# BassyKuo/DAVO

Measured on AMD Instinct MI355X. Metric: pose-net triplets/sec (128x416x3-frame), higher is better.
Workload: dtype f32 (v_mfma_f32_32x32x2_f32: the reference's arithmetic, slim.conv2d in float32); 1 GPU; BASELINE.json configs[1]: single MI355X, batch=32 synthetic 128x416 triplets, dilatedPoseNN-cnv6_128 + se_flow + fc_tanh (segmask_all + abs_flow); batch_per_gpu=32, height=128, width=416, parallelism=window-sharded replicas x1, batches_in_flight=1

## Files before the change

davo_amd/_lib.py:

```python
import ctypes
import os
import subprocess

_HERE = os.path.dirname(os.path.abspath(__file__))
CSRC = os.path.join(_HERE, "csrc")
INCLUDE = os.path.join(os.path.dirname(_HERE), "include")
UNITS = ("api", "forward", "range_guard", "plan", "weights", "launch_f32", "launch_h3", "launch_h3s", "launch_h3w", "launch_h3_generic", "launch_misc", "launch_feature", "comm")


HIPCC_FLAGS = ["--offload-arch=gfx950", "-O3", "-std=c++17", "-fno-slp-vectorize"]


def lib_path(suffix=None):
    if suffix is None:
        suffix = os.environ.get("DAVO_LIB_SUFFIX", "")
    return os.path.join(_HERE, "libdavo_hip%s.so" % suffix)


LIB_PATH = lib_path()

EXPORTS = (
    "davo_create", "davo_set_posenn_se", "davo_load_weight", "davo_weights_missing", "davo_forward", "davo_forward_device", "davo_submit", "davo_wait", "davo_pending",
    "davo_forward_depth", "davo_forward_device_depth", "davo_submit_depth", "davo_calibrate_depth",
    "davo_last_error", "davo_destroy", "davo_device_malloc", "davo_device_free", "davo_memcpy_h2d",
    "davo_memcpy_d2h", "davo_synchronize", "davo_set_stream", "davo_set_inflight", "davo_profile_enable",
    "davo_profile_reset", "davo_profile_entry", "davo_profile_samples", "davo_last_plan", "davo_last_split", "davo_set_option", "davo_set_precision", "davo_set_impl", "davo_debug_read", "davo_conv2d_same",
    "davo_host_alloc", "davo_host_free", "davo_host_register", "davo_host_unregister", "davo_calibrate", "davo_activation_range", "davo_set_activation_shifts", "davo_reset_range_state", "davo_range_stats", "davo_range_report",
    "davo_comm_preload", "davo_comm_unique_id", "davo_comm_init", "davo_comm_size", "davo_allgather_poses", "davo_allgather_poses_device",
    "davo_comm_allreduce", "davo_comm_barrier", "davo_comm_destroy", "davo_plan_layer", "davo_tile_filter_rows",
    "davo_set_pairs", "davo_get_pairs",
    "davo_set_feature_export", "davo_forward_features",
)
COMM_ID_BYTES = 128


class DavoVariant(ctypes.Structure):
    _fields_ = [(n, ctypes.c_int32) for n in ("cin_per_frame", "cnv6_out", "se_act", "norm_flow",
                                              "abs_mode", "att_source", "mask_rgb", "mask_info")]


class DavoFeatureOut(ctypes.Structure):
    _fields_ = [(n, ctypes.c_void_p) for n in ("att_19", "attention", "masked_image", "image", "feat_rot", "feat_trans")]


def sources():
    return sorted(os.path.join(CSRC, f) for f in os.listdir(CSRC) if f.endswith((".hip", ".h"))) + \
           [os.path.join(INCLUDE, "davo_hip.h")]


LLVM_OBJDUMP = "/opt/rocm/lib/llvm/bin/llvm-objdump"


class PackedF32Error(RuntimeError):
    """The linked device code holds packed float32 arithmetic (see HIPCC_FLAGS above): the build is refused."""


def scan_packed_f32(so_path):
    import re
    import shutil
    import tempfile
    pat = re.compile(r"^\s*v_pk_(fma|mul|add)_f32\b")
    hits = []
    d = tempfile.mkdtemp(prefix="davo_isa_")
    try:
        tmp = os.path.join(d, "lib.so")
        shutil.copy(so_path, tmp)
        subprocess.check_call([LLVM_OBJDUMP, "--offloading", tmp], stdout=subprocess.DEVNULL, cwd=d)
        objs = sorted(f for f in os.listdir(d) if "amdgcn" in f)
        if not objs:
            raise PackedF32Error("no gfx950 code object found in %s: the packed-float32 scan cannot vouch for it" % so_path)
        for f in objs:
            kernel = None
            out = subprocess.run([LLVM_OBJDUMP, "-d", os.path.join(d, f)], check=True, capture_output=True, text=True).stdout
            for line in out.splitlines():
                m = re.match(r"^[0-9a-f]+ <([^>]+)>:", line)
                if m:
                    kernel = m.group(1)
                elif pat.match(line):
                    hits.append((kernel, line.strip()))
    finally:
        shutil.rmtree(d, ignore_errors=True)
    return hits


def build(force=False, verbose=False, suffix=None, extra_flags=(), allow_packed_f32=False):
    out = lib_path(suffix)
    if not force and os.path.exists(out) and all(os.path.getmtime(out) >= os.path.getmtime(s) for s in sources()):
        return out
    from concurrent.futures import ThreadPoolExecutor
    hipcc = os.environ.get("HIPCC", "/opt/rocm/bin/hipcc")
    flags = HIPCC_FLAGS + ["-fPIC", "-Wall", "-Wno-unused-function"] + \
        list(extra_flags) + os.environ.get("DAVO_EXTRA_HIPCC_FLAGS", "").split()
    objdir = os.path.join(CSRC, "build%s" % (suffix if suffix is not None else os.environ.get("DAVO_LIB_SUFFIX", "")))
    os.makedirs(objdir, exist_ok=True)
    headers = [s for s in sources() if s.endswith(".h")]
    newest_header = max(os.path.getmtime(h) for h in headers)

    def compile_unit(u):
        src, obj = os.path.join(CSRC, u + ".hip"), os.path.join(objdir, u + ".o")
        if not force and os.path.exists(obj) and os.path.getmtime(obj) >= max(os.path.getmtime(src), newest_header):
            return obj
        cmd = [hipcc] + flags + ["-c", "-o", obj, src]
        if verbose:
            print(" ".join(cmd), flush=True)
        subprocess.check_call(cmd)
        return obj

    with ThreadPoolExecutor(max_workers=min(len(UNITS), os.cpu_count() or 4)) as ex:
        objs = list(ex.map(compile_unit, UNITS))
    staged = out + ".unchecked"
    cmd = [hipcc, "--offload-arch=gfx950", "-shared", "-fPIC", "-o", staged] + objs + ["-ldl", "-Wl,-rpath,/opt/rocm/lib"]
    if verbose:
        print(" ".join(cmd), flush=True)
    subprocess.check_call(cmd)
    hits = [] if allow_packed_f32 else scan_packed_f32(staged)
    if hits:
        os.remove(staged)
        raise PackedF32Error("%d packed float32 instruction(s) in the device code, e.g. %s: `%s' - one operand-select form of them "
                             "miscomputes on gfx950 (DESIGN.md section 4); the library was not installed"
                             % (len(hits), hits[0][0], hits[0][1]))
    os.replace(staged, out)
    return out


_lib = None
_lib_lock = __import__("threading").Lock()


def lib():
    global _lib
    if _lib is not None:
        return _lib
    with _lib_lock:
        return _load()


def _load():
    global _lib
    if _lib is not None:
        return _lib
    if not os.path.exists(LIB_PATH):
        raise RuntimeError("libdavo_hip.so is not built (%s missing): run `python -c 'import "
                           "__graft_entry__ as g; g.build()'`; there is no CPU fallback" % LIB_PATH)
    L = ctypes.CDLL(LIB_PATH)
    vp, i, f32p = ctypes.c_void_p, ctypes.c_int, ctypes.POINTER(ctypes.c_float)
    L.davo_create.argtypes = [ctypes.POINTER(vp), i, i, i, i, ctypes.POINTER(DavoVariant)]
    L.davo_set_posenn_se.argtypes = [vp, i]
    L.davo_load_weight.argtypes = [vp, ctypes.c_char_p, f32p, ctypes.POINTER(ctypes.c_int64), i]
    L.davo_weights_missing.argtypes = [vp]
    L.davo_forward.argtypes = [vp, i, vp, vp, vp, vp]
    L.davo_forward_device.argtypes = [vp, i, vp, vp, vp, vp, ctypes.POINTER(ctypes.c_float)]
    L.davo_submit.argtypes = [vp, i, vp, vp, vp, vp, i]
    L.davo_forward_depth.argtypes = [vp, i, vp, vp, vp, vp, vp]
    L.davo_forward_device_depth.argtypes = [vp, i, vp, vp, vp, vp, vp, ctypes.POINTER(ctypes.c_float)]
    L.davo_submit_depth.argtypes = [vp, i, vp, vp, vp, vp, vp, i]
    L.davo_calibrate_depth.argtypes = [vp, i, vp, vp, vp, vp, ctypes.POINTER(i)]
    L.davo_wait.argtypes = [vp, i]
    L.davo_pending.argtypes = [vp]
    L.davo_last_error.argtypes = [vp]
    L.davo_last_error.restype = ctypes.c_char_p
    L.davo_destroy.argtypes = [vp]
    L.davo_destroy.restype = None
    L.davo_device_malloc.argtypes = [vp, ctypes.c_size_t, ctypes.POINTER(vp)]
    L.davo_device_free.argtypes = [vp, vp]
    L.davo_host_alloc.argtypes = [i, ctypes.c_size_t, ctypes.POINTER(vp)]
    L.davo_host_free.argtypes = [vp]
    L.davo_host_register.argtypes = [i, vp, ctypes.c_size_t]
    L.davo_host_unregister.argtypes = [vp]
    L.davo_calibrate.argtypes = [vp, i, vp, vp, vp, ctypes.POINTER(i)]
    L.davo_activation_range.argtypes = [vp, f32p, ctypes.POINTER(i), i]
    L.davo_set_activation_shifts.argtypes = [vp, ctypes.POINTER(i)]
    L.davo_reset_range_state.argtypes = [vp]
    llp = ctypes.POINTER(ctypes.c_longlong)
    L.davo_range_stats.argtypes = [vp, llp, llp, llp]
    L.davo_range_report.argtypes = [vp]
    L.davo_range_report.restype = ctypes.c_char_p
    L.davo_memcpy_h2d.argtypes = [vp, vp, vp, ctypes.c_size_t]
    L.davo_memcpy_d2h.argtypes = [vp, vp, vp, ctypes.c_size_t]
    L.davo_synchronize.argtypes = [vp]
    L.davo_set_stream.argtypes = [vp, vp]
    L.davo_set_inflight.argtypes = [vp, i]
    L.davo_profile_enable.argtypes = [vp, i]
    L.davo_profile_reset.argtypes = [vp]
    L.davo_profile_entry.argtypes = [vp, i, ctypes.c_char_p, i, ctypes.POINTER(i), ctypes.POINTER(ctypes.c_double)]
    L.davo_profile_samples.argtypes = [vp, ctypes.c_char_p, i, f32p, i]
    L.davo_last_plan.argtypes = [vp, i, i, ctypes.POINTER(i), ctypes.POINTER(i)]
    L.davo_last_split.argtypes = [vp, i, ctypes.POINTER(i)]
    L.davo_set_option.argtypes = [vp, ctypes.c_char_p, i]
    L.davo_set_precision.argtypes = [vp, i]
    L.davo_set_impl.argtypes = [vp, i]
    L.davo_set_pairs.argtypes = [vp, i]
    L.davo_get_pairs.argtypes = [vp]
    L.davo_set_feature_export.argtypes = [vp, i]
    L.davo_forward_features.argtypes = [vp, i, vp, vp, vp, vp, vp, ctypes.POINTER(DavoFeatureOut)]
    L.davo_debug_read.argtypes = [vp, ctypes.c_char_p, f32p, ctypes.c_size_t]
    L.davo_conv2d_same.argtypes = [i, f32p, i, i, i, i, f32p, i, i, f32p, i, i, i, i, f32p, ctypes.c_char_p, i]
    ip = ctypes.POINTER(i)
    L.davo_plan_layer.argtypes = [i, i, i, ip, ip, ip]
    L.davo_tile_filter_rows.argtypes = [i] * 8 + [ip, ip, i, ip]
    L.davo_comm_preload.argtypes = [ctypes.c_char_p, i]
    L.davo_comm_unique_id.argtypes = [vp, ctypes.c_char_p, i]
    L.davo_comm_init.argtypes = [vp, i, i, vp]
    L.davo_comm_size.argtypes = [vp, ip, ip]
    L.davo_allgather_poses.argtypes = [vp, f32p, i, i, f32p, f32p]
    L.davo_allgather_poses_device.argtypes = [vp, vp, i, vp, f32p]
    L.davo_comm_allreduce.argtypes = [vp, ctypes.POINTER(ctypes.c_double), i]
    L.davo_comm_barrier.argtypes = [vp]
    L.davo_comm_destroy.argtypes = [vp]
    for name in EXPORTS:
        fn = getattr(L, name)
        if name not in ("davo_last_error", "davo_destroy", "davo_range_report"):
            fn.restype = ctypes.c_int
    _lib = L
    return L
```

davo_amd/csrc/api.hip:

```cpp
#include <algorithm>
#include <cmath>
#include <cstdlib>
#include <cstdint>
#include <cstring>

#include "ctx.h"
#include "launch.h"
#include "plan.h"

using namespace davo;

namespace davo {

int zero_now(davo_ctx* c, void* p, size_t bytes) {
    HIP_TRY(c, hipMemset(p, 0, bytes));
    HIP_TRY(c, hipStreamSynchronize(nullptr));
    return DAVO_OK;
}

int alloc_input_set(davo_ctx* c, InputSet* s, bool zero_unread) {
    const PlaneBytes nb = plane_bytes(c);
    const size_t n = (size_t)c->max_batch;
    HIP_TRY(c, hipMalloc(&s->img, nb.img * n));
    HIP_TRY(c, hipMalloc(&s->flow, nb.flow * n));
    HIP_TRY(c, hipMalloc(&s->seg, nb.seg * n));
    if (needs_depth(c)) HIP_TRY(c, hipMalloc(&s->depth, nb.depth * n));
    if (zero_unread) {
        { int rc = zero_now(c, s->flow, nb.flow * n); if (rc) return rc; }
        { int rc = zero_now(c, s->seg, nb.seg * n); if (rc) return rc; }
    }
    return DAVO_OK;
}

}

namespace {

void free_input_set(InputSet& s) {
    for (void* q : {s.img, s.flow, s.seg, s.depth}) if (q) (void)hipFree(q);
    s = InputSet();
}

void free_slot(Slot& s) {
    for (auto p : s.d_act) if (p) (void)hipFree(p);
    void* misc[] = {s.d_partial, s.d_tab, s.d_packed, s.d_pose_partial, s.d_counters, s.d_se, s.d_se_scale, s.d_se_partial};
    for (auto p : misc) if (p) (void)hipFree(p);
    if (s.stream) (void)hipStreamDestroy(s.stream);
    s = Slot();
}

void free_se_workspace(Slot& s) {
    for (float** p : {&s.d_se, &s.d_se_scale, &s.d_se_partial}) { if (*p) (void)hipFree(*p); *p = nullptr; }
}

int alloc_se_workspace(davo_ctx* c, Slot* s) {
    const size_t NB = 2 * (size_t)c->max_batch;
    free_se_workspace(*s);
    HIP_TRY(c, hipMalloc(reinterpret_cast<void**>(&s->d_se), NB * c->H2 * c->W2 * 512 * sizeof(float)));
    HIP_TRY(c, hipMalloc(reinterpret_cast<void**>(&s->d_se_scale), NB * 2 * 256 * sizeof(float)));
    HIP_TRY(c, hipMalloc(reinterpret_cast<void**>(&s->d_se_partial), NB * SE5_CHUNKS * 256 * sizeof(float)));
    return DAVO_OK;
}

int alloc_slot(davo_ctx* c, Slot* s) {
    const size_t NB = 2 * (size_t)c->max_batch;
    HIP_TRY(c, hipStreamCreateWithFlags(&s->stream, hipStreamNonBlocking));
    for (int i = 0; i < 7; ++i)
        HIP_TRY(c, hipMalloc(reinterpret_cast<void**>(&s->d_act[i]), NB * c->act_floats_per_img[i] * sizeof(float)));
    HIP_TRY(c, hipMalloc(reinterpret_cast<void**>(&s->d_packed), NB * (size_t)c->H * c->W * 10 * sizeof(float)));
    const size_t partial_bytes = (size_t)c->max_batch * SQ_CHUNKS * (att_class_table(c->v.att_source) ? 3 * SQ_REC : 2 * 2) * sizeof(float);
    HIP_TRY(c, hipMalloc(reinterpret_cast<void**>(&s->d_partial), partial_bytes));
    HIP_TRY(c, hipMalloc(reinterpret_cast<void**>(&s->d_tab), (size_t)c->max_batch * 3 * NCLS * sizeof(float)));
    HIP_TRY(c, hipMalloc(reinterpret_cast<void**>(&s->d_pose_partial), NB * 2 * PH_SPLIT * 3 * sizeof(float)));
    { int rc = zero_now(c, s->d_partial, partial_bytes); if (rc) return rc; }
    HIP_TRY(c, hipMalloc(reinterpret_cast<void**>(&s->d_counters), ((size_t)c->max_batch + 1 + SK_TILE_COUNTERS) * sizeof(unsigned)));
    { int rc = zero_now(c, s->d_counters, ((size_t)c->max_batch + 1 + SK_TILE_COUNTERS) * sizeof(unsigned)); if (rc) return rc; }
    if (c->posenn_se) { int rc = alloc_se_workspace(c, s); if (rc) return rc; }
    return DAVO_OK;
}

}

extern "C" {

int davo_create(davo_ctx** out, int device, int H, int W, int max_batch, const davo_variant* v) {
    if (!out || !v) return DAVO_ERR_INVALID;
    *out = nullptr;
    davo_ctx* c = new davo_ctx();
    *out = c;
    c->device = device; c->H = H; c->W = W; c->max_batch = max_batch;
    c->v = Variant{v->cin_per_frame, v->cnv6_out, v->se_act, v->norm_flow, v->abs_mode, v->att_source,
                   v->mask_rgb, v->mask_info};
    if (H < 16 || W < 16 || H % 4 || W % 4) return fail(c, DAVO_ERR_INVALID, "H and W must be multiples of 4 and >= 16 (got %dx%d)", H, W);
    if (max_batch < 1) return fail(c, DAVO_ERR_INVALID, "max_batch must be >= 1");
    if (v->cin_per_frame != 5 && v->cin_per_frame != 3) return fail(c, DAVO_ERR_INVALID, "cin_per_frame must be 3 or 5");
    if (ilog2_exact(v->cnv6_out) < 5 || v->cnv6_out > 256) return fail(c, DAVO_ERR_INVALID, "cnv6_out must be 32, 64, 128 or 256");
    if (v->se_act < 0 || v->se_act > 2 || v->abs_mode < 0 || v->abs_mode > 3 || v->att_source < 0 || v->att_source > 12)
        return fail(c, DAVO_ERR_INVALID, "variant field out of range");
    int ndev = 0;
    HIP_TRY(c, hipGetDeviceCount(&ndev));
    if (device < 0 || device >= ndev) return fail(c, DAVO_ERR_INVALID, "device %d not present (%d visible)", device, ndev);
    HIP_TRY(c, hipSetDevice(device));
    {
        hipDeviceProp_t prop;
        HIP_TRY(c, hipGetDeviceProperties(&prop, device));
        c->dev_cus = prop.multiProcessorCount > 0 ? prop.multiProcessorCount : 256;
        c->ncu = c->dev_cus;
    }
    c->needed = needed_names(c->v);

    c->H1 = (H + 1) / 2; c->W1 = (W + 1) / 2;
    c->H2 = (c->H1 + 1) / 2; c->W2 = (c->W1 + 1) / 2;
    c->H3 = (c->H2 + 1) / 2; c->W3 = (c->W2 + 1) / 2;
    const int c6 = c->v.cnv6_out;
    init_layer(c->L[0], "cnv1", 7, 2, 1, 8, 16, 1);
    init_layer(c->L[1], "cnv2", 5, 2, 1, 16, 32, 1);
    init_layer(c->L[2], "cnv3", 3, 1, 2, 32, 64, 1);
    init_layer(c->L[3], "cnv4", 3, 1, 4, 64, 128, 1);
    init_layer(c->L[4], "cnv5", 3, 1, 8, 128, 256, 1);
    init_layer(c->L[5], "cnv6", 3, 1, 2, 256, 2 * c6, 1);
    init_layer(c->L[6], "cnv7", 3, 2, 1, c6, 256, 2);

    const int ch[7] = {16, 32, 64, 128, 256, 2 * c6, 512};
    const size_t px[7] = {(size_t)c->H1 * c->W1, (size_t)c->H2 * c->W2, (size_t)c->H2 * c->W2, (size_t)c->H2 * c->W2,
                          (size_t)c->H2 * c->W2, (size_t)c->H2 * c->W2, (size_t)c->H3 * c->W3};
    for (int i = 0; i < 7; ++i) {
        c->act_ch[i] = ch[i];
        c->act_floats_per_img[i] = px[i] * ch[i];
    }
    c->slots.resize(1);
    { int rc = alloc_slot(c, &c->slots[0]); if (rc) return rc; }
    HIP_TRY(c, hipMalloc(reinterpret_cast<void**>(&c->d_zeros), 256));
    { int rc = zero_now(c, c->d_zeros, 256); if (rc) return rc; }
    HIP_TRY(c, hipMalloc(reinterpret_cast<void**>(&c->d_range_base), (1 + RANGE_RING) * RANGE_WORDS * sizeof(unsigned)));
    { int rc = zero_now(c, c->d_range_base, (1 + RANGE_RING) * RANGE_WORDS * sizeof(unsigned)); if (rc) return rc; }
    return DAVO_OK;
}

int davo_set_posenn_se(davo_ctx* c, int mode) {
    if (!c) return DAVO_ERR_INVALID;
    if (mode != 0 && mode != 1) return fail(c, DAVO_ERR_INVALID, "posenn_se mode must be 0 (none) or 1 (insert)");
    if (!c->weights.empty() || c->forward_seen)
        return fail(c, DAVO_ERR_INVALID, "davo_set_posenn_se must be called before the first davo_load_weight and the first forward "
                    "(it changes the variant's variables and cnv6's layout)");
    if (mode && c->v.att_source != 0)
        return fail(c, DAVO_ERR_INVALID, "the feature-attention PoseNN (`-se_insert') runs with att_source 0 (`-no_segmask') only, got %d", c->v.att_source);
    HIP_TRY(c, hipSetDevice(c->device));
    c->posenn_se = mode;
    const int c6 = c->v.cnv6_out;
    if (mode) init_layer(c->L[5], "cnv6", 3, 1, 2, 256, c6, 2);
    else init_layer(c->L[5], "cnv6", 3, 1, 2, 256, 2 * c6, 1);
    c->needed = needed_names(c->v, mode);
    for (Slot& s : c->slots) {
        if (mode) { int rc = alloc_se_workspace(c, &s); if (rc) return rc; }
        else free_se_workspace(s);
    }
    c->last_slot = 0;
    return DAVO_OK;
}

int davo_load_weight(davo_ctx* c, const char* tf_name, const float* data, const int64_t* shape, int ndim) {
    if (!c || !tf_name || !data || !shape || ndim < 1 || ndim > 4) return fail(c, DAVO_ERR_INVALID, "bad argument to davo_load_weight");
    std::vector<int64_t> want;
    if (!expected_shape(c, tf_name, &want)) return fail(c, DAVO_ERR_INVALID, "unknown variable `%s'", tf_name);
    bool listed = false;
    for (auto& n : c->needed) listed |= (n == tf_name);
    if (!listed) return fail(c, DAVO_ERR_INVALID, "variable `%s' is not part of this variant", tf_name);
    std::vector<int64_t> got(shape, shape + ndim);
    if (got != want) {
        std::string g, w;
        for (auto d : got) g += std::to_string(d) + ",";
        for (auto d : want) w += std::to_string(d) + ",";
        return fail(c, DAVO_ERR_INVALID, "`%s': shape [%s] does not match expected [%s]", tf_name, g.c_str(), w.c_str());
    }
    size_t n = 1;
    for (auto d : got) n *= (size_t)d;
    HostTensor& t = c->weights[tf_name];
    t.shape = got;
    t.data.assign(data, data + n);
    HIP_TRY(c, hipSetDevice(c->device));
    const std::string nm = tf_name;
    const bool dense = is_dense_weight(nm);
    if (t.dev) { (void)hipFree(t.dev); t.dev = nullptr; }
    if (dense) { int rc = upload(c, t.data, &t.dev); if (rc) return rc; }
    c->packed_ready = false;
    c->packed_h_ready = false;
    c->pred_ready = false;
    return DAVO_OK;
}

int davo_weights_missing(davo_ctx* c) {
    if (!c) return DAVO_ERR_INVALID;
    std::string names;
    const int n = missing_weights(c, &names);
    if (n) c->err = "weights not loaded: " + names;
    return n;
}

namespace {

int resolve_depth(davo_ctx* c, const char* fn, bool depth_form, const void** depth) {
    if (!needs_depth(c)) { *depth = nullptr; return DAVO_OK; }
    if (!depth_form) return fail(c, DAVO_ERR_INVALID, "%s: this variant reads depth planes (att_source %d): call %s_depth", fn, c->v.att_source, fn);
    if (!*depth) return fail(c, DAVO_ERR_INVALID, "%s_depth: null depth pointer", fn);
    return DAVO_OK;
}

}

static int forward_device_entry(davo_ctx* c, int B, const void* d_img, const void* d_flow, const void* d_seg, const void* d_depth,
                                void* d_pose, float* elapsed_ms, bool depth_form) {
    if (!c) return DAVO_ERR_INVALID;
    if (B < 1 || B > c->max_batch) return fail(c, DAVO_ERR_INVALID, "batch %d outside [1,%d]", B, c->max_batch);
    if (!d_img || !d_flow || !d_seg || !d_pose) return fail(c, DAVO_ERR_INVALID, "null device pointer");
    { int rc = resolve_depth(c, "davo_forward_device", depth_form, &d_depth); if (rc) return rc; }
    const Inputs in{d_img, d_flow, d_seg, d_depth};
    HIP_TRY(c, hipSetDevice(c->device));
    const bool ticketed = c->impl == 0 && c->precision == 1;
    if (ticketed) { int rc = ticket_reserve(c); if (rc) return rc; }
    Run run = make_run(c, c->next_slot);
    c->next_slot = (c->next_slot + 1) % c->inflight;
    Ticket t{};
    if (ticketed) { int rc = ticket_begin(c, &run, B, in, &t); if (rc) return rc; }
    if (!ticketed && c->book.spans_full()) {
        const int rc = judge_all(c);
        if (rc == DAVO_ERR_RANGE) c->book.defer(rc, c->err);
        else if (rc) return rc;
    }
    c->book.note_issue(d_pose, B);
    RunResult res;
    if (!elapsed_ms) {
        int rc = forward_device(c, run, B, in, d_pose, &res);
        return ticketed ? ticket_end(c, rc, res, t, d_pose) : rc;
    }
    hipEvent_t e0 = nullptr, e1 = nullptr;
    int rc = DAVO_OK;
    auto hip_ok = [&](hipError_t e, const char* what) {
        if (e != hipSuccess && rc == DAVO_OK) rc = fail(c, DAVO_ERR_HIP, "%s failed: %s", what, hipGetErrorString(e));
        return e == hipSuccess;
    };
    if (hip_ok(hipEventCreate(&e0), "hipEventCreate") && hip_ok(hipEventCreate(&e1), "hipEventCreate") &&
        hip_ok(hipEventRecord(e0, run.stream), "hipEventRecord")) {
        rc = forward_device(c, run, B, in, d_pose, &res);
        if (rc == DAVO_OK && hip_ok(hipEventRecord(e1, run.stream), "hipEventRecord") &&
            hip_ok(hipEventSynchronize(e1), "hipEventSynchronize"))
            hip_ok(hipEventElapsedTime(elapsed_ms, e0, e1), "hipEventElapsedTime");
    }
    if (e0) (void)hipEventDestroy(e0);
    if (e1) (void)hipEventDestroy(e1);
    if (ticketed) rc = ticket_end(c, rc, res, t, d_pose);
    if (rc == DAVO_OK && c->inflight == 1) rc = judge_all(c);
    return rc;
}

int davo_forward_device(davo_ctx* c, int B, const void* d_img, const void* d_flow, const void* d_seg,
                        void* d_pose, float* elapsed_ms) {
    return forward_device_entry(c, B, d_img, d_flow, d_seg, nullptr, d_pose, elapsed_ms, false);
}

int davo_forward_device_depth(davo_ctx* c, int B, const void* d_img, const void* d_flow, const void* d_seg, const void* d_depth,
                              void* d_pose, float* elapsed_ms) {
    return forward_device_entry(c, B, d_img, d_flow, d_seg, d_depth, d_pose, elapsed_ms, true);
}


namespace {

int ensure_stream_state(davo_ctx* c, int slot) {
    if (!c->d_pose_ring[0])
        for (int k = 0; k < STREAM_POSES; ++k) {
            HIP_TRY(c, hipMalloc(reinterpret_cast<void**>(&c->d_pose_ring[k]), (size_t)c->max_batch * 12 * sizeof(float)));
            HIP_TRY(c, hipHostMalloc(reinterpret_cast<void**>(&c->h_pose_ring[k]), (size_t)c->max_batch * 12 * sizeof(float), hipHostMallocDefault));
            HIP_TRY(c, hipEventCreateWithFlags(&c->pose_done[k], hipEventDisableTiming));
            HIP_TRY(c, hipEventCreateWithFlags(&c->st_copied[k], hipEventDisableTiming));
        }
    if (!c->stream_sets[slot].img) { int rc = alloc_input_set(c, &c->stream_sets[slot], true); if (rc) return rc; }
    return DAVO_OK;
}

Inputs from_window(const davo_ctx* c, const Inputs& in, int b0) {
    const PlaneBytes nb = plane_bytes(c);
    auto at = [b0](const void* q, size_t bytes) -> const void* { return q ? static_cast<const uint8_t*>(q) + bytes * b0 : nullptr; };
    return Inputs{at(in.img, nb.img), at(in.flow, nb.flow), at(in.seg, nb.seg), at(in.depth, nb.depth)};
}

int stage_inputs(davo_ctx* c, const InputSet& set, const Inputs& host, int b0, int nb, bool sources_only_seg, int sel, hipStream_t s) {
    const PlaneBytes n = plane_bytes(c);
    const Inputs src = from_window(c, host, b0);
    auto dst = [b0](void* q, size_t bytes) { return static_cast<uint8_t*>(q) + bytes * b0; };
    if (sel != PAIRS_BOTH) {
        const int src1 = sel == PAIRS_SRC1;
        auto copy2d = [&](uint8_t* d, const void* h, size_t pitch, size_t off, size_t width, size_t rows) {
            return hipMemcpy2DAsync(d + off, pitch, static_cast<const uint8_t*>(h) + off, pitch, width, rows, hipMemcpyHostToDevice, s);
        };
        const size_t row = (size_t)c->W * 9, third = row / 3;
        HIP_TRY(c, copy2d(dst(set.img, n.img), src.img, row, src1 ? third : 0, 2 * third, (size_t)nb * c->H));
        HIP_TRY(c, copy2d(dst(set.flow, n.flow), src.flow, n.flow, src1 ? n.flow / 4 : 0, n.flow / 4, nb));
        const size_t plane = n.seg / 3;
        if (att_tgt_attended(c->v.att_source)) HIP_TRY(c, copy2d(dst(set.seg, n.seg), src.seg, n.seg, src1 ? plane : 0, 2 * plane, nb));
        else HIP_TRY(c, copy2d(dst(set.seg, n.seg), src.seg, n.seg, src1 ? 2 * plane : 0, plane, nb));
        if (src.depth) HIP_TRY(c, copy2d(dst(set.depth, n.depth), src.depth, n.depth, src1 ? plane : 0, 2 * plane, nb));
        return DAVO_OK;
    }
    HIP_TRY(c, hipMemcpyAsync(dst(set.img, n.img), src.img, n.img * nb, hipMemcpyHostToDevice, s));
    if (nb == 1) HIP_TRY(c, hipMemcpyAsync(dst(set.flow, n.flow), src.flow, n.flow / 2, hipMemcpyHostToDevice, s));
    else HIP_TRY(c, hipMemcpy2DAsync(dst(set.flow, n.flow), n.flow, src.flow, n.flow, n.flow / 2, nb, hipMemcpyHostToDevice, s));
    if (!sources_only_seg || att_tgt_attended(c->v.att_source) || nb < 4) HIP_TRY(c, hipMemcpyAsync(dst(set.seg, n.seg), src.seg, n.seg * nb, hipMemcpyHostToDevice, s));
    else
        for (int plane = 0; plane < 3; plane += 2)
            HIP_TRY(c, hipMemcpy2DAsync(dst(set.seg, n.seg) + plane * (n.seg / 3), n.seg, (const uint8_t*)src.seg + plane * (n.seg / 3), n.seg,
                                        n.seg / 3, nb, hipMemcpyHostToDevice, s));
    if (src.depth) HIP_TRY(c, hipMemcpyAsync(dst(set.depth, n.depth), src.depth, n.depth * nb, hipMemcpyHostToDevice, s));
    return DAVO_OK;
}

int deliver_front(davo_ctx* c) {
    const StreamJob j = c->jobs.front();
    c->jobs.pop_front();
    while (j.ticketed && c->book.pending(j.seq)) {
        const int rc = judge_front(c);
        if (rc == DAVO_ERR_RANGE && !c->opt_auto_range) c->book.defer(rc, c->err);
        else if (rc) return rc;
    }
    HIP_TRY(c, hipEventSynchronize(c->pose_done[j.pr]));
    memcpy(j.pose_out, c->h_pose_ring[j.pr], (size_t)j.B * 12 * sizeof(float));
    return DAVO_OK;
}

int deliver_all(davo_ctx* c) {
    while (!c->jobs.empty()) { const int rc = deliver_front(c); if (rc) { c->jobs.clear(); return rc; } }
    return DAVO_OK;
}

}

static int submit_entry(davo_ctx* c, int B, const uint8_t* img, const float* flow, const float* seg, const float* depth_in, float* pose_out,
                        int hold, bool depth_form) {
    if (!c) return DAVO_ERR_INVALID;
    if (!img || !flow || !seg || !pose_out) return fail(c, DAVO_ERR_INVALID, "null host pointer");
    const void* depth = depth_in;
    { int rc = resolve_depth(c, "davo_submit", depth_form, &depth); if (rc) return rc; }
    if (B < 1 || B > c->max_batch) return fail(c, DAVO_ERR_INVALID, "batch %d outside [1,%d]", B, c->max_batch);
    if (hold < 0) return fail(c, DAVO_ERR_INVALID, "hold must be >= 0");
    HIP_TRY(c, hipSetDevice(c->device));
    while (!c->jobs.empty() && ((int)c->jobs.size() >= STREAM_POSES || hipEventQuery(c->pose_done[c->jobs.front().pr]) == hipSuccess)) {
        const int rc = deliver_front(c);
        if (rc) return rc;
    }
    const bool ticketed = c->impl == 0 && c->precision == 1;
    if (ticketed) { int rc = ticket_reserve(c); if (rc) return rc; }
    const int slot = c->next_slot, pr = (int)(c->n_submitted % STREAM_POSES);
    { int rc = ensure_stream_state(c, slot); if (rc) return rc; }
    Run run = make_run(c, slot);
    c->next_slot = (c->next_slot + 1) % c->inflight;
    hipStream_t s = run.stream;
    const InputSet& set = c->stream_sets[slot];
    { int rc = stage_inputs(c, set, Inputs{img, flow, seg, depth}, 0, B, true, c->pairs, s); if (rc) return rc; }
    const bool track_copy = hold < STREAM_POSES;
    if (track_copy) HIP_TRY(c, hipEventRecord(c->st_copied[pr], s));

    Ticket t{};
    if (ticketed) { int rc = ticket_begin(c, &run, B, set.view(), &t, true); if (rc) return rc; }
    c->book.note_issue();
    RunResult res;
    int rc = forward_device(c, run, B, set.view(), c->d_pose_ring[pr], &res);
    if (ticketed) rc = ticket_end(c, rc, res, t, c->d_pose_ring[pr], c->h_pose_ring[pr]);
    if (rc) return rc;
    HIP_TRY(c, hipMemcpyAsync(c->h_pose_ring[pr], c->d_pose_ring[pr], (size_t)B * 12 * sizeof(float), hipMemcpyDeviceToHost, s));
    HIP_TRY(c, hipEventRecord(c->pose_done[pr], s));
    c->jobs.push_back(StreamJob{B, pose_out, pr, ticketed && res.h3, t.seq});
    c->copy_tracked[pr] = track_copy;
    ++c->n_submitted;
    if (track_copy && (unsigned long long)hold < c->n_submitted) {
        const int q = (int)((c->n_submitted - 1 - hold) % STREAM_POSES);
        if (c->copy_tracked[q]) HIP_TRY(c, hipEventSynchronize(c->st_copied[q]));
    }
    return DAVO_OK;
}

int davo_submit(davo_ctx* c, int B, const uint8_t* img, const float* flow, const float* seg, float* pose_out, int hold) {
    return submit_entry(c, B, img, flow, seg, nullptr, pose_out, hold, false);
}

int davo_submit_depth(davo_ctx* c, int B, const uint8_t* img, const float* flow, const float* seg, const float* depth, float* pose_out, int hold) {
    return submit_entry(c, B, img, flow, seg, depth, pose_out, hold, true);
}

int davo_wait(davo_ctx* c, int leave_pending) {
    if (!c) return DAVO_ERR_INVALID;
    if (leave_pending < 0) return fail(c, DAVO_ERR_INVALID, "leave_pending must be >= 0");
    HIP_TRY(c, hipSetDevice(c->device));
    while ((int)c->jobs.size() > leave_pending) { const int rc = deliver_front(c); if (rc) return rc; }
    return DAVO_OK;
}

int davo_pending(davo_ctx* c) { return c ? (int)c->jobs.size() : DAVO_ERR_INVALID; }

namespace {

struct FxLayout { size_t rot, trans, masked, image, attention, att_19, total; };
FxLayout fx_layout(const davo_ctx* c, int cap) {
    const size_t HW = (size_t)c->H * c->W, n = (size_t)cap, c6 = (size_t)c->v.cnv6_out;
    FxLayout l{};
    l.rot = 0;
    l.trans = l.rot + n * HW * c6;
    l.masked = l.trans + n * HW * c6;
    l.image = l.masked + n * HW * 9;
    l.attention = l.image + n * HW * 9;
    l.att_19 = l.attention + n * HW * 3;
    l.total = l.att_19 + n * 3 * NCLS;
    return l;
}

void free_fx_workspace(davo_ctx* c) {
    if (c->d_fx) (void)hipFree(c->d_fx);
    c->d_fx = nullptr;
    c->fx_cap = 0;
}

bool fx_wanted(const davo_feature_out* o) {
    return o && (o->att_19 || o->attention || o->masked_image || o->image || o->feat_rot || o->feat_trans);
}

int export_features(davo_ctx* c, const Inputs& in, int w0, int nw, int b0, int B, const davo_feature_out& out) {
    if (!c->d_fx || c->fx_cap < 1) return fail(c, DAVO_ERR_INVALID, "internal: no feature export workspace");
    if (c->last_pairs != PAIRS_BOTH || w0 < 0 || w0 + nw > c->last_B) return fail(c, DAVO_ERR_INVALID, "internal: feature export of windows the last forward did not run");
    const size_t HW = (size_t)c->H * c->W, c6 = (size_t)c->v.cnv6_out;
    const bool h3 = c->last_precision == 1;
    const FxLayout l = fx_layout(c, c->fx_cap);
    const Slot& ws = last_workspace(c);
    hipStream_t s = last_stream(c);
    for (int p0 = 0; p0 < nw; p0 += c->fx_cap) {
        const int np = std::min(c->fx_cap, nw - p0);
        const Inputs win = from_window(c, in, w0 + p0);
        float* const w_att19 = out.att_19 ? c->d_fx + l.att_19 : nullptr;
        float* const w_att = out.attention ? c->d_fx + l.attention : nullptr;
        float* const w_masked = out.masked_image ? c->d_fx + l.masked : nullptr;
        float* const w_image = out.image ? c->d_fx + l.image : nullptr;
        float* const w_rot = out.feat_rot ? c->d_fx + l.rot : nullptr;
        float* const w_trans = out.feat_trans ? c->d_fx + l.trans : nullptr;
        if (w_att19 || w_att || w_masked || w_image) {
            ProfScope ps(c, s, "feature_maps");
            HIP_TRY(c, launch_feature_maps(static_cast<const uint8_t*>(win.img), static_cast<const float*>(win.seg),
                                           ws.d_tab + (size_t)(w0 + p0) * 3 * NCLS, c->v, np, c->H, c->W, w_att19, w_att, w_masked, w_image, s));
        }
        if (w_rot || w_trans) {
            ProfScope ps(c, s, "feature_resize_cnv6");
            HIP_TRY(c, launch_feature_resize_cnv6(h3, ws.d_act[5], w0 + p0, np, c->H2, c->W2, (int)c6, h3 ? ldexpf(1.0f, -c->act_shift[5]) : 1.0f,
                                                  w_rot, w_trans, s));
        }
        const size_t first = (size_t)(b0 + p0);
        auto frames = [&](float* host, const float* dev, size_t per_window) -> int {
            if (!host) return DAVO_OK;
            for (int f = 0; f < 3; ++f)
                HIP_TRY(c, hipMemcpyAsync(host + ((size_t)f * B + first) * per_window, dev + (size_t)f * np * per_window,
                                          (size_t)np * per_window * sizeof(float), hipMemcpyDeviceToHost, s));
            return DAVO_OK;
        };
        { int rc = frames(out.att_19, w_att19, NCLS); if (rc) return rc; }
        { int rc = frames(out.attention, w_att, HW); if (rc) return rc; }
        { int rc = frames(out.masked_image, w_masked, HW * 3); if (rc) return rc; }
        { int rc = frames(out.image, w_image, HW * 3); if (rc) return rc; }
        if (w_rot) HIP_TRY(c, hipMemcpyAsync(out.feat_rot + first * HW * c6, w_rot, (size_t)np * HW * c6 * sizeof(float), hipMemcpyDeviceToHost, s));
        if (w_trans) HIP_TRY(c, hipMemcpyAsync(out.feat_trans + first * HW * c6, w_trans, (size_t)np * HW * c6 * sizeof(float), hipMemcpyDeviceToHost, s));
        HIP_TRY(c, hipStreamSynchronize(s));
    }
    return DAVO_OK;
}

}

static int forward_entry(davo_ctx* c, int B, const uint8_t* img, const float* flow, const float* seg, const float* depth_in, float* pose_out,
                         bool depth_form, const davo_feature_out* fx = nullptr) {
    if (!c) return DAVO_ERR_INVALID;
    if (!img || !flow || !seg || !pose_out) return fail(c, DAVO_ERR_INVALID, "null host pointer");
    const void* depth = depth_in;
    { int rc = resolve_depth(c, "davo_forward", depth_form, &depth); if (rc) return rc; }
    if (B < 1 || B > c->max_batch) return fail(c, DAVO_ERR_INVALID, "batch %d outside [1,%d]", B, c->max_batch);
    HIP_TRY(c, hipSetDevice(c->device));
    { int rc = deliver_all(c); if (rc) return rc; }
    { int rc = sync_all_slots(c); if (rc) return rc; }
    if (!c->host_set.img) {
        { int rc = alloc_input_set(c, &c->host_set, false); if (rc) return rc; }
        HIP_TRY(c, hipMalloc(&c->s_pose, (size_t)c->max_batch * 12 * sizeof(float)));
    }
    if (!c->copy_stream) HIP_TRY(c, hipStreamCreateWithFlags(&c->copy_stream, hipStreamNonBlocking));
    { int rc = judge_all(c); if (rc) return rc; }
    Run run = make_run(c, 0);
    if (c->book.host_record_due()) {
        HIP_TRY(c, hipMemsetAsync(c->d_range_base, 0, RANGE_WORDS * sizeof(unsigned), run.stream));
    }
    const int chunk = (c->host_chunk > 0 && B >= 2 * c->host_chunk) ? c->host_chunk : B;
    const int nchunks = (B + chunk - 1) / chunk;
    while ((int)c->copy_done.size() < nchunks) {
        hipEvent_t e;
        HIP_TRY(c, hipEventCreateWithFlags(&e, hipEventDisableTiming));
        c->copy_done.push_back(e);
    }
    bool f32_fallback = false;
    RunResult res;
    const bool h3_call = c->impl == 0 && c->precision == 1;
    if (h3_call) { int rc = ensure_ring(c, false); if (rc) return rc; }
    if (!c->h_sync_pose) HIP_TRY(c, hipHostMalloc(reinterpret_cast<void**>(&c->h_sync_pose), (size_t)c->max_batch * 12 * sizeof(float), hipHostMallocDefault));
    unsigned seq = 0;
    for (int i = 0; i < nchunks; ++i) {
        const int b0 = i * chunk, nb = std::min(chunk, B - b0);
        hipStream_t cs = nchunks == 1 ? run.stream : c->copy_stream;
        { int rc = stage_inputs(c, c->host_set, Inputs{img, flow, seg, depth}, b0, nb, false, c->pairs, cs); if (rc) return rc; }
        if (nchunks > 1) {
            HIP_TRY(c, hipEventRecord(c->copy_done[i], c->copy_stream));
            HIP_TRY(c, hipStreamWaitEvent(run.stream, c->copy_done[i], 0));
        }
        if (h3_call && i == nchunks - 1) {
            seq = c->book.next_seq();
            run.snap.record = c->d_range_base; run.snap.host_mirror = c->h_range_dev; run.snap.seq = seq; run.snap.B = nb; run.snap.se = c->posenn_se;
        }
        int rc = forward_device(c, run, nb, from_window(c, c->host_set.view(), b0), (float*)c->s_pose + (size_t)b0 * 12, &res);
        if (rc) return rc;
        f32_fallback |= res.f32_fallback;
        if (fx && i < nchunks - 1 && (rc = export_features(c, from_window(c, c->host_set.view(), b0), 0, nb, b0, B, *fx))) return rc;
    }
    const int last_b0 = (nchunks - 1) * chunk;
    auto export_last = [&]() { return fx ? export_features(c, from_window(c, c->host_set.view(), last_b0), 0, B - last_b0, last_b0, B, *fx) : DAVO_OK; };
    if (f32_fallback) ++c->n_f32_batches;
    HIP_TRY(c, hipMemcpyAsync(c->h_sync_pose, c->s_pose, (size_t)B * 12 * sizeof(float), hipMemcpyDeviceToHost, run.stream));
    HIP_TRY(c, hipStreamSynchronize(run.stream));
    memcpy(pose_out, c->h_sync_pose, (size_t)B * 12 * sizeof(float));
    if (!res.h3) return export_last();
    unsigned raw[RANGE_WORDS];
    int rc = wait_record(c, c->h_range, seq, run.stream, raw);
    if (rc) return rc;
    rc = judge_record(c, raw, c->act_shift);
    if (rc == DAVO_ERR_RANGE && c->opt_auto_range) {
        rc = recover_batch(c, Reissue{B, c->pairs, c->host_set.view(), c->s_pose, false, 0});
        if (rc == DAVO_OK) HIP_TRY(c, hipMemcpy(pose_out, c->s_pose, (size_t)B * 12 * sizeof(float), hipMemcpyDeviceToHost));
        if (rc == DAVO_OK && fx) rc = export_features(c, c->host_set.view(), 0, B, 0, B, *fx);
        return rc;
    }
    return rc == DAVO_OK ? export_last() : rc;
}

int davo_forward(davo_ctx* c, int B, const uint8_t* img, const float* flow, const float* seg, float* pose_out) {
    return forward_entry(c, B, img, flow, seg, nullptr, pose_out, false);
}

int davo_forward_depth(davo_ctx* c, int B, const uint8_t* img, const float* flow, const float* seg, const float* depth, float* pose_out) {
    return forward_entry(c, B, img, flow, seg, depth, pose_out, true);
}

int davo_set_feature_export(davo_ctx* c, int on) {
    if (!c) return DAVO_ERR_INVALID;
    HIP_TRY(c, hipSetDevice(c->device));
    { int rc = sync_all_slots(c); if (rc) return rc; }
    if (!on) { free_fx_workspace(c); c->fx_on = false; return DAVO_OK; }
    if (!c->d_fx) {
        const int cap = c->host_chunk > 0 ? std::min(c->max_batch, 2 * c->host_chunk - 1) : c->max_batch;
        HIP_TRY(c, hipMalloc(reinterpret_cast<void**>(&c->d_fx), fx_layout(c, cap).total * sizeof(float)));
        c->fx_cap = cap;
    }
    c->fx_on = true;
    return DAVO_OK;
}

int davo_forward_features(davo_ctx* c, int B, const uint8_t* img, const float* flow, const float* seg, const float* depth, float* pose_out,
                          const davo_feature_out* out) {
    if (!c) return DAVO_ERR_INVALID;
    if (!c->fx_on) return fail(c, DAVO_ERR_NOT_READY, "davo_forward_features: the feature export is off - call davo_set_feature_export(ctx, 1) first");
    if (c->pairs != PAIRS_BOTH)
        return fail(c, DAVO_ERR_INVALID, "davo_forward_features runs both pairs of every window, the reference's semantics (davo.py:1456-1457): "
                    "davo_set_pairs(ctx, DAVO_PAIRS_BOTH) first (the selection is %d)", c->pairs);
    return forward_entry(c, B, img, flow, seg, depth, pose_out, true, fx_wanted(out) ? out : nullptr);
}

int davo_range_stats(davo_ctx* c, long long* recalibrations, long long* f32_batches, long long* reissued) {
    if (!c) return DAVO_ERR_INVALID;
    if (recalibrations) *recalibrations = c->n_recalibrations;
    if (f32_batches) *f32_batches = c->n_f32_batches;
    if (reissued) *reissued = c->n_reissued;
    return DAVO_OK;
}

int davo_activation_range(davo_ctx* c, float* max_abs, int* shifts, int reset) {
    if (!c) return DAVO_ERR_INVALID;
    HIP_TRY(c, hipSetDevice(c->device));
    { int rc = judge_all(c); if (rc && rc != DAVO_ERR_RANGE) return rc; }
    for (int i = 0; i < 6; ++i) {
        if (max_abs) max_abs[i] = c->range_seen[i];
        if (shifts) shifts[i] = c->act_shift[i];
    }
    if (reset) for (int i = 0; i < 6; ++i) c->range_seen[i] = 0.f;
    return DAVO_OK;
}

const char* davo_range_report(const davo_ctx* c) { return c ? c->range_report.c_str() : ""; }

int davo_set_activation_shifts(davo_ctx* c, const int* shifts) {
    if (!c) return DAVO_ERR_INVALID;
    { int rc = judge_all(c); if (rc) return rc; }
    { int rc = freeze_pending_and_reset_ring(c); if (rc) return rc; }
    c->book.host_record_stale();
    for (int i = 0; i < 6; ++i) {
        const int s = shifts ? shifts[i] : 0;
        if (s < -60 || s > 60) return fail(c, DAVO_ERR_INVALID, "activation shift %d outside [-60,60]", s);
        c->act_shift[i] = s;
    }
    return DAVO_OK;
}

int davo_reset_range_state(davo_ctx* c) {
    if (!c) return DAVO_ERR_INVALID;
    HIP_TRY(c, hipSetDevice(c->device));
    const int verdict = judge_all(c);
    if (verdict && verdict != DAVO_ERR_RANGE) return verdict;
    const std::string verdict_err = c->err;
    { int rc = freeze_pending_and_reset_ring(c); if (rc) return rc; }
    { int rc = zero_now(c, c->d_range_base, RANGE_WORDS * sizeof(unsigned)); if (rc) return rc; }
    for (int i = 0; i < 7; ++i) c->act_shift[i] = 0;
    for (int i = 0; i < 6; ++i) c->range_seen[i] = 0.f;
    c->book.reset();
    c->range_report.clear();
    if (verdict) { c->err = verdict_err; return verdict; }
    return DAVO_OK;
}

static int calibrate_entry(davo_ctx* c, int B, const void* d_img, const void* d_flow, const void* d_seg, const void* d_depth, int* shifts_out,
                           bool depth_form) {
    if (!c) return DAVO_ERR_INVALID;
    if (B < 1 || B > c->max_batch) return fail(c, DAVO_ERR_INVALID, "batch %d outside [1,%d]", B, c->max_batch);
    if (!d_img || !d_flow || !d_seg) return fail(c, DAVO_ERR_INVALID, "null device pointer");
    { int rc = resolve_depth(c, "davo_calibrate", depth_form, &d_depth); if (rc) return rc; }
    HIP_TRY(c, hipSetDevice(c->device));
    { int rc = judge_all(c); if (rc) return rc; }
    { int rc = freeze_pending_and_reset_ring(c); if (rc) return rc; }
    float* d_pose = nullptr;
    HIP_TRY(c, hipMalloc(reinterpret_cast<void**>(&d_pose), (size_t)B * 12 * sizeof(float)));
    const int rc = calibrate_on(c, B, Inputs{d_img, d_flow, d_seg, d_depth}, d_pose, PAIRS_BOTH);
    (void)hipFree(d_pose);
    if (rc == DAVO_OK && shifts_out) for (int i = 0; i < 6; ++i) shifts_out[i] = c->act_shift[i];
    return rc;
}

int davo_calibrate(davo_ctx* c, int B, const void* d_img, const void* d_flow, const void* d_seg, int* shifts_out) {
    return calibrate_entry(c, B, d_img, d_flow, d_seg, nullptr, shifts_out, false);
}

int davo_calibrate_depth(davo_ctx* c, int B, const void* d_img, const void* d_flow, const void* d_seg, const void* d_depth, int* shifts_out) {
    return calibrate_entry(c, B, d_img, d_flow, d_seg, d_depth, shifts_out, true);
}

const char* davo_last_error(const davo_ctx* c) { return c ? c->err.c_str() : "null context"; }

void davo_destroy(davo_ctx* c) {
    if (!c) return;
    (void)hipSetDevice(c->device);
    (void)sync_all_slots(c);
    comm_release(c);
    for (auto& kv : c->weights) if (kv.second.dev) (void)hipFree(kv.second.dev);
    for (auto& L : c->L) {
        if (L.d_w) (void)hipFree(L.d_w);
        if (L.d_b) (void)hipFree(L.d_b);
        if (L.d_wh) (void)hipFree(L.d_wh);
        if (L.d_bh) (void)hipFree(L.d_bh);
    }
    for (auto e : c->copy_done) (void)hipEventDestroy(e);
    if (c->copy_stream) { (void)hipStreamSynchronize(c->copy_stream); (void)hipStreamDestroy(c->copy_stream); }
    free_input_set(c->host_set);
    for (InputSet& set : c->stream_sets) free_input_set(set);
    for (InputSet& set : c->snap_sets) free_input_set(set);
    if (c->read_stream) { (void)hipStreamSynchronize(c->read_stream); (void)hipStreamDestroy(c->read_stream); }
    if (c->h_range) (void)hipHostFree(c->h_range);
    for (int k = 0; k < STREAM_POSES; ++k) {
        if (c->d_pose_ring[k]) (void)hipFree(c->d_pose_ring[k]);
        if (c->h_pose_ring[k]) (void)hipHostFree(c->h_pose_ring[k]);
        if (c->pose_done[k]) (void)hipEventDestroy(c->pose_done[k]);
        if (c->st_copied[k]) (void)hipEventDestroy(c->st_copied[k]);
    }
    if (c->h_sync_pose) (void)hipHostFree(c->h_sync_pose);
    free_fx_workspace(c);
    void* misc[] = {c->d_reissue_pose, c->d_range_base, c->d_splitk, c->d_pose_tiles, c->d_w1patch, c->d_w2patch, c->d_w3patch, c->d_w1patch_f32, c->d_w2patch_f32, c->d_w3patch_f32, c->d_zeros, c->d_wpred, c->d_bpred, c->s_pose};
    for (auto p : misc) if (p) (void)hipFree(p);
    for (auto& kv : c->tile_orders) if (kv.second) (void)hipFree(kv.second);
    for (auto& pe : c->prof_entries)
        for (auto& ab : pe.pending) { (void)hipEventDestroy(ab.first); (void)hipEventDestroy(ab.second); }
    for (auto e : c->event_pool) (void)hipEventDestroy(e);
    for (auto& sl : c->slots) free_slot(sl);
    delete c;
}

int davo_host_alloc(int device, size_t bytes, void** out) {
    if (!out || bytes == 0) return DAVO_ERR_INVALID;
    if (hipSetDevice(device) != hipSuccess) return DAVO_ERR_HIP;
    return hipHostMalloc(out, bytes, hipHostMallocDefault) == hipSuccess ? DAVO_OK : DAVO_ERR_HIP;
}
int davo_host_free(void* p) { return hipHostFree(p) == hipSuccess ? DAVO_OK : DAVO_ERR_HIP; }
int davo_host_register(int device, void* p, size_t bytes) {
    if (!p || bytes == 0) return DAVO_ERR_INVALID;
    if (hipSetDevice(device) != hipSuccess) return DAVO_ERR_HIP;
    return hipHostRegister(p, bytes, hipHostRegisterDefault) == hipSuccess ? DAVO_OK : DAVO_ERR_HIP;
}
int davo_host_unregister(void* p) { return hipHostUnregister(p) == hipSuccess ? DAVO_OK : DAVO_ERR_HIP; }

int davo_device_malloc(davo_ctx* c, size_t bytes, void** out) {
    if (!c || !out) return DAVO_ERR_INVALID;
    HIP_TRY(c, hipSetDevice(c->device));
    HIP_TRY(c, hipMalloc(out, bytes));
    return DAVO_OK;
}
int davo_device_free(davo_ctx* c, void* p) {
    if (!c) return DAVO_ERR_INVALID;
    HIP_TRY(c, hipSetDevice(c->device));
    HIP_TRY(c, hipFree(p));
    return DAVO_OK;
}
int davo_memcpy_h2d(davo_ctx* c, void* dst, const void* src, size_t bytes) {
    if (!c) return DAVO_ERR_INVALID;
    HIP_TRY(c, hipSetDevice(c->device));
    HIP_TRY(c, hipMemcpyAsync(dst, src, bytes, hipMemcpyHostToDevice, last_stream(c)));
    HIP_TRY(c, hipStreamSynchronize(last_stream(c)));
    return DAVO_OK;
}
int davo_memcpy_d2h(davo_ctx* c, void* dst, const void* src, size_t bytes) {
    if (!c) return DAVO_ERR_INVALID;
    HIP_TRY(c, hipSetDevice(c->device));
    HIP_TRY(c, hipMemcpyAsync(dst, src, bytes, hipMemcpyDeviceToHost, last_stream(c)));
    HIP_TRY(c, hipStreamSynchronize(last_stream(c)));
    return DAVO_OK;
}
int davo_synchronize(davo_ctx* c) {
    if (!c) return DAVO_ERR_INVALID;
    HIP_TRY(c, hipSetDevice(c->device));
    { int rc = deliver_all(c); if (rc) return rc; }
    return judge_all(c);
}
int davo_set_stream(davo_ctx* c, void* hip_stream) {
    if (!c) return DAVO_ERR_INVALID;
    if (hip_stream && c->inflight > 1) return fail(c, DAVO_ERR_INVALID, "a caller-owned stream needs davo_set_inflight(ctx, 1)");
    HIP_TRY(c, hipSetDevice(c->device));
    { int rc = deliver_all(c); if (rc) return rc; }
    { int rc = judge_all(c); if (rc) return rc; }
    c->user_stream = static_cast<hipStream_t>(hip_stream);
    c->last_slot = 0;
    return DAVO_OK;
}

int davo_profile_enable(davo_ctx* c, int on) {
    if (!c) return DAVO_ERR_INVALID;
    if (!on && c->prof) { int rc = prof_collect(c); if (rc) return rc; }
    c->prof = on != 0;
    c->prof_dominant_only = on == 2;
    return DAVO_OK;
}
int davo_profile_reset(davo_ctx* c) {
    if (!c) return DAVO_ERR_INVALID;
    int rc = prof_collect(c);
    if (rc) return rc;
    for (auto& pe : c->prof_entries) { pe.launches = 0; pe.total_ms = 0.0; pe.dur_ms.clear(); pe.period_ms.clear(); }
    return DAVO_OK;
}
int davo_profile_samples(davo_ctx* c, const char* name, int which, float* out, int cap) {
    if (!c || !name || which < 0 || which > 1 || cap < 0 || (cap > 0 && !out)) return DAVO_ERR_INVALID;
    int rc = prof_collect(c);
    if (rc) return rc;
    for (const auto& pe : c->prof_entries)
        if (pe.name == name) {
            const std::vector<float>& v = which == 0 ? pe.dur_ms : pe.period_ms;
            const int n = (int)std::min(v.size(), (size_t)cap);
            for (int i = 0; i < n; ++i) out[i] = v[i];
            return (int)v.size();
        }
    return 0;
}
int davo_profile_entry(davo_ctx* c, int i, char* name, int name_len, int* launches, double* total_ms) {
    if (!c) return DAVO_ERR_INVALID;
    int rc = prof_collect(c);
    if (rc) return rc;
    if (i < 0 || i >= (int)c->prof_entries.size()) return DAVO_ERR_INVALID;
    const ProfEntry& pe = c->prof_entries[i];
    if (name && name_len > 0) { strncpy(name, pe.name.c_str(), name_len - 1); name[name_len - 1] = 0; }
    if (launches) *launches = pe.launches;
    if (total_ms) *total_ms = pe.total_ms;
    return DAVO_OK;
}

int davo_last_plan(davo_ctx* c, int layer, int launch, int* mtiles, int* bn) {
    if (!c || layer < 0 || layer > 6 || launch < 0 || launch > 1) return DAVO_ERR_INVALID;
    const int v = c->last_plan[layer][launch];
    if (mtiles) *mtiles = v / 1000;
    if (bn) *bn = v % 1000;
    return DAVO_OK;
}

int davo_last_split(davo_ctx* c, int layer, int* parts) {
    if (!c || layer < 0 || layer > 6) return DAVO_ERR_INVALID;
    if (parts) *parts = c->last_split[layer];
    return DAVO_OK;
}

static int rebuild_slot_streams(davo_ctx* c, int n) {
    for (int i = 0; i < (int)c->slots.size(); ++i) {
        Slot& s = c->slots[i];
        if (s.stream) { HIP_TRY(c, hipStreamDestroy(s.stream)); s.stream = nullptr; }
        if (c->cu_partition && n > 1 && i < n && c->dev_cus == 256) {
            uint32_t mask[8] = {0, 0, 0, 0, 0, 0, 0, 0};
            const int lo = i * 32 / n, hi = (i + 1) * 32 / n;
            for (int b = 0; b < 256; ++b)
                if (b / 8 >= lo && b / 8 < hi) mask[b / 32] |= 1u << (b % 32);
            HIP_TRY(c, hipExtStreamCreateWithCUMask(&s.stream, 8, mask));
        } else {
            HIP_TRY(c, hipStreamCreateWithFlags(&s.stream, hipStreamNonBlocking));
        }
    }
    c->ncu = (c->cu_partition && n > 1 && c->dev_cus == 256) ? 256 / n : c->dev_cus;
    c->last_slot = 0;
    return DAVO_OK;
}

int davo_set_inflight(davo_ctx* c, int n) {
    if (!c || n < 1 || n > MAX_INFLIGHT) return fail(c, DAVO_ERR_INVALID, "inflight must be 1..4");
    if (n > 1 && c->user_stream) return fail(c, DAVO_ERR_INVALID, "in-flight slots use the context's own streams: clear davo_set_stream first");
    HIP_TRY(c, hipSetDevice(c->device));
    { int rc = deliver_all(c); if (rc) return rc; }
    { int rc = sync_all_slots(c); if (rc) return rc; }
    while ((int)c->slots.size() < n) {
        c->slots.emplace_back();
        int rc = alloc_slot(c, &c->slots.back());
        if (rc) return rc;
    }
    c->inflight = n;
    c->next_slot = 0;
    if (c->cu_partition || c->ncu != c->dev_cus) { int rc = rebuild_slot_streams(c, n); if (rc) return rc; }
    return DAVO_OK;
}

int davo_set_option(davo_ctx* c, const char* key, int value) {
    if (!c || !key) return DAVO_ERR_INVALID;
    const std::string k = key;
    if (k == "fuse_pose") c->opt_fuse_pose = value != 0;
    else if (k == "fuse_pack") c->opt_fuse_pack = value < 0 ? -1 : (value != 0);
    else if (k == "share_taps") c->opt_share_taps = value != 0;
    else if (k == "merge_rem") c->opt_merge_rem = value != 0;
    else if (k == "merge_cnv4") c->opt_merge_cnv4 = value != 0;
    else if (k == "tile_208x128") c->opt_tile_208x128 = value != 0;
    else if (k == "merge_order") c->opt_merge_order = value < 0 ? -1 : (value > 2 ? 0 : value);
    else if (k == "skip_order") c->opt_skip_order = value < 0 ? 0 : (value > 2 ? 2 : value);
    else if (k == "patch_cnv2") c->opt_patch_cnv2 = value != 0;
    else if (k == "patch_cnv3") c->opt_patch_cnv3 = value != 0;
    else if (k == "fold_tails") c->opt_fold_tails = value < 0 ? -1 : (value > 2 ? 1 : value);
    else if (k == "deep_ring") c->opt_deep_ring = value != 0;
    else if (k == "wave128") c->opt_wave128 = value < 0 ? 0 : (value > 3 ? 3 : value);
    else if (k == "split_k") c->opt_split_k = value != 0;
    else if (k == "fold_fixup") c->opt_fold_fixup = value != 0;
    else if (k == "f32_n16") c->opt_f32_n16 = value != 0;
    else if (k == "f32_n256") c->opt_f32_n256 = value != 0;
    else if (k == "merge_rem_f32") c->opt_merge_rem_f32 = value < 0 ? 0 : (value > 2 ? 2 : value);
    else if (k == "patch_f32") c->opt_patch_f32 = value != 0;
    else if (k == "auto_range") { int rc = judge_all(c); if (rc) return rc; c->opt_auto_range = value != 0; }
    else if (k == "stable_inputs") { int rc = judge_all(c); if (rc) return rc; c->opt_stable_inputs = value != 0; }
    else if (k == "force_tile") {
        if (value < -1 || value >= NUM_TILES) return fail(c, DAVO_ERR_INVALID, "force_tile must be -1..%d", NUM_TILES - 1);
        for (auto& L : c->L) L.tile_h = (value >= 0 && L.cout >= tile_shape(value).bn) ? value : -1;
    }
    else if (k == "cu_partition") {
        if (c->user_stream) return fail(c, DAVO_ERR_INVALID, "cu_partition uses the context's own streams: clear davo_set_stream first");
        HIP_TRY(c, hipSetDevice(c->device));
        { int rc = sync_all_slots(c); if (rc) return rc; }
        c->cu_partition = value != 0;
        int rc = rebuild_slot_streams(c, c->inflight);
        if (rc) return rc;
    }
    else if (k == "profile_stride") { if (value < 1) return fail(c, DAVO_ERR_INVALID, "profile_stride must be >= 1"); c->prof_stride = value; c->prof_tick = 0; }
    else if (k == "host_chunk") { if (value < 0) return fail(c, DAVO_ERR_INVALID, "host_chunk must be >= 0"); c->host_chunk = value; }
    else return fail(c, DAVO_ERR_INVALID, "unknown option `%s'", key);
    return DAVO_OK;
}

int davo_set_precision(davo_ctx* c, int precision) {
    if (!c || (precision != 0 && precision != 1)) return fail(c, DAVO_ERR_INVALID, "precision must be 0 (f32) or 1 (f16x3)");
    c->precision = precision;
    return DAVO_OK;
}

int davo_set_pairs(davo_ctx* c, int pairs) {
    if (!c) return DAVO_ERR_INVALID;
    if (pairs != DAVO_PAIRS_SRC0 && pairs != DAVO_PAIRS_SRC1 && pairs != DAVO_PAIRS_BOTH)
        return fail(c, DAVO_ERR_INVALID, "pairs must be DAVO_PAIRS_SRC0 (1), DAVO_PAIRS_SRC1 (2) or DAVO_PAIRS_BOTH (3), got %d", pairs);
    c->pairs = pairs;
    return DAVO_OK;
}

int davo_get_pairs(const davo_ctx* c) { return c ? c->pairs : DAVO_ERR_INVALID; }

int davo_set_impl(davo_ctx* c, int impl) {
    if (!c || (impl != 0 && impl != 1)) return fail(c, DAVO_ERR_INVALID, "impl must be 0 (mfma) or 1 (direct)");
    c->impl = impl;
    return DAVO_OK;
}

int davo_debug_read(davo_ctx* c, const char* tensor, float* host_out, size_t n_floats) {
    if (!c || !tensor || !host_out) return DAVO_ERR_INVALID;
    if (c->last_B < 1) return fail(c, DAVO_ERR_NOT_READY, "no forward has run yet");
    const size_t NB = (size_t)pairs_per_window(c->last_pairs) * c->last_B;
    const float* src = nullptr;
    size_t n = 0;
    const std::string t = tensor;
    const Slot& ws = last_workspace(c);
    if (t == "att_table") { src = ws.d_tab; n = (size_t)c->last_B * 3 * NCLS; }
    else if (t == "cnv5_se_scale" || t == "cnv5_se") {
        if (!c->posenn_se) return fail(c, DAVO_ERR_NOT_READY, "`%s' exists in the feature-attention variant only (davo_set_posenn_se)", tensor);
        if (t == "cnv5_se") { src = ws.d_se; n = NB * c->H2 * c->W2 * 512; }
        else { src = ws.d_se_scale; n = NB * 2 * 256; }
    }
    else if (t == "packed") {
        if (!c->packed_valid) {
            HIP_TRY(c, launch_mask_pack(16, static_cast<const uint8_t*>(c->last_in.img), static_cast<const float*>(c->last_in.flow),
                                        static_cast<const float*>(c->last_in.seg), ws.d_tab, c->v, c->last_B, c->H, c->W, ws.d_packed, c->last_pairs, last_stream(c)));
            c->packed_valid = true;
        }
        src = ws.d_packed; n = NB * c->H * c->W * c->packed_ld;
    }
    else {
        const char* names[7] = {"cnv1", "cnv2", "cnv3", "cnv4", "cnv5", "cnv6", "cnv7"};
        for (int i = 0; i < 7; ++i)
            if (t == names[i]) { src = ws.d_act[i]; n = NB * c->act_floats_per_img[i]; }
    }
    if (t == "pose_tiles") {
        if (c->cnv7_valid || !c->d_pose_tiles) return fail(c, DAVO_ERR_NOT_READY, "the pose head did not run fused");
#ifndef DAVO_POSE_DEBUG
        if (n_floats > c->pose_tiles_floats) return fail(c, DAVO_ERR_INVALID, "pose_tiles holds %zu floats", c->pose_tiles_floats);
#endif
        return davo_memcpy_d2h(c, host_out, c->d_pose_tiles, n_floats * sizeof(float));
    }
    if (t == "cnv7" && !c->cnv7_valid)
        return fail(c, DAVO_ERR_NOT_READY, "cnv7 was not materialised: the pose head ran fused (davo_set_option(ctx, \"fuse_pose\", 0))");
    if (!src) return fail(c, DAVO_ERR_INVALID, "unknown tensor `%s'", tensor);
    if (n != n_floats) return fail(c, DAVO_ERR_INVALID, "`%s' holds %zu floats, caller asked for %zu", tensor, n, n_floats);
    int rc = davo_memcpy_d2h(c, host_out, src, n * sizeof(float));
    if (rc) return rc;
    const bool split = c->last_precision == 1 && t != "att_table" && t != "cnv7" && t != "cnv5_se_scale";
    if (split) {
        int ch = 8;
        const char* names[6] = {"cnv1", "cnv2", "cnv3", "cnv4", "cnv5", "cnv6"};
        for (int i = 0; i < 6; ++i) if (t == names[i]) ch = c->act_ch[i];
        if (t == "cnv5_se") ch = 512;
        const int cb = ch < 32 ? ch : 32;
        int shift = t == "cnv5_se" ? c->act_shift[4] : 0;
        for (int i = 0; i < 6; ++i) if (t == names[i]) shift = c->act_shift[i];
        std::vector<float> tmp(ch);
        const size_t npix = n / ch;
        for (size_t px = 0; px < npix; ++px) {
            const _Float16* raw = reinterpret_cast<const _Float16*>(host_out + px * ch);
            for (int k = 0; k < ch; ++k) {
                const _Float16* blk = raw + (size_t)(k / cb) * cb * 2;
                tmp[k] = ldexpf((float)blk[k % cb] + (float)blk[cb + k % cb], -shift);
            }
            memcpy(host_out + px * ch, tmp.data(), ch * sizeof(float));
        }
    }
    return DAVO_OK;
}

int davo_tile_filter_rows(int m0, int m1, int Hout, int Wout, int Hin, int stride, int pad_t, int rate,
                          int* ky0, int* nky, int nblocks, int* chunk_map) {
    if (!ky0 || !nky || Hout < 1 || Wout < 1 || Hin < 1 || stride < 1 || rate < 1 || m0 < 0 || nblocks < 0) return DAVO_ERR_INVALID;
    const FilterRows fr = valid_filter_rows(m0, m1, Hout, Wout, Hin, stride, pad_t, rate);
    *ky0 = fr.ky0;
    *nky = fr.nky;
    if (chunk_map)
        for (int v = 0; v < 3 * fr.nky * nblocks; ++v) chunk_map[v] = h3_real_chunk(v, fr.ky0, fr.nky);
    return DAVO_OK;
}

int davo_plan_layer(int M, int npad, int groups, int* rows, int* tile_bm, int* tile_bn) {
    if (M < 1 || npad < 32 || npad % 32 || groups < 1 || !rows || !tile_bm || !tile_bn) return DAVO_ERR_INVALID;
    const std::vector<LaunchH> plan = plan_layer_h3(M, npad, groups, -1, npad == 256);
    if (plan.empty() || plan.size() > 2) return DAVO_ERR_INVALID;
    for (size_t i = 0; i < plan.size(); ++i) {
        const TileShape ts = tile_shape(plan[i].tile);
        rows[i] = plan[i].rows; tile_bm[i] = ts.bm; tile_bn[i] = ts.bn;
    }
    return (int)plan.size();
}

int davo_conv2d_same(int device, const float* x, int N, int H, int W, int Cin, const float* w, int k, int Cout,
                     const float* bias, int stride, int rate, int relu, int precision, float* y, char* err, int err_len) {
    auto bad = [&](const char* m, int code) {
        if (err && err_len > 0) { strncpy(err, m, err_len - 1); err[err_len - 1] = 0; }
        return code;
    };
    const int cl = ilog2_exact(Cin);
    if (!x || !w || !bias || !y) return bad("null pointer", DAVO_ERR_INVALID);
    if (cl < 2) return bad("Cin must be a power of two >= 4", DAVO_ERR_INVALID);
    if (precision == 1 && cl < 3) return bad("f16x3 needs Cin >= 8", DAVO_ERR_INVALID);
    if (!(k == 1 || k == 3 || k == 5 || k == 7) || !(stride == 1 || stride == 2) || rate < 1)
        return bad("k in {1,3,5,7}, stride in {1,2}, rate >= 1", DAVO_ERR_INVALID);
    if (hipSetDevice(device) != hipSuccess) return bad("hipSetDevice failed", DAVO_ERR_HIP);
    ConvLayer L;
    init_layer(L, "conv", k, stride, rate, Cin, Cout, 1);
    int Ho, Wo, pt, pl;
    same_pad(H, k, stride, rate, &Ho, &pt);
    same_pad(W, k, stride, rate, &Wo, &pl);
    const size_t nx = (size_t)N * H * W * Cin, ny = (size_t)N * Ho * Wo * Cout;
    std::vector<float> bp(precision == 1 ? L.npad_h : L.npad, 0.f);
    memcpy(bp.data(), bias, Cout * sizeof(float));
    std::vector<float> wp;
    std::vector<_Float16> wph, xh;
    const void *hx = x, *hw = nullptr;
    size_t wbytes = 0;
    if (precision == 1) {
        wph.assign((size_t)L.npad_h * L.nchunks_h * 64, (_Float16)0.0f);
        L.wscale = weight_prescale(w, (size_t)k * k * Cin * Cout);
        pack_conv_weights_h3(w, k, Cin, Cout, nullptr, Cin, L.cb_log2, L.tpc_log2, L.cpb, L.nchunks_h, L.wscale, wph.data());
        hw = wph.data(); wbytes = wph.size() * sizeof(_Float16);
        const int cb = 1 << L.cb_log2;
        xh.resize(nx * 2);
        for (size_t px = 0; px < nx / Cin; ++px)
            for (int ch = 0; ch < Cin; ++ch) {
                _Float16* blk = xh.data() + px * Cin * 2 + (size_t)(ch / cb) * cb * 2;
                split_f16(x[px * Cin + ch], blk + ch % cb, blk + cb + ch % cb);
            }
        hx = xh.data();
    } else {
        wp.assign((size_t)L.npad * L.kpad, 0.f);
        pack_conv_weights(w, k, Cin, Cout, nullptr, Cin, L.npad, L.kpad, wp.data());
        hw = wp.data(); wbytes = wp.size() * sizeof(float);
    }
    void *dx = nullptr, *dw = nullptr, *db = nullptr, *dy = nullptr, *dz = nullptr;
    hipError_t e = hipSuccess;
    auto chk = [&](hipError_t r) { if (e == hipSuccess) e = r; };
    chk(hipMalloc(&dx, nx * 4)); chk(hipMalloc(&dw, wbytes));
    chk(hipMalloc(&db, bp.size() * 4)); chk(hipMalloc(&dy, ny * 4));
    chk(hipMalloc(&dz, 256));
    if (e == hipSuccess) {
        chk(hipMemset(dz, 0, 256));
        chk(hipMemcpy(dx, hx, nx * 4, hipMemcpyHostToDevice));
        chk(hipMemcpy(dw, hw, wbytes, hipMemcpyHostToDevice));
        chk(hipMemcpy(db, bp.data(), bp.size() * 4, hipMemcpyHostToDevice));
        if (precision == 1) {
            const int tile = Cout <= 32 ? TILE_128x32 : Cout <= 64 ? TILE_256x64 : Cout <= 128 ? TILE_256x128 : TILE_128x256;
            const TileShape ts = tile_shape(tile);
            ConvParamsH p{};
            p.x = static_cast<const uint8_t*>(dx); p.w = static_cast<const uint8_t*>(dw);
            p.bias = static_cast<const float*>(db); p.y = static_cast<uint8_t*>(dy);
            p.zeros = static_cast<const uint8_t*>(dz);
            p.Hin = H; p.Win = W; p.Hout = Ho; p.Wout = Wo; p.x_pix_bytes = (long)Cin * 4; p.x_pix_log2 = -1;
            p.cb_log2 = L.cb_log2; p.tpc_log2 = L.tpc_log2; p.cpb = L.cpb; p.nchunks = L.nchunks_h;
            p.w_row_bytes = (long)L.nchunks_h * 128; p.y_mode = 0; p.y_ld = Cout; p.Cout = Cout;
            p.pad_t = pt; p.pad_l = pl; p.rate = rate; p.M = N * Ho * Wo; p.ntaps = k * k;
            p.Mtot = p.M; p.xs = 0; p.ntiles_n = L.npad_h / ts.bn; p.relu = relu; p.out_scale = 1.0f / L.wscale; p.bias_scale = L.wscale; p.range = nullptr;
            dim3 grid((p.M + ts.bm - 1) / ts.bm * p.ntiles_n, 1);
            const hipError_t le = launch_h3_generic(k, stride, tile, p, grid, nullptr);
            chk(le);
        } else {
            ConvParams p{};
            p.x = static_cast<const float*>(dx); p.w = static_cast<const float*>(dw);
            p.bias = static_cast<const float*>(db); p.y = static_cast<float*>(dy);
            p.zeros = static_cast<const float*>(dz);
            p.Hin = H; p.Win = W; p.Hout = Ho; p.Wout = Wo; p.cin_log2 = cl; p.x_ld = Cin; p.y_ld = Cout;
            p.Cout = Cout; p.pad_t = pt; p.pad_l = pl; p.rate = rate; p.M = N * Ho * Wo;
            p.nchunks = L.nchunks; p.Kpad = L.kpad; p.ntaps = k * k; p.ntiles_n = L.npad / L.BN; p.relu = relu;
            dim3 grid((p.M + BM - 1) / BM * p.ntiles_n, 1);
            chk(launch_conv(k, stride, L.BN, p, grid, nullptr));
        }
        chk(hipDeviceSynchronize());
        chk(hipMemcpy(y, dy, ny * 4, hipMemcpyDeviceToHost));
    }
    (void)hipFree(dz); (void)hipFree(dx); (void)hipFree(dw); (void)hipFree(db); (void)hipFree(dy);
    if (e != hipSuccess) return bad(hipGetErrorString(e), DAVO_ERR_HIP);
    return DAVO_OK;
}

}
```

davo_amd/csrc/conv_igemm.h:

```cpp
#pragma once
#include <hip/hip_runtime.h>
#include <stdint.h>

#include "params.h"

#ifndef DAVO_F32_ABLATE_A
#define DAVO_F32_ABLATE_A 0
#define DAVO_F32_ABLATE_B 0
#endif
#ifndef DAVO_F32_EARLY_STORE
#define DAVO_F32_EARLY_STORE 1
#endif
#ifndef DAVO_F32_FRAG0
#define DAVO_F32_FRAG0 1
#endif
#ifndef DAVO_F32_FAST_EPILOGUE
#define DAVO_F32_FAST_EPILOGUE 1
#endif
#ifndef DAVO_F32_FRAG_AHEAD
#define DAVO_F32_FRAG_AHEAD 0
#endif
#ifndef DAVO_F32_EARLY_STORE_MIN_BN
#define DAVO_F32_EARLY_STORE_MIN_BN 32
#endif
#ifndef DAVO_F32_ACC_AGPR
#define DAVO_F32_ACC_AGPR 0
#endif
#if DAVO_F32_ACC_AGPR
#define DAVO_MFMA32(acc_, a_, b_) asm volatile("v_mfma_f32_32x32x2_f32 %0, %1, %2, %0" : "+a"(acc_) : "v"(a_), "v"(b_))
#else
#define DAVO_MFMA32(acc_, a_, b_) acc_ = __builtin_amdgcn_mfma_f32_32x32x2f32(a_, b_, acc_, 0, 0, 0)
#endif
#if DAVO_F32_ACC_AGPR
#define DAVO_F4C(v_, c_) ((c_) == 0 ? (v_).x : (c_) == 1 ? (v_).y : (c_) == 2 ? (v_).z : (v_).w)
#define DAVO_MFMA_TILE(FA_, FB_)                                                                   \
            _Pragma("unroll") for (int c_ = 0; c_ < 4; ++c_)                                       \
                _Pragma("unroll") for (int i_ = 0; i_ < T::TM; ++i_)                               \
                    _Pragma("unroll") for (int j_ = 0; j_ < T::TN; ++j_)                           \
                        DAVO_MFMA32(acc[i_][j_], DAVO_F4C(FA_, c_), DAVO_F4C(FB_, c_));
#else
#define DAVO_MFMA_TILE(FA_, FB_)                                                                   \
            _Pragma("unroll") for (int i_ = 0; i_ < T::TM; ++i_)                                   \
                _Pragma("unroll") for (int j_ = 0; j_ < T::TN; ++j_) {                             \
                    DAVO_MFMA32(acc[i_][j_], (FA_).x, (FB_).x);                                    \
                    DAVO_MFMA32(acc[i_][j_], (FA_).y, (FB_).y);                                    \
                    DAVO_MFMA32(acc[i_][j_], (FA_).z, (FB_).z);                                    \
                    DAVO_MFMA32(acc[i_][j_], (FA_).w, (FB_).w);                                    \
                }
#endif
#ifndef DAVO_F32_ABLATE_BARRIER
#define DAVO_F32_ABLATE_BARRIER 0
#endif

namespace davo {

typedef float f32x16 __attribute__((ext_vector_type(16)));

__device__ __forceinline__ int xcd_remap(int bid, int nwg) {
    const int q = nwg >> 3, r = nwg & 7, xcd = bid & 7;
    const int start = xcd < r ? xcd * (q + 1) : r * (q + 1) + (xcd - r) * q;
    return start + (bid >> 3);
}

template <int KS, int STRIDE, int BN, int LAYER>
__device__ __forceinline__ void conv_igemm_f32_body(const ConvParams& p, const int wg_x, const int nwg_x, const int wg_y) {
    using T = Tile<BN>;
    constexpr bool N16 = BN == 16;
    extern __shared__ __attribute__((aligned(16))) float smem[];
    float* As = smem;
    float* Bs = smem + 2 * BM * LDK;

    const int tid = threadIdx.x;
    const int lane = tid & 63, wid = tid >> 6;
    const int li = lane & 31, lh = lane >> 5;
    const int wm = wid / T::WN, wn = wid % T::WN;

    const int tile_i = xcd_remap(wg_x, nwg_x);
    const int tile = p.tile_order ? __builtin_amdgcn_readfirstlane(p.tile_order[tile_i]) : tile_i;
    const int ntile = tile % p.ntiles_n, mtile = p.mtile0 + tile / p.ntiles_n;
    const int grp = wg_y;
    const float* __restrict__ xg = p.x + p.x_coff + grp * p.g_x_coff;
    const float* __restrict__ wg = p.w + grp * p.g_w + (long)ntile * BN * p.Kpad;
    const float* __restrict__ bg = p.bias + grp * p.g_bias + ntile * BN;
    float* __restrict__ yg = p.y + p.y_coff + grp * p.g_y_coff;

    const int r0 = tid >> 3, kk = (tid & 7) * 4;
    constexpr int RPP = T::RPP;
    int iy0[4], ix0[4], pix0[4];
#pragma unroll
    for (int j = 0; j < 4; ++j) {
        if (j >= T::A_LOADS) { iy0[j] = -(1 << 28); ix0[j] = 0; pix0[j] = 0; continue; }
        const int m = mtile * BM + r0 + RPP * j;
        if (m < p.M) {
            const int hw = p.Hout * p.Wout;
            const int n = m / hw, rem = m - n * hw;
            const int oy = rem / p.Wout, ox = rem - oy * p.Wout;
            iy0[j] = oy * STRIDE - p.pad_t;
            ix0[j] = ox * STRIDE - p.pad_l;
            pix0[j] = n * p.Hin * p.Win;
        } else {
            iy0[j] = -(1 << 28);
            ix0[j] = 0;
            pix0[j] = 0;
        }
    }
    const int cmask = (1 << p.cin_log2) - 1;

    float4 ra0, ra1, ra2, ra3, rb0, rb1, rb2, rb3;
    rb0 = rb1 = rb2 = rb3 = make_float4(0.f, 0.f, 0.f, 0.f);
    float4 sa0, sa1, sa2, sa3, sb0, sb1, sb2, sb3;
    sa0 = sa1 = sa2 = sa3 = sb0 = sb1 = sb2 = sb3 = make_float4(0.f, 0.f, 0.f, 0.f);
    const float *pa0 = p.zeros, *pa1 = p.zeros, *pa2 = p.zeros, *pa3 = p.zeros;
    int st0 = 0, st1 = 0, st2 = 0, st3 = 0;
    const int cpt = p.cin_log2 >= 5 ? 1 << (p.cin_log2 - 5) : 1;
    int l_cb = 0;
#define DAVO_ADDR_A(j_, ptr_, st_)                                                                 \
    {                                                                                              \
        const int iy = iy0[j_] + dy, ix = ix0[j_] + dx;                                            \
        const bool ok = tap_ok && (unsigned)iy < (unsigned)p.Hin && (unsigned)ix < (unsigned)p.Win && !DAVO_F32_ABLATE_A; \
        const long off = (long)(pix0[j_] + iy * p.Win + ix) * p.x_ld + c;                          \
               \
        ptr_ = ok ? xg + off : p.zeros;                                                            \
        st_ = ok ? BK : 0;                                                                         \
    }
#define DAVO_LOAD_CHUNK(q_) DAVO_LOAD_CHUNK_R(q_, ra0, ra1, ra2, ra3, rb0, rb1, rb2, rb3)
#define DAVO_LOAD_CHUNK_R(q_, ra0, ra1, ra2, ra3, rb0, rb1, rb2, rb3)                              \
    {                                                                                              \
        const int kg = (q_) * BK + kk;                                                             \
        if (l_cb == 0) {                                                                           \
            const int tap = kg >> p.cin_log2, c = kg & cmask;                                      \
            const int ky = tap / KS, kx = tap - ky * KS;                                           \
            const int dy = ky * p.rate, dx = kx * p.rate;                                          \
            const bool tap_ok = tap < p.ntaps;                                                     \
            DAVO_ADDR_A(0, pa0, st0) DAVO_ADDR_A(1, pa1, st1)                                      \
            if constexpr (T::A_LOADS > 2) { DAVO_ADDR_A(2, pa2, st2) DAVO_ADDR_A(3, pa3, st3) }    \
        } else {                                                                                   \
            pa0 += st0; pa1 += st1;                                                                \
            if constexpr (T::A_LOADS > 2) { pa2 += st2; pa3 += st3; }                              \
        }                                                                                          \
        l_cb = l_cb + 1 == cpt ? 0 : l_cb + 1;                                                     \
        ra0 = *reinterpret_cast<const float4*>(pa0);                                               \
        ra1 = *reinterpret_cast<const float4*>(pa1);                                               \
        if constexpr (T::A_LOADS > 2) {                                                            \
            ra2 = *reinterpret_cast<const float4*>(pa2);                                           \
            ra3 = *reinterpret_cast<const float4*>(pa3);                                           \
        }                                                                                          \
        const float* wrow = wg + (long)r0 * p.Kpad + (DAVO_F32_ABLATE_B ? kk : kg);               \
        if (!N16 || r0 < 16) rb0 = *reinterpret_cast<const float4*>(wrow);                         \
        if constexpr (T::NB_LOADS > 1) rb1 = *reinterpret_cast<const float4*>(wrow + (long)RPP * p.Kpad); \
        if constexpr (T::NB_LOADS > 2) {                                                           \
            rb2 = *reinterpret_cast<const float4*>(wrow + 2L * RPP * p.Kpad);                      \
            rb3 = *reinterpret_cast<const float4*>(wrow + 3L * RPP * p.Kpad);                      \
        }                                                                                          \
    }
#define DAVO_STORE_CHUNK(buf_) DAVO_STORE_CHUNK_R(buf_, ra0, ra1, ra2, ra3, rb0, rb1, rb2, rb3)
#define DAVO_STORE_CHUNK_R(buf_, ra0, ra1, ra2, ra3, rb0, rb1, rb2, rb3)                           \
    {                                                                                              \
        float* a_ = As + (buf_) * BM * LDK + r0 * LDK + kk;                                        \
        float* b_ = Bs + (buf_) * BN * LDK + r0 * LDK + kk;                                        \
        *reinterpret_cast<float4*>(a_) = ra0;                                                      \
        *reinterpret_cast<float4*>(a_ + RPP * LDK) = ra1;                                          \
        if constexpr (T::A_LOADS > 2) {                                                            \
            *reinterpret_cast<float4*>(a_ + 2 * RPP * LDK) = ra2;                                  \
            *reinterpret_cast<float4*>(a_ + 3 * RPP * LDK) = ra3;                                  \
        }                                                                                          \
        if (!N16 || r0 < 16) *reinterpret_cast<float4*>(b_) = rb0;                                 \
        if constexpr (T::NB_LOADS > 1) *reinterpret_cast<float4*>(b_ + RPP * LDK) = rb1;           \
        if constexpr (T::NB_LOADS > 2) {                                                           \
            *reinterpret_cast<float4*>(b_ + 2 * RPP * LDK) = rb2;                                  \
            *reinterpret_cast<float4*>(b_ + 3 * RPP * LDK) = rb3;                                  \
        }                                                                                          \
    }

    f32x16 acc[T::TM][T::TN];
    typedef float f32x4_t __attribute__((ext_vector_type(4)));
    f32x4_t acc16[2];
    const int l16 = lane & 15, q16 = lane >> 4;
    if constexpr (N16) {
        const float bv = bg[l16];
#pragma unroll
        for (int i = 0; i < 2; ++i)
#pragma unroll
            for (int r = 0; r < 4; ++r) acc16[i][r] = bv;
    } else {
#pragma unroll
    for (int j = 0; j < T::TN; ++j) {
        const float bv = bg[wn * T::TN * 32 + j * 32 + li];
#pragma unroll
        for (int i = 0; i < T::TM; ++i)
#pragma unroll
            for (int r = 0; r < 16; ++r) acc[i][j][r] = bv;
    }
    }

    int q0 = 0, q1 = p.nchunks;
    if constexpr (KS == 3) {
        if (p.cin_log2 >= 5) {
            const FilterRows fr = valid_filter_rows(mtile * BM, min(mtile * BM + BM, p.M) - 1, p.Hout, p.Wout, p.Hin, STRIDE, p.pad_t, p.rate);
            const int per_row = 3 << (p.cin_log2 - 5);
            q0 = __builtin_amdgcn_readfirstlane(fr.ky0 * per_row);
            q1 = __builtin_amdgcn_readfirstlane((fr.ky0 + fr.nky) * per_row);
        }
    }
    DAVO_LOAD_CHUNK(q0)
    DAVO_STORE_CHUNK(0)
    __syncthreads();

#define DAVO_COMPUTE16(buf_)                                                                       \
    {                                                                                              \
        const float* a = As + (buf_) * BM * LDK + (wm * 32 + l16) * LDK + 4 * q16;                 \
        const float* b = Bs + (buf_) * BN * LDK + l16 * LDK + 4 * q16;                             \
        _Pragma("unroll") for (int g = 0; g < 2; ++g) {                                            \
            const float4 fb = *reinterpret_cast<const float4*>(b + g * 16);                        \
            _Pragma("unroll") for (int i = 0; i < 2; ++i) {                                        \
                const float4 fa = *reinterpret_cast<const float4*>(a + i * 16 * LDK + g * 16);     \
                acc16[i] = __builtin_amdgcn_mfma_f32_16x16x4f32(fa.x, fb.x, acc16[i], 0, 0, 0);    \
                acc16[i] = __builtin_amdgcn_mfma_f32_16x16x4f32(fa.y, fb.y, acc16[i], 0, 0, 0);    \
                acc16[i] = __builtin_amdgcn_mfma_f32_16x16x4f32(fa.z, fb.z, acc16[i], 0, 0, 0);    \
                acc16[i] = __builtin_amdgcn_mfma_f32_16x16x4f32(fa.w, fb.w, acc16[i], 0, 0, 0);    \
            }                                                                                      \
        }                                                                                          \
    }
#define DAVO_COMPUTE(buf_)                                                                         \
    if constexpr (N16) DAVO_COMPUTE16(buf_) else                                                   \
    {                                                                                              \
        const float* a = As + (buf_) * BM * LDK + (wm * T::TM * 32 + li) * LDK + 4 * lh;           \
        const float* b = Bs + (buf_) * BN * LDK + (wn * T::TN * 32 + li) * LDK + 4 * lh;           \
        _Pragma("unroll") for (int g = 0; g < 4; ++g) {                                            \
            float4 fa[T::TM], fb[T::TN];                                                           \
            _Pragma("unroll") for (int i = 0; i < T::TM; ++i)                                      \
                fa[i] = *reinterpret_cast<const float4*>(a + i * 32 * LDK + g * 8);                \
            _Pragma("unroll") for (int j = 0; j < T::TN; ++j)                                      \
                fb[j] = *reinterpret_cast<const float4*>(b + j * 32 * LDK + g * 8);                \
            DAVO_MFMA_TILE(fa[i_], fb[j_])                                                         \
        }                                                                                          \
    }

#define DAVO_FRAG0(buf_)                                                                           \
    {                                                                                              \
        const float* a = As + (buf_) * BM * LDK + (wm * T::TM * 32 + li) * LDK + 4 * lh;           \
        const float* b = Bs + (buf_) * BN * LDK + (wn * T::TN * 32 + li) * LDK + 4 * lh;           \
        _Pragma("unroll") for (int i = 0; i < T::TM; ++i) pf_a[i] = *reinterpret_cast<const float4*>(a + i * 32 * LDK); \
        _Pragma("unroll") for (int j = 0; j < T::TN; ++j) pf_b[j] = *reinterpret_cast<const float4*>(b + j * 32 * LDK); \
    }
#define DAVO_COMPUTE_PF(buf_) DAVO_COMPUTE_PF_G(buf_, 0, 4)
#define DAVO_COMPUTE_PF_G(buf_, G0_, G1_)                                                           \
    {                                                                                              \
        const float* a = As + (buf_) * BM * LDK + (wm * T::TM * 32 + li) * LDK + 4 * lh;           \
        const float* b = Bs + (buf_) * BN * LDK + (wn * T::TN * 32 + li) * LDK + 4 * lh;           \
        float4 fa[2][T::TM], fb[2][T::TN];                                                         \
        _Pragma("unroll") for (int i = 0; i < T::TM; ++i) fa[0][i] = pf_a[i];                      \
        _Pragma("unroll") for (int j = 0; j < T::TN; ++j) fb[0][j] = pf_b[j];                      \
        _Pragma("unroll") for (int g = (G0_); g < (G1_); ++g) {                                    \
             \
            if (DAVO_F32_FRAG_AHEAD && g + 1 < 4) {                                                \
                _Pragma("unroll") for (int i = 0; i < T::TM; ++i)                                  \
                    fa[(g + 1) & 1][i] = *reinterpret_cast<const float4*>(a + i * 32 * LDK + (g + 1) * 8); \
                _Pragma("unroll") for (int j = 0; j < T::TN; ++j)                                  \
                    fb[(g + 1) & 1][j] = *reinterpret_cast<const float4*>(b + j * 32 * LDK + (g + 1) * 8); \
                __builtin_amdgcn_sched_barrier(0);                                                 \
            }                                                                                      \
            if (!DAVO_F32_FRAG_AHEAD && g > 0) {                                                   \
                _Pragma("unroll") for (int i = 0; i < T::TM; ++i)                                  \
                    fa[g & 1][i] = *reinterpret_cast<const float4*>(a + i * 32 * LDK + g * 8);     \
                _Pragma("unroll") for (int j = 0; j < T::TN; ++j)                                  \
                    fb[g & 1][j] = *reinterpret_cast<const float4*>(b + j * 32 * LDK + g * 8);     \
            }                                                                                      \
            DAVO_MFMA_TILE(fa[g & 1][i_], fb[g & 1][j_])                                           \
            if (DAVO_F32_FRAG_AHEAD) __builtin_amdgcn_sched_barrier(0);                            \
        }                                                                                          \
    }
    float4 pf_a[T::TM], pf_b[T::TN];

    constexpr bool EARLY_STORE = DAVO_F32_EARLY_STORE && BN >= DAVO_F32_EARLY_STORE_MIN_BN;
    if constexpr (EARLY_STORE) {
        int q = q0;
        if (q + 1 < q1) DAVO_LOAD_CHUNK_R(q + 1, sa0, sa1, sa2, sa3, sb0, sb1, sb2, sb3)
#define DAVO_EARLY_STEP(buf_, RS_, RL_)                                                             \
        {                                                                                          \
            if (DAVO_F32_FRAG0) { DAVO_FRAG0(buf_) __builtin_amdgcn_sched_barrier(0); }            \
            DAVO_STORE_CHUNK_R((buf_) ^ 1, RS_)                         \
            __builtin_amdgcn_sched_barrier(0);                                                     \
            if (q + 2 < q1) DAVO_LOAD_CHUNK_R(q + 2, RL_)               \
            __builtin_amdgcn_sched_barrier(0);                                                     \
            DAVO_PRIO_UP(DAVO_MMPRIO);                                                             \
            if (DAVO_F32_FRAG0) DAVO_COMPUTE_PF(buf_) else DAVO_COMPUTE(buf_)                      \
            DAVO_PRIO_DOWN(DAVO_MMPRIO);                                                           \
            __builtin_amdgcn_sched_barrier(0);                                                     \
            if (!DAVO_F32_ABLATE_BARRIER) __syncthreads();                                         \
            ++q;                                                                                   \
        }
#define DAVO_SET_S sa0, sa1, sa2, sa3, sb0, sb1, sb2, sb3
#define DAVO_SET_R ra0, ra1, ra2, ra3, rb0, rb1, rb2, rb3
        while (q + 2 < q1) {
            DAVO_EARLY_STEP(0, DAVO_SET_S, DAVO_SET_R)
            DAVO_EARLY_STEP(1, DAVO_SET_R, DAVO_SET_S)
        }
        if (q + 1 < q1) {
            DAVO_EARLY_STEP(0, DAVO_SET_S, DAVO_SET_R)
            DAVO_COMPUTE(1)
        } else {
            DAVO_COMPUTE(0)
        }
#undef DAVO_EARLY_STEP
#undef DAVO_SET_S
#undef DAVO_SET_R
    } else {
    for (int q = q0; q + 1 < q1; ++q) {
        const int buf = (q - q0) & 1;
        DAVO_LOAD_CHUNK(q + 1)
        __builtin_amdgcn_sched_barrier(0);
        DAVO_PRIO_UP(DAVO_MMPRIO);
        DAVO_COMPUTE(buf)
        DAVO_PRIO_DOWN(DAVO_MMPRIO);
        __builtin_amdgcn_sched_barrier(0);
        DAVO_STORE_CHUNK(buf ^ 1)
        if (!DAVO_F32_ABLATE_BARRIER) __syncthreads();
    }
    DAVO_COMPUTE((q1 - 1 - q0) & 1)
    }

#if DAVO_F32_ACC_AGPR
    if constexpr (!N16) {
#pragma unroll
        for (int i = 0; i < T::TM; ++i)
#pragma unroll
            for (int j = 0; j < T::TN; ++j) asm volatile("s_nop 15\n\ts_nop 3" : "+a"(acc[i][j]));
    }
#endif
    if constexpr (N16) {
        const int n = ntile * BN + l16;
#pragma unroll
        for (int i = 0; i < 2; ++i)
#pragma unroll
            for (int r = 0; r < 4; ++r) {
                const int m = mtile * BM + wm * 32 + i * 16 + 4 * q16 + r;
                float v = acc16[i][r];
                if (p.relu) v = fmaxf(v, 0.f);
                if (n < p.Cout && m < p.M) yg[(long)m * p.y_ld + n] = v;
            }
        return;
    }
    if (p.pose_w) {
        const int row0 = mtile * BM;
        const int img0 = row0 / p.pose_P;
        const int split_row = (img0 + 1) * p.pose_P - row0;
        float q[6] = {0.f, 0.f, 0.f, 0.f, 0.f, 0.f};
#pragma unroll
        for (int j = 0; j < T::TN; ++j) {
            const int n = ntile * BN + wn * T::TN * 32 + j * 32 + li;
            const bool n_ok = n < p.Cout;
            const float* wp = p.pose_w + ((long)grp * p.Cout + (n_ok ? n : 0)) * 3;
            const float w0 = n_ok ? wp[0] : 0.f, w1 = n_ok ? wp[1] : 0.f, w2 = n_ok ? wp[2] : 0.f;
            float s0 = 0.f, s1 = 0.f;
#pragma unroll
            for (int i = 0; i < T::TM; ++i)
#pragma unroll
                for (int r = 0; r < 16; ++r) {
                    const int row = wm * T::TM * 32 + i * 32 + (r & 3) + 8 * (r >> 2) + 4 * lh;
                    float v = fmaxf(acc[i][j][r], 0.f);
                    if (row0 + row >= p.M) v = 0.f;
                    if (row < split_row) s0 += v; else s1 += v;
                }
            q[0] += s0 * w0; q[1] += s0 * w1; q[2] += s0 * w2;
            q[3] += s1 * w0; q[4] += s1 * w1; q[5] += s1 * w2;
        }
#pragma unroll
        for (int k = 0; k < 6; ++k)
#pragma unroll
            for (int o = 32; o > 0; o >>= 1) q[k] += __shfl_down(q[k], o, 64);
        __syncthreads();
        float* red = smem;
        if (lane == 0)
#pragma unroll
            for (int k = 0; k < 6; ++k) red[wid * 6 + k] = q[k];
        __syncthreads();
        constexpr int UNITS = BN >= 32 ? BN / 32 : 1;
        if (tid < 6 * UNITS) {
            const int unit = tid / 6, k = tid - unit * 6;
            float t = 0.f;
            if (unit == 0)
                for (int w = 0; w < T::WAVES; ++w) t += red[w * 6 + k];
            p.pose_partial[(((long)grp * p.pose_mt + mtile) * 8 + ntile * UNITS + unit) * 6 + k] = t;
        }
        return;
    }
    if (DAVO_F32_FAST_EPILOGUE && (mtile + 1) * BM <= p.M && (ntile + 1) * BN <= p.Cout) {
        float* __restrict__ tbase = yg + (long)mtile * BM * p.y_ld + ntile * BN;
        const unsigned ld = (unsigned)p.y_ld;
        const bool relu = p.relu != 0;
#pragma unroll
        for (int i = 0; i < T::TM; ++i)
#pragma unroll
            for (int r = 0; r < 16; ++r) {
                const unsigned roff = (unsigned)(wm * T::TM * 32 + i * 32 + (r & 3) + 8 * (r >> 2) + 4 * lh) * ld + (unsigned)(wn * T::TN * 32 + li);
#pragma unroll
                for (int j = 0; j < T::TN; ++j) {
                    float v = acc[i][j][r];
                    if (relu) v = fmaxf(v, 0.f);
                    tbase[roff + j * 32] = v;
                }
            }
        return;
    }
#pragma unroll
    for (int j = 0; j < T::TN; ++j) {
        const int ncol = wn * T::TN * 32 + j * 32 + li;
        const int n = ntile * BN + ncol;
        const bool n_ok = n < p.Cout;
#pragma unroll
        for (int i = 0; i < T::TM; ++i)
#pragma unroll
            for (int r = 0; r < 16; ++r) {
                const int row = wm * T::TM * 32 + i * 32 + (r & 3) + 8 * (r >> 2) + 4 * lh;
                const int m = mtile * BM + row;
                float v = acc[i][j][r];
                if (p.relu) v = fmaxf(v, 0.f);
                if (n_ok && m < p.M) yg[(long)m * p.y_ld + n] = v;
            }
    }
}

template <int KS, int STRIDE, int BN, int LAYER>
__global__ __launch_bounds__(256, 2) void conv_igemm_f32(ConvParams p) {
    conv_igemm_f32_body<KS, STRIDE, BN, LAYER>(p, blockIdx.x, gridDim.x, blockIdx.y);
}

template <int KS, int STRIDE, int LAYER>
__global__ __launch_bounds__(512, 1) void conv_igemm_f32_n256(ConvParams p) {
    conv_igemm_f32_body<KS, STRIDE, 256, LAYER>(p, blockIdx.x, gridDim.x, blockIdx.y);
}

template <int KS, int STRIDE, int RBN, int LAYER>
__global__ __launch_bounds__(256, 2) void conv_igemm_f32_mainrem(ConvParams pm, ConvParams pr, int n_main, int n_rem, int groups) {
    const int b = blockIdx.x, nm = groups * n_main;
    if (b < nm) conv_igemm_f32_body<KS, STRIDE, 128, LAYER>(pm, b % n_main, n_main, b / n_main);
    else conv_igemm_f32_body<KS, STRIDE, RBN, LAYER>(pr, (b - nm) % n_rem, n_rem, (b - nm) / n_rem);
}

#undef DAVO_ADDR_A
#undef DAVO_LOAD_CHUNK
#undef DAVO_LOAD_CHUNK_R
#undef DAVO_STORE_CHUNK_R
#undef DAVO_STORE_CHUNK
#undef DAVO_COMPUTE
#undef DAVO_COMPUTE16
#undef DAVO_FRAG0
#undef DAVO_COMPUTE_PF
#undef DAVO_COMPUTE_PF_G

}
```

davo_amd/csrc/ctx.h:

```cpp
#pragma once
#include <hip/hip_runtime.h>

#include <cstdarg>
#include <cstdint>
#include <cstdio>
#include <deque>
#include <map>
#include <string>
#include <vector>

#include "../../include/davo_hip.h"
#include "params.h"
#include "range_book.h"

namespace davo {

static_assert(RECORD_WORDS == RANGE_WORDS, "range_book.h sizes a ticket's copy of its record");

struct HostTensor {
    std::vector<float> data;
    std::vector<int64_t> shape;
    float* dev = nullptr;
};

struct ConvLayer {
    const char* label;
    int KS, stride, rate;
    int cin, cin_log2, cout;
    int BN, npad, kpad, nchunks, groups;
    float* d_w = nullptr;
    float* d_b = nullptr;
    int cb_log2 = 0, tpc_log2 = 0, cpb = 0, nchunks_h = 0, npad_h = 0, tile_h = 0;
    float wscale = 1.f;
    uint8_t* d_wh = nullptr;
    float* d_bh = nullptr;
};

struct ProfEntry {
    std::string name;
    int launches = 0;
    double total_ms = 0.0;
    std::vector<std::pair<hipEvent_t, hipEvent_t>> pending;
    std::vector<float> dur_ms, period_ms;
};
constexpr size_t PROF_SAMPLES_CAP = 8192;

constexpr int MAX_INFLIGHT = 4;
struct Slot {
    hipStream_t stream = nullptr;
    float *d_partial = nullptr, *d_tab = nullptr, *d_packed = nullptr, *d_pose_partial = nullptr;
    float* d_act[7] = {nullptr, nullptr, nullptr, nullptr, nullptr, nullptr, nullptr};
    float *d_se = nullptr, *d_se_scale = nullptr, *d_se_partial = nullptr;
    unsigned* d_counters = nullptr;
};

struct InputSet {
    void *img = nullptr, *flow = nullptr, *seg = nullptr, *depth = nullptr;
    Inputs view() const { return Inputs{img, flow, seg, depth}; }
};

constexpr int SK_TILE_COUNTERS = 256;

constexpr int STREAM_POSES = 8;
struct StreamJob {
    int B;
    float* pose_out;
    int pr;
    bool ticketed;
    unsigned seq;
};

struct Run {
    int slot = 0;
    hipStream_t stream = nullptr;
    unsigned* range = nullptr;
    bool zero_record = false;
    SnapArgs snap{};
    int pairs = PAIRS_BOTH;
    int precision = 1, impl = 0;
};
struct RunResult {
    bool h3 = false;
    bool f32_fallback = false;
};

struct Comm;

}

struct davo_ctx {
    int device = 0, H = 0, W = 0, max_batch = 0;
    std::vector<davo::Slot> slots;
    int inflight = 1, next_slot = 0;
    int dev_cus = 256;
    int ncu = 256;
    bool cu_partition = false;
    hipStream_t user_stream = nullptr;
    bool opt_fuse_pose = true;
    int opt_fuse_pack = -1;
    bool opt_patch_cnv2 = true;
    bool opt_patch_cnv3 = true;
    bool opt_merge_rem = true;
    int opt_fold_tails = -1;
    int opt_wave128 = 2;
    bool opt_deep_ring = true;
    int opt_merge_order = -1;
    int opt_skip_order = 1;
    std::map<std::vector<int>, int*> tile_orders;
    bool opt_tile_208x128 = false;
    bool opt_merge_cnv4 = false;
    bool opt_share_taps = true;
    bool opt_f32_n256 = false;
    int opt_merge_rem_f32 = 1;
    bool opt_f32_n16 = true;
    bool opt_fold_fixup = false;
    int xcd_rr = -1;
    bool opt_split_k = true;
    float* d_splitk = nullptr;
    size_t splitk_floats = 0;
    float* d_pose_tiles = nullptr;
    size_t pose_tiles_floats = 0;
    bool cnv7_valid = true;
    davo::Variant v{};
    int posenn_se = 0;
    bool forward_seen = false;
    int impl = 0;
    int precision = 1;
    bool packed_h_ready = false;
    int weight_channel_spread_log2 = 0;
    std::string weight_channel_spread_layer;
    std::string err;
    std::map<std::string, davo::HostTensor> weights;
    std::vector<std::string> needed;
    bool packed_ready = false;
    bool pred_ready = false;
    davo::ConvLayer L[7];
    float *d_wpred = nullptr, *d_bpred = nullptr;
    uint8_t* d_w1patch = nullptr;
    uint8_t* d_w2patch = nullptr;
    float *d_w1patch_f32 = nullptr, *d_w2patch_f32 = nullptr, *d_w3patch_f32 = nullptr;
    bool opt_patch_f32 = true;
    uint8_t* d_w3patch = nullptr;
    int H1, W1, H2, W2, H3, W3;
    float* d_zeros = nullptr;
    size_t act_floats_per_img[7];
    int act_ch[7];
    int pairs = davo::PAIRS_BOTH;
    int last_slot = 0;
    int last_B = 0;
    int last_pairs = davo::PAIRS_BOTH;
    int last_precision = 0;
    int packed_ld = 8;
    bool packed_valid = true;
    davo::Inputs last_in{};
    int last_plan[7][2] = {};
    int last_split[7] = {};
    davo::InputSet host_set;
    void* s_pose = nullptr;
    float* h_sync_pose = nullptr;
    hipStream_t copy_stream = nullptr;
    std::vector<hipEvent_t> copy_done;
    int act_shift[7] = {0, 0, 0, 0, 0, 0, 0};
    unsigned* d_range_base = nullptr;
    bool opt_auto_range = true;
    bool opt_stable_inputs = false;
    davo::RangeBook book;
    davo::InputSet snap_sets[davo::RANGE_RING];
    hipStream_t read_stream = nullptr;
    unsigned* h_range = nullptr;
    unsigned* h_range_dev = nullptr;
    float range_seen[6] = {0.f, 0.f, 0.f, 0.f, 0.f, 0.f};
    std::string range_report;
    long long n_recalibrations = 0, n_f32_batches = 0, n_reissued = 0;
    int host_chunk = 8;
    bool fx_on = false;
    float* d_fx = nullptr;
    int fx_cap = 0;
    davo::InputSet stream_sets[davo::MAX_INFLIGHT];
    hipEvent_t st_copied[davo::STREAM_POSES] = {};
    bool copy_tracked[davo::STREAM_POSES] = {};
    float *d_pose_ring[davo::STREAM_POSES] = {}, *h_pose_ring[davo::STREAM_POSES] = {};
    hipEvent_t pose_done[davo::STREAM_POSES] = {};
    std::deque<davo::StreamJob> jobs;
    unsigned long long n_submitted = 0;
    float* d_reissue_pose = nullptr;
    bool prof = false;
    bool prof_dominant_only = false;
    int prof_stride = 1, prof_tick = 0;
    std::vector<davo::ProfEntry> prof_entries;
    std::vector<hipEvent_t> event_pool;
    davo::Comm* comm = nullptr;
};

namespace davo {

inline int fail(davo_ctx* c, int code, const char* fmt, ...) {
    char buf[1024];
    va_list ap;
    va_start(ap, fmt);
    vsnprintf(buf, sizeof buf, fmt, ap);
    va_end(ap);
    if (c) c->err = buf;
    return code;
}

#define HIP_TRY(c, expr)                                                                       \
    do {                                                                                       \
        hipError_t e_ = (expr);                                                                \
        if (e_ != hipSuccess)                                                                  \
            return ::davo::fail(c, DAVO_ERR_HIP, "%s failed: %s (%s:%d)", #expr, hipGetErrorString(e_), \
                                __FILE__, __LINE__);                                           \
    } while (0)

inline void same_pad(int in, int k, int stride, int rate, int* out, int* before) {
    const int o = (in + stride - 1) / stride;
    const int keff = (k - 1) * rate + 1;
    int total = (o - 1) * stride + keff - in;
    if (total < 0) total = 0;
    *out = o;
    *before = total / 2;
}

struct PlaneBytes { size_t img, flow, seg, depth; };
inline PlaneBytes plane_bytes(const davo_ctx* c) {
    const size_t HW = (size_t)c->H * c->W;
    return PlaneBytes{HW * 9, HW * 8 * sizeof(float), HW * 3 * sizeof(float), HW * 3 * sizeof(float)};
}
inline bool needs_depth(const davo_ctx* c) { return att_desc_depth(c->v.att_source); }

inline int ilog2_exact(int v) {
    int l = 0;
    while ((1 << l) < v) ++l;
    return (1 << l) == v ? l : -1;
}

inline hipStream_t slot_stream(const davo_ctx* c, int i) { return (c->user_stream && i == 0) ? c->user_stream : c->slots[i].stream; }
inline Run make_run(const davo_ctx* c, int i) {
    return Run{i, slot_stream(c, i), c->d_range_base, false, SnapArgs{}, c->pairs, c->precision, c->impl};
}
inline hipStream_t last_stream(const davo_ctx* c) { return slot_stream(c, c->last_slot); }
inline const Slot& last_workspace(const davo_ctx* c) { return c->slots[c->last_slot]; }

struct ProfScope {
    davo_ctx* c;
    hipStream_t s;
    ProfEntry* e = nullptr;
    hipEvent_t a = nullptr, b = nullptr;
    ProfScope(davo_ctx* ctx, hipStream_t stream, const char* name);
    ~ProfScope();
};
int prof_collect(davo_ctx* c);
int sync_all_slots(davo_ctx* c);

void init_layer(ConvLayer& L, const char* label, int KS, int stride, int rate, int cin, int cout, int groups);
std::vector<std::string> needed_names(const Variant& v, int posenn_se = 0);
const char* se_weight_name(int att_source, int k);
bool is_dense_weight(const std::string& name);
bool expected_shape(const davo_ctx* c, const std::string& name, std::vector<int64_t>* sh);
int upload(davo_ctx* c, const std::vector<float>& host, float** dev);
int build_packed_weights(davo_ctx* c);
int build_pred_weights(davo_ctx* c);
int build_packed_weights_h3(davo_ctx* c);
int missing_weights(davo_ctx* c, std::string* names);
float weight_prescale(const float* w, size_t n);
void pack_conv_weights(const float* w_tf, int KS, int cin_tf, int cout, const int* chmap, int cin_packed,
                       int npad, int kpad, float* out);
void pack_conv_weights_h3(const float* w_tf, int KS, int cin_tf, int cout, const int* chmap, int cin_packed,
                          int cb_log2, int tpc_log2, int cpb, int nchunks, float scale, _Float16* out);
inline void split_f16(float v, _Float16* hi, _Float16* lo) {
    const _Float16 h = (_Float16)v;
    *hi = h;
    *lo = (_Float16)(v - (float)h);
}

int forward_device(davo_ctx* c, const Run& run, int B, const Inputs& in, void* d_pose, RunResult* res = nullptr);

int zero_now(davo_ctx* c, void* p, size_t bytes);
int alloc_input_set(davo_ctx* c, InputSet* s, bool zero_unread);

int ensure_ring(davo_ctx* c, bool snapshots);
int wait_record(davo_ctx* c, const unsigned* m, unsigned seq, hipStream_t s, unsigned raw[RANGE_WORDS]);
int judge_record(davo_ctx* c, const unsigned* raw , const int* shifts);
int recover_batch(davo_ctx* c, const Reissue& b);
int judge_front(davo_ctx* c);
int judge_all(davo_ctx* c);
int freeze_pending_and_reset_ring(davo_ctx* c);
int calibrate_on(davo_ctx* c, int B, const Inputs& in, void* d_pose, int sel);
int ticket_reserve(davo_ctx* c);
int ticket_begin(davo_ctx* c, Run* run, int B, const Inputs& in, Ticket* t, bool own_inputs = false);
int ticket_end(davo_ctx* c, int rc, const RunResult& res, Ticket t, void* d_pose, float* h_pose = nullptr);

void comm_release(davo_ctx* c);

}
```

davo_amd/csrc/forward.hip:

```cpp
#include <cmath>
#include <cstdlib>
#include <cstring>

#include "ctx.h"
#include "launch.h"
#include "plan.h"

namespace davo {

ProfScope::ProfScope(davo_ctx* ctx, hipStream_t stream, const char* name) : c(ctx), s(stream) {
    if (!c->prof) return;
    if (c->prof_dominant_only) {
        if (strcmp(name, "cnv6") != 0) return;
        if (c->prof_tick++ % c->prof_stride != 0) return;
    }
    for (auto& pe : c->prof_entries)
        if (pe.name == name) { e = &pe; break; }
    if (!e) {
        c->prof_entries.emplace_back();
        e = &c->prof_entries.back();
        e->name = name;
    }
    auto get = [&]() {
        hipEvent_t ev = nullptr;
        if (!c->event_pool.empty()) { ev = c->event_pool.back(); c->event_pool.pop_back(); }
        else if (hipEventCreate(&ev) != hipSuccess) ev = nullptr;
        return ev;
    };
    a = get(); b = get();
    if (a) (void)hipEventRecord(a, s);
}

ProfScope::~ProfScope() {
    if (!e) return;
    if (b) (void)hipEventRecord(b, s);
    if (a && b) e->pending.emplace_back(a, b);
    else {
        if (a) c->event_pool.push_back(a);
        if (b) c->event_pool.push_back(b);
    }
}

int sync_all_slots(davo_ctx* c) {
    for (auto& s : c->slots) HIP_TRY(c, hipStreamSynchronize(s.stream));
    if (c->user_stream) HIP_TRY(c, hipStreamSynchronize(c->user_stream));
    return DAVO_OK;
}

int prof_collect(davo_ctx* c) {
    { int rc = sync_all_slots(c); if (rc) return rc; }
    for (auto& pe : c->prof_entries) {
        hipEvent_t prev_start = nullptr;
        for (auto& ab : pe.pending) {
            float ms = 0.f, gap = -1.f;
            if (hipEventElapsedTime(&ms, ab.first, ab.second) == hipSuccess) {
                pe.total_ms += ms;
                pe.launches += 1;
                if (prev_start && hipEventElapsedTime(&gap, prev_start, ab.first) != hipSuccess) gap = -1.f;
                if (pe.dur_ms.size() < PROF_SAMPLES_CAP) { pe.dur_ms.push_back(ms); pe.period_ms.push_back(gap); }
            }
            if (prev_start) c->event_pool.push_back(prev_start);
            prev_start = ab.first;
            c->event_pool.push_back(ab.second);
        }
        if (prev_start) c->event_pool.push_back(prev_start);
        pe.pending.clear();
    }
    return DAVO_OK;
}

namespace {

constexpr int MAX_WEIGHT_CHANNEL_SPREAD_LOG2 = 14;
constexpr int FOLD_EXCITE_MAX_BATCH = 2;
constexpr int FUSE_PACK_MAX_BATCH = 0;

const int* tile_order_for(davo_ctx* c, int li, int kind, int bm, int mtile0, int mtiles, int ntiles_n, int M,
                          int Hout, int Wout, int Hin, int stride, int pad_t, int rate) {
    if (!c->opt_skip_order) return nullptr;
    const std::vector<int> key = {li, kind, bm, mtile0, mtiles, ntiles_n, M, Hout, Wout};
    auto it = c->tile_orders.find(key);
    if (it != c->tile_orders.end()) return it->second;
    const int nt = mtiles * ntiles_n;
    std::vector<int> cost(nt), order(nt);
    bool uniform = true;
    for (int t = 0; t < nt; ++t) {
        const int m0 = (mtile0 + t / ntiles_n) * bm, m1 = std::min(m0 + bm, M) - 1;
        cost[t] = valid_filter_rows(m0, m1, Hout, Wout, Hin, stride, pad_t, rate).nky;
        uniform = uniform && cost[t] == cost[0];
    }
    int* dev = nullptr;
    if (!uniform) {
        const int q = nt >> 3, r = nt & 7;
        for (int x = 0; x < 8; ++x) {
            const int start = x < r ? x * (q + 1) : r * (q + 1) + (x - r) * q, len = q + (x < r ? 1 : 0);
            int w = start;
            for (int want = 3; want >= 1; --want)
                for (int t = start; t < start + len; ++t)
                    if (cost[t] == want) order[w++] = t;
        }
        if (hipMalloc(reinterpret_cast<void**>(&dev), nt * sizeof(int)) != hipSuccess ||
            hipMemcpy(dev, order.data(), nt * sizeof(int), hipMemcpyHostToDevice) != hipSuccess) {
            if (dev) (void)hipFree(dev);
            dev = nullptr;
            (void)hipGetLastError();
        }
    }
    c->tile_orders[key] = dev;
    return dev;
}

int slot_scratch(davo_ctx* c, const Run& run, float** buf, size_t* floats, size_t need, float** region, size_t extra_bytes = 0) {
    if (need > *floats) {
        if (*buf) { int rs = sync_all_slots(c); if (rs) return rs; HIP_TRY(c, hipFree(*buf)); *buf = nullptr; }
        HIP_TRY(c, hipMalloc(reinterpret_cast<void**>(buf), need * sizeof(float) * MAX_INFLIGHT + extra_bytes));
        *floats = need;
    }
    *region = *buf + (size_t)run.slot * *floats;
    return DAVO_OK;
}

int run_conv_layer(davo_ctx* c, const Run& run, int li, const float* x, int x_ld, int Hin, int Win, float* y, int y_ld, int NB, bool fuse_pose = false, int* pose_mt = nullptr) {
    const ConvLayer& L = c->L[li];
    ConvParams p{};
    int Ho, Wo, pt, pl;
    same_pad(Hin, L.KS, L.stride, L.rate, &Ho, &pt);
    same_pad(Win, L.KS, L.stride, L.rate, &Wo, &pl);
    p.x = x; p.w = L.d_w; p.bias = L.d_b; p.y = y; p.zeros = c->d_zeros;
    p.Hin = Hin; p.Win = Win; p.Hout = Ho; p.Wout = Wo;
    p.cin_log2 = L.cin_log2; p.x_ld = x_ld; p.x_coff = 0; p.y_ld = y_ld; p.y_coff = 0;
    p.Cout = L.cout; p.pad_t = pt; p.pad_l = pl; p.rate = L.rate;
    p.M = NB * Ho * Wo; p.nchunks = L.nchunks; p.Kpad = L.kpad; p.ntaps = L.KS * L.KS;
    p.ntiles_n = L.npad / L.BN; p.relu = 1;
    if (L.groups == 2) {
        p.g_x_coff = L.cin; p.g_y_coff = L.cout;
        p.g_w = (long)L.npad * L.kpad; p.g_bias = L.npad;
    }
    const int mtiles = (p.M + BM - 1) / BM;
    std::vector<Launch> plan = plan_layer(mtiles, L.npad, L.groups, c->ncu);
    if (li == 0 && L.cout <= 16 && c->opt_f32_n16) plan = {{0, mtiles, 16}};
    if (fuse_pose) {
        { int rs = slot_scratch(c, run, &c->d_pose_tiles, &c->pose_tiles_floats, (size_t)L.groups * mtiles * 8 * 6, &p.pose_partial); if (rs) return rs; }
        p.pose_w = c->d_wpred;
        p.pose_P = Ho * Wo; p.pose_mt = mtiles;
        if (pose_mt) *pose_mt = mtiles;
    }
    c->last_plan[li][0] = c->last_plan[li][1] = 0; c->last_split[li] = 1;
    auto order_for = [&](const Launch& l, int ntn) {
        return (L.KS == 3 && L.cin_log2 >= 5) ? tile_order_for(c, li, 0, BM, l.mtile0, l.mtiles, ntn, p.M, Ho, Wo, Hin, L.stride, pt, L.rate) : nullptr;
    };
    if (c->opt_f32_n256 && (li == 4 || li == 5) && L.npad == 256 && L.groups == 1 && !fuse_pose && mtiles >= c->ncu) {
        const int main_m = (mtiles / c->ncu) * c->ncu;
        ConvParams pm = p;
        pm.mtile0 = 0; pm.ntiles_n = 1;
        pm.tile_order = tile_order_for(c, li, 2, BM, 0, main_m, 1, p.M, Ho, Wo, Hin, L.stride, pt, L.rate);
        {
            ProfScope ps(c, run.stream, L.label);
            HIP_TRY(c, launch_layer_n256(li, pm, dim3(main_m, 1), run.stream));
        }
        c->last_plan[li][0] = main_m * 1000 + 256;
        if (main_m < mtiles) {
            ConvParams pr = p;
            pr.mtile0 = main_m; pr.ntiles_n = L.npad / 64;
            pr.tile_order = tile_order_for(c, li, 0, BM, main_m, mtiles - main_m, pr.ntiles_n, p.M, Ho, Wo, Hin, L.stride, pt, L.rate);
            const std::string label = std::string(L.label) + ".rem";
            ProfScope ps(c, run.stream, label.c_str());
            HIP_TRY(c, launch_layer(li, 64, pr, dim3((mtiles - main_m) * pr.ntiles_n, 1), run.stream));
            c->last_plan[li][1] = (mtiles - main_m) * 1000 + 64;
        }
        return DAVO_OK;
    }
    if (c->opt_merge_rem_f32 && li >= 3 && (li <= 5 || c->opt_merge_rem_f32 > 1) && plan.size() == 2 && plan[0].BN == 128 && (plan[1].BN == 32 || plan[1].BN == 64)) {
        ConvParams pm = p, pr = p;
        pm.mtile0 = plan[0].mtile0; pm.ntiles_n = L.npad / 128; pm.tile_order = order_for(plan[0], pm.ntiles_n);
        pr.mtile0 = plan[1].mtile0; pr.ntiles_n = L.npad / plan[1].BN; pr.tile_order = order_for(plan[1], pr.ntiles_n);
        const int n_main = plan[0].mtiles * pm.ntiles_n, n_rem = plan[1].mtiles * pr.ntiles_n;
        if (n_main % 8 == 0 && (L.groups == 1 || n_rem % 8 == 0)) {
            ProfScope ps(c, run.stream, L.label);
            HIP_TRY(c, launch_layer_mainrem(li, plan[1].BN, pm, pr, n_main, n_rem, L.groups, run.stream));
            c->last_plan[li][0] = (plan[0].mtiles + plan[1].mtiles) * 1000 + 128;
            return DAVO_OK;
        }
    }
    for (size_t i = 0; i < plan.size(); ++i) {
        p.mtile0 = plan[i].mtile0;
        p.ntiles_n = plan[i].BN == 16 ? 1 : L.npad / plan[i].BN;
        dim3 grid(plan[i].mtiles * p.ntiles_n, L.groups);
        p.tile_order = (L.KS == 3 && L.cin_log2 >= 5) ? tile_order_for(c, li, 0, BM, plan[i].mtile0, plan[i].mtiles, p.ntiles_n, p.M, Ho, Wo, Hin, L.stride, pt, L.rate) : nullptr;
        const std::string label = i == 0 ? std::string(L.label) : std::string(L.label) + ".rem";
        ProfScope ps(c, run.stream, label.c_str());
        HIP_TRY(c, launch_layer(li, plan[i].BN, p, grid, run.stream));
        c->last_plan[li][i] = plan[i].mtiles * 1000 + plan[i].BN;
    }
    return DAVO_OK;
}

int run_conv_layer_h3(davo_ctx* c, const Run& run, int li, const void* x, int x_ch, int Hin, int Win, void* y, int y_ld,
                      bool y_f32, int NB, bool fuse_pose = false, int* pose_bm = nullptr, int* pose_mt = nullptr,
                      int* pose_ntn = nullptr, float* pose_out = nullptr) {
    const ConvLayer& L = c->L[li];
    ConvParamsH p{};
    int Ho, Wo, pt, pl;
    same_pad(Hin, L.KS, L.stride, L.rate, &Ho, &pt);
    same_pad(Win, L.KS, L.stride, L.rate, &Wo, &pl);
    p.x = static_cast<const uint8_t*>(x); p.w = L.d_wh; p.bias = L.d_bh; p.y = static_cast<uint8_t*>(y);
    p.zeros = reinterpret_cast<const uint8_t*>(c->d_zeros);
    p.Hin = Hin; p.Win = Win; p.Hout = Ho; p.Wout = Wo;
    p.x_pix_bytes = (long)x_ch * 4; p.x_boff = 0; p.x_pix_log2 = ilog2_exact(x_ch * 4);
    p.cb_log2 = L.cb_log2; p.tpc_log2 = L.tpc_log2; p.cpb = L.cpb; p.nchunks = L.nchunks_h;
    p.w_row_bytes = (long)L.nchunks_h * 128;
    p.y_mode = y_f32 ? 0 : 1; p.y_ld = y_ld; p.y_coff = 0; p.Cout = L.cout;
    p.pad_t = pt; p.pad_l = pl; p.rate = L.rate;
    p.M = NB * Ho * Wo; p.ntaps = L.KS * L.KS; p.mtile0 = 0; p.relu = 1;
    p.Mtot = p.M; p.xs = c->opt_share_taps ? 1 : 0;
    {
        const int sin = li == 0 ? 0 : c->act_shift[li - 1], sout = li == 6 ? 0 : c->act_shift[li];
        p.out_scale = ldexpf(1.0f / L.wscale, sout - sin);
        p.bias_scale = ldexpf(L.wscale, sin);
        p.range = run.range ? run.range + li : nullptr;
    }
    if (L.groups == 2) {
        p.g_x_boff = L.cin * 4; p.g_y_coff = L.cout;
        p.g_w = (long)L.npad_h * p.w_row_bytes; p.g_bias = L.npad_h;
    }
    if (const char* e = tuning_env("DAVO_DBG")) p.dbg = atoi(e);
    const bool allow_208 = (li >= 4 && L.npad_h == 256) || (li == 3 && L.npad_h == 128 && c->opt_tile_208x128);
    const double others_scale = (c->opt_wave128 && (li == 4 || li == 5) && L.npad_h == 256 && L.groups == 1 && !fuse_pose) ? 0.955 : 1.0;
    std::vector<LaunchH> plan = plan_layer_h3(p.M, L.npad_h, L.groups, L.tile_h, allow_208, c->ncu, others_scale);
    if (fuse_pose) {
        const int P = Ho * Wo;
        const int best = plan_single_tile_h3(p.M, L.npad_h, L.groups, P, L.tile_h, allow_208, c->ncu);
        if (best < 0) return fail(c, DAVO_ERR_INVALID, "no tile fits the fused pose head");
        plan = {{0, p.M, best}};
        const TileShape ts = tile_shape(best);
        const int mt = (p.M + ts.bm - 1) / ts.bm, ntn = L.npad_h / ts.bn;
        size_t debug_bytes = 0;
#ifdef DAVO_POSE_DEBUG
        debug_bytes = (size_t)L.groups * mt * ntn * 512 * 20 * sizeof(float);
#endif
        { int rs = slot_scratch(c, run, &c->d_pose_tiles, &c->pose_tiles_floats, (size_t)L.groups * mt * ntn * 6, &p.pose_partial, debug_bytes); if (rs) return rs; }
        p.y_mode = 2; p.pose_w = c->d_wpred;
        p.pose_P = P; p.pose_mt = mt;
        if (pose_out) {
            p.pose_counter = c->slots[run.slot].d_counters; p.pose_bias = c->d_bpred; p.pose_out = pose_out;
            p.pose_NB = NB; p.pose_bm = ts.bm; p.pose_total = L.groups * mt * ntn; p.pose_sel = run.pairs;
        }
        if (pose_bm) *pose_bm = ts.bm;
        if (pose_mt) *pose_mt = mt;
        if (pose_ntn) *pose_ntn = ntn;
    }
    c->last_plan[li][0] = c->last_plan[li][1] = 0; c->last_split[li] = 1;
    const long t256 = (p.M + 255) / 256;
    const bool rounds_ok = t256 >= c->ncu && (double)((t256 + c->ncu - 1) / c->ncu) * c->ncu <= 1.12 * (double)t256;
    if ((c->opt_wave128 >= 3 || (c->opt_wave128 >= 2 && rounds_ok)) && li == 3 && !fuse_pose && L.groups == 1 && L.npad_h == 128 && L.tile_h < 0 &&
        p.M >= 256 * c->ncu) {
        ConvParamsH pw = p;
        pw.ntiles_n = 1; pw.mtile0 = 0;
        if (layer_h3w128_supported(pw)) {
            {
                ProfScope ps(c, run.stream, L.label);
                HIP_TRY(c, launch_layer_h3w128(pw, run.stream));
            }
            c->last_plan[li][0] = ((p.M + 127) / 128) * 1000 + TILE_256x128;
            return DAVO_OK;
        }
    }
    if (c->opt_merge_cnv4 && c->opt_merge_rem && li == 3 && !fuse_pose && L.npad_h == 128 && L.groups == 1 && c->ncu == 256 && L.tile_h < 0 &&
        plan.size() == 1 && plan[0].tile == TILE_128x128) {
        const int rows1 = (p.M / 256 / c->ncu) * c->ncu * 256;
        const int rem = p.M - rows1, n_rem = (rem + 127) / 128;
        if (rows1 > 0 && rem > 0 && rem % 128 == 0 && n_rem % 64 == 0 && n_rem <= 256)
            plan = {{0, rows1, TILE_256x128}, {rows1, rem, TILE_128x128}};
    }
    const bool merge_256 = plan.size() == 2 && plan[0].tile == TILE_256x256 && plan[1].tile == TILE_128x128 && L.npad_h == 256;
    const bool merge_128 = li == 3 && plan.size() == 2 && plan[0].tile == TILE_256x128 && plan[1].tile == TILE_128x128 && L.npad_h == 128;
    if (c->opt_merge_rem && !fuse_pose && (merge_256 || merge_128) && L.groups == 1 && c->ncu == 256 && !tuning_env("DAVO_NO_MERGE")) {
        ConvParamsH pm = p, pr = p;
        const int rem_ntn = L.npad_h / 128;
        pm.ntiles_n = 1; pm.mtile0 = 0; pm.M = plan[0].rows;
        pr.ntiles_n = rem_ntn; pr.mtile0 = plan[1].row0 / 128; pr.M = plan[1].row0 + plan[1].rows;
        const int n_main = plan[0].rows / 256, n_rem = ((plan[1].rows + 127) / 128) * rem_ntn;
        const bool own_launch = c->opt_wave128 && merge_256 && layer_h3w_supported(li, pm);
        if (!own_launch && layer_h3_mainrem_supported(li, pm, n_main, n_rem)) {
            pm.tile_order = c->opt_skip_order >= 2 ? tile_order_for(c, li, 1, 256, 0, n_main, 1, pm.M, Ho, Wo, Hin, L.stride, pt, L.rate) : nullptr;
            const int order = c->opt_merge_order >= 0 ? c->opt_merge_order : (pm.tile_order ? 2 : 0);
            {
                ProfScope ps(c, run.stream, L.label);
                HIP_TRY(c, launch_layer_h3_mainrem(li, pm, n_main, pr, n_rem, order, run.stream));
            }
            c->last_plan[li][0] = ((plan[0].rows + plan[1].rows + 127) / 128) * 1000 + 7;
            return DAVO_OK;
        }
    }
    if (c->opt_split_k && !fuse_pose && (li == 4 || li == 5) && L.groups == 1 && plan.size() == 1 && p.y_mode == 1 && L.cout % 32 == 0 &&
        !is_208(plan[0].tile)) {
        const TileShape ts = tile_shape(plan[0].tile);
        const int mtiles = (p.M + ts.bm - 1) / ts.bm, ntn = L.npad_h / ts.bn;
        const long tiles = (long)mtiles * ntn;
        auto fits = [&](int S) { return L.nchunks_h % (S * L.cpb) == 0 && ((L.nchunks_h / S) % 3) == 0; };
        const int per_cu = ts.lds * 2 <= 160 * 1024 ? 2 : 1;
        const int S = (fits(4) && tiles * 4 <= (long)per_cu * c->ncu && tiles * 2 <= c->ncu) ? 4 : (fits(2) && tiles * 2 <= c->ncu ? 2 : 1);
        if (S > 1) {
            float* part = nullptr;
            { int rs = slot_scratch(c, run, &c->d_splitk, &c->splitk_floats, (size_t)p.M * S * L.cout, &part); if (rs) return rs; }
            ConvParamsH ps = p;
            ps.nchunks = L.nchunks_h / S;
            ps.g_x_boff = (L.cin / S) * 4; ps.g_w = (long)ps.nchunks * 128; ps.g_bias = L.npad_h; ps.g_y_coff = L.cout;
            ps.y = reinterpret_cast<uint8_t*>(part); ps.y_mode = 0; ps.y_ld = S * L.cout; ps.relu = 0; ps.range = nullptr;
            ps.ntiles_n = ntn; ps.mtile0 = 0;
            dim3 grid(mtiles * ntn, S);
            ps.deep = c->opt_deep_ring && tiles * S <= c->ncu;
            c->last_plan[li][0] = ((p.M + 127) / 128) * 1000 + plan[0].tile; c->last_split[li] = S;
            bool fold = c->opt_fold_fixup && S <= 4 && grid.x % 8 == 0 && (int)grid.x <= SK_TILE_COUNTERS && c->ncu == c->dev_cus && !c->cu_partition &&
                        !c->user_stream;
            if (fold && c->xcd_rr < 0) {
                int ok = 0;
                HIP_TRY(c, xcd_round_robin_probe(run.stream, &ok));
                c->xcd_rr = ok;
            }
            fold = fold && c->xcd_rr > 0;
            if (fold) {
                ps.sk_counter = c->slots[run.slot].d_counters + 1 + c->max_batch;
                ps.sk_y = p.y; ps.sk_range = p.range; ps.sk_parts = S; ps.sk_relu = 1;
            }
            ProfScope pscope(c, run.stream, L.label);
            HIP_TRY(c, launch_layer_h3(li, plan[0].tile, ps, grid, run.stream));
            if (!fold) HIP_TRY(c, launch_splitk_fixup(part, p.M, L.cout, S, 1, p.y, p.range, run.stream));
            return DAVO_OK;
        }
    }
    for (size_t i = 0; i < plan.size() && i < 2; ++i) {
        const TileShape ts = tile_shape(plan[i].tile);
        p.ntiles_n = L.npad_h / ts.bn;
        p.mtile0 = plan[i].row0 / ts.bm;
        const int full_m = p.M;
        p.M = plan[i].row0 + plan[i].rows;
        const int mtiles = (plan[i].rows + ts.bm - 1) / ts.bm;
        dim3 grid(mtiles * p.ntiles_n, L.groups);
        p.deep = c->opt_deep_ring && plan.size() == 1 && (long)grid.x * grid.y <= c->ncu;
        c->last_plan[li][i] = ((plan[i].rows + 127) / 128) * 1000 + plan[i].tile;
        const std::string label = i == 0 ? std::string(L.label) : std::string(L.label) + ".rem";
        {
            ProfScope ps(c, run.stream, label.c_str());
            bool done = false;
            if (c->opt_wave128 && L.groups == 1 && !fuse_pose) {
                if (plan[i].tile == TILE_256x256 && layer_h3w_supported(li, p)) {
                    HIP_TRY(c, launch_layer_h3w(li, p, grid, run.stream));
                    done = true;
                } else if (c->opt_wave128 >= 2 && i == 1 && plan.size() == 2 && plan[0].tile == TILE_256x256 && plan[1].tile == TILE_128x128 &&
                           L.npad_h == 256 && plan[1].row0 % 256 == 0 && plan[1].rows % 256 == 0) {
                    ConvParamsH pr = p;
                    pr.ntiles_n = 4; pr.mtile0 = plan[1].row0 / 256;
                    const hipError_t e = launch_layer_h3w64(li, pr, run.stream);
                    if (e == hipSuccess) done = true;
                    else if (e != hipErrorNotSupported) HIP_TRY(c, e);
                }
            }
            if (!done) HIP_TRY(c, launch_layer_h3(li, plan[i].tile, p, grid, run.stream));
        }
        p.M = full_m;
    }
    return DAVO_OK;
}

struct PatchLayer { int tw, th, per_cu, plan_id; };
constexpr PatchLayer PATCH_LAYERS[3] = {
    {cp1::TW, cp1::TH, 3, 99},
    {cp2::TW, cp2::TH, 2, 98},
    {cp3::TW, cp3::TH, 3, 97}};

int run_patch_layer(davo_ctx* c, const Run& run, int li, bool f32, const void* x, void* y, int NB, bool fused = false, const Inputs& in = Inputs{}) {
    const ConvLayer& L = c->L[li];
    const PatchLayer& t = PATCH_LAYERS[li];
    const uint8_t* const w_h3[3] = {c->d_w1patch, c->d_w2patch, c->d_w3patch};
    const float* const w_f32[3] = {c->d_w1patch_f32, c->d_w2patch_f32, c->d_w3patch_f32};
    const int Hin[3] = {c->H, c->H1, c->H2}, Win[3] = {c->W, c->W1, c->W2};
    ConvPatchParams p{};
    same_pad(Hin[li], L.KS, L.stride, L.rate, &p.Ho, &p.pad_t);
    same_pad(Win[li], L.KS, L.stride, L.rate, &p.Wo, &p.pad_l);
    p.x = static_cast<const uint8_t*>(x); p.w = f32 ? reinterpret_cast<const uint8_t*>(w_f32[li]) : w_h3[li];
    p.bias = f32 ? L.d_b : L.d_bh; p.y = static_cast<uint8_t*>(y);
    p.zeros = reinterpret_cast<const uint8_t*>(c->d_zeros);
    p.H = Hin[li]; p.W = Win[li];
    p.tiles_x = (p.Wo + t.tw - 1) / t.tw; p.tiles_y = (p.Ho + t.th - 1) / t.th;
    p.ntiles = NB * p.tiles_x * p.tiles_y;
    if (!f32) {
        const int sin = li == 0 ? 0 : c->act_shift[li - 1];
        p.out_scale = ldexpf(1.0f / L.wscale, c->act_shift[li] - sin);
        p.bias_scale = ldexpf(L.wscale, sin);
        p.range = run.range ? run.range + li : nullptr;
        if (const char* e = tuning_env("DAVO_PDBG")) p.dbg = atoi(e);
        if (li == 0) {
            p.img = static_cast<const uint8_t*>(in.img); p.flow = static_cast<const float*>(in.flow);
            p.seg = static_cast<const float*>(in.seg); p.tab = c->slots[run.slot].d_tab; p.v = c->v; p.sel = run.pairs;
        }
    }
    c->last_plan[li][0] = ((NB * p.Ho * p.Wo + 127) / 128) * 1000 + t.plan_id; c->last_plan[li][1] = 0; c->last_split[li] = 1;
    const int nblk = p.ntiles < t.per_cu * c->ncu ? p.ntiles : t.per_cu * c->ncu;
    ProfScope ps(c, run.stream, L.label);
    HIP_TRY(c, launch_patch_layer(li, f32, fused, p, nblk, run.stream));
    return DAVO_OK;
}

int run_direct(davo_ctx* c, const Run& run, const char* label, const float* x, int N, int Hin, int Win, int cin, int x_ld,
               int x_coff, const std::string& wname, const std::string& bname, int KS, int cout, int stride,
               int rate, float* y, int y_ld, int y_coff) {
    int Ho, Wo, pt, pl;
    same_pad(Hin, KS, stride, rate, &Ho, &pt);
    same_pad(Win, KS, stride, rate, &Wo, &pl);
    for (const std::string* n : {&wname, &bname}) {
        HostTensor& t = c->weights.at(*n);
        if (!t.dev) { int rc = upload(c, t.data, &t.dev); if (rc) return rc; }
    }
    ProfScope ps(c, run.stream, label);
    HIP_TRY(c, launch_conv_direct(x, N, Hin, Win, cin, x_ld, x_coff, c->weights.at(wname).dev, KS, cout,
                                  c->weights.at(bname).dev, stride, rate, pt, pl, Ho, Wo, 1, y, y_ld, y_coff, run.stream));
    return DAVO_OK;
}

int run_posenn_se(davo_ctx* c, const Run& run, bool h3, const void* x, int NB) {
    static const char* const heads[2] = {"rotation", "translation"};
    static const char* const parts[4] = {"bottleneck_fc/kernel", "bottleneck_fc/bias", "recover_fc/kernel", "recover_fc/bias"};
    const float* w[8];
    for (int h = 0; h < 2; ++h)
        for (int k = 0; k < 4; ++k) {
            const auto it = c->weights.find(std::string("pose_exp_net/pose/") + heads[h] + "/cnv5_se_attention/" + parts[k]);
            if (it == c->weights.end() || !it->second.dev) return fail(c, DAVO_ERR_NOT_READY, "feature-attention weights not loaded");
            w[h * 4 + k] = it->second.dev;
        }
    const Slot& ws = c->slots[run.slot];
    if (!ws.d_se || !ws.d_se_scale || !ws.d_se_partial) return fail(c, DAVO_ERR_INVALID, "internal: no feature-attention workspace");
    const int P = c->H2 * c->W2;
    {
        ProfScope ps(c, run.stream, "se5_squeeze");
        HIP_TRY(c, launch_se5_squeeze(h3, x, NB, P, ws.d_se_partial, run.stream));
    }
    {
        ProfScope ps(c, run.stream, "se5_excite");
        HIP_TRY(c, launch_se5_excite(ws.d_se_partial, NB, P, h3 ? ldexpf(1.0f, -c->act_shift[4]) : 1.0f, w, ws.d_se_scale, run.stream));
    }
    ProfScope ps(c, run.stream, "se5_scale");
    HIP_TRY(c, launch_se5_scale(h3, x, ws.d_se_scale, NB, P, ws.d_se, (h3 && run.range) ? run.range + RANGE_SE : nullptr, run.stream));
    return DAVO_OK;
}

}

int forward_device(davo_ctx* c, const Run& run, int B, const Inputs& in, void* d_pose, RunResult* res) {
    const int sel = run.pairs;
    if (sel != PAIRS_SRC0 && sel != PAIRS_SRC1 && sel != PAIRS_BOTH) return fail(c, DAVO_ERR_INVALID, "internal: pair selection %d", sel);
    if (B < 1 || B > c->max_batch) return fail(c, DAVO_ERR_INVALID, "batch %d outside [1,%d]", B, c->max_batch);
    if (!in.img || !in.flow || !in.seg || !d_pose) return fail(c, DAVO_ERR_INVALID, "null device pointer");
    if (needs_depth(c) && (!in.depth || ((uintptr_t)in.depth & 15)))
        return fail(c, DAVO_ERR_INVALID, "this variant reads depth planes: a 16-byte aligned device pointer is required");
    {
        std::string names;
        if (missing_weights(c, &names)) return fail(c, DAVO_ERR_NOT_READY, "weights not loaded: %s", names.c_str());
    }
    HIP_TRY(c, hipSetDevice(c->device));
    c->forward_seen = true;
    c->last_slot = run.slot;
    if (!c->pred_ready) { int rc = build_pred_weights(c); if (rc) return rc; }
    bool h3 = run.impl == 0 && run.precision == 1, f32_fallback = false;
    if (h3 && !c->packed_h_ready) { int rc = build_packed_weights_h3(c); if (rc) return rc; }
    if (h3 && c->weight_channel_spread_log2 > MAX_WEIGHT_CHANNEL_SPREAD_LOG2) {
        if (!c->opt_auto_range)
            return fail(c, DAVO_ERR_RANGE, "`%s': per-input-channel weight norms span 2^%d (> 2^%d): the f16x3 storage cannot hold every channel "
                        "float32-grade - davo_set_precision(ctx, 0), or leave \"auto_range\" on", c->weight_channel_spread_layer.c_str(),
                        c->weight_channel_spread_log2, MAX_WEIGHT_CHANNEL_SPREAD_LOG2);
        h3 = false;
        f32_fallback = true;
        char note[256];
        snprintf(note, sizeof note, "float32 kernels: per-input-channel weight norms of `%s' span 2^%d (> 2^%d)",
                 c->weight_channel_spread_layer.c_str(), c->weight_channel_spread_log2, MAX_WEIGHT_CHANNEL_SPREAD_LOG2);
        c->range_report = note;
    }
    if (!h3 && run.impl == 0 && !c->packed_ready) { int rc = build_packed_weights(c); if (rc) return rc; }
    unsigned* const range_reset = (h3 && run.zero_record) ? run.range : nullptr;

    const int H = c->H, W = c->W, HW = H * W, NB = pairs_per_window(sel) * B;
    const Variant& v = c->v;
    const Slot& ws = c->slots[run.slot];
    hipStream_t s = run.stream;
    const uint8_t* const d_img = static_cast<const uint8_t*>(in.img);
    const float* const d_flow = static_cast<const float*>(in.flow);
    const float* const d_seg = static_cast<const float*>(in.seg);
    auto wdev = [&](const char* n) -> const float* {
        auto it = c->weights.find(n);
        return it == c->weights.end() ? nullptr : it->second.dev;
    };
    const bool class_table = att_class_table(v.att_source);
    const bool fold_excite = (v.att_source == 1 || class_table) &&
                             (c->opt_fold_tails >= 1 || (c->opt_fold_tails < 0 && B <= FOLD_EXCITE_MAX_BATCH));
    const bool fold_pose = c->opt_fold_tails == 1;
    const float* se_w1 = wdev(se_weight_name(v.att_source, 0));
    const float* se_b1 = wdev(se_weight_name(v.att_source, 1));
    const float* se_w2 = wdev(se_weight_name(v.att_source, 2));
    const float* se_b2 = wdev(se_weight_name(v.att_source, 3));
    if (needs_depth(c)) {
        ProfScope ps(c, run.stream, "se_depth_squeeze");
        HIP_TRY(c, launch_se_depth_squeeze(fold_excite, static_cast<const float*>(in.depth), B, HW, v, reinterpret_cast<unsigned*>(ws.d_partial),
                                           ws.d_counters + 1, se_w1, se_b1, se_w2, se_b2, ws.d_tab, range_reset, sel, s));
    } else if (class_table) {
        ProfScope ps(c, run.stream, "se_class_squeeze");
        HIP_TRY(c, launch_se_class_squeeze(fold_excite, d_img, d_flow, d_seg, B, H, W, v, reinterpret_cast<unsigned*>(ws.d_partial),
                                           ws.d_counters + 1, se_w1, se_b1, se_w2, se_b2, ws.d_tab, range_reset, sel, s));
    } else if (fold_excite) {
        ProfScope ps(c, run.stream, "se_squeeze_partial");
        HIP_TRY(c, launch_se_squeeze_excite(d_flow, B, HW, v, ws.d_partial, ws.d_counters + 1,
                                            se_w1, se_b1, se_w2, se_b2,
                                            wdev("pose_exp_net/pose_exp_net/seg_channel_weight/weight"), ws.d_tab, range_reset, sel, s));
    } else if (v.att_source == 1) {
        ProfScope ps(c, run.stream, "se_squeeze_partial");
        HIP_TRY(c, launch_se_squeeze(d_flow, B, HW, v, ws.d_partial, sel, s));
    }
    if (!fold_excite) {
        ProfScope ps(c, run.stream, "se_excite");
        HIP_TRY(c, launch_se_excite(ws.d_partial, B, HW, v, se_w1, se_b1, se_w2, se_b2,
                                    wdev("pose_exp_net/pose_exp_net/seg_channel_weight/weight"), ws.d_tab, range_reset, sel, s));
    }
    const char* fe = tuning_env("DAVO_FUSE_PACK");
    const char* pe = tuning_env("DAVO_CNV1_PATCH");
    const bool fuse_env = (fe && atoi(fe) == 1) || c->opt_fuse_pack == 1 || (c->opt_fuse_pack < 0 && B <= FUSE_PACK_MAX_BATCH);
    const bool patch1 = !(pe && atoi(pe) == 0);
    const bool fused = h3 && patch1 && fuse_env;
    c->packed_valid = !fused;
    c->last_in = in;
    c->packed_ld = run.impl == 0 ? 8 : 10;
    if (!fused) {
        ProfScope ps(c, run.stream, "mask_pack");
        HIP_TRY(c, launch_mask_pack(h3 ? 16 : (run.impl == 0 ? 8 : 10), d_img, d_flow, d_seg, ws.d_tab, v, B, H, W, ws.d_packed, sel, s));
    }
    const int c6 = v.cnv6_out;
    float* const* a = ws.d_act;
    int rc;
    bool pose_fused = false;
    int pose_bm = 0, pose_mt = 0, pose_ntn = 0;
    c->cnv7_valid = true;
    if (h3) {
        if (patch1) { if ((rc = run_patch_layer(c, run, 0, false, ws.d_packed, a[0], NB, fused, in))) return rc; }
        else if ((rc = run_conv_layer_h3(c, run, 0, ws.d_packed, 8, H, W, a[0], 16, false, NB))) return rc;
        const char* p2e = tuning_env("DAVO_CNV2_PATCH");
        if (c->opt_patch_cnv2 && c->L[1].tile_h < 0 && !(p2e && atoi(p2e) == 0)) { if ((rc = run_patch_layer(c, run, 1, false, a[0], a[1], NB))) return rc; }
        else if ((rc = run_conv_layer_h3(c, run, 1, a[0], 16, c->H1, c->W1, a[1], 32, false, NB))) return rc;
        const char* p3e = tuning_env("DAVO_CNV3_PATCH");
        if (c->opt_patch_cnv3 && c->L[2].tile_h < 0 && !(p3e && atoi(p3e) == 0)) { if ((rc = run_patch_layer(c, run, 2, false, a[1], a[2], NB))) return rc; }
        else if ((rc = run_conv_layer_h3(c, run, 2, a[1], 32, c->H2, c->W2, a[2], 64, false, NB))) return rc;
        if ((rc = run_conv_layer_h3(c, run, 3, a[2], 64, c->H2, c->W2, a[3], 128, false, NB))) return rc;
        if ((rc = run_conv_layer_h3(c, run, 4, a[3], 128, c->H2, c->W2, a[4], 256, false, NB))) return rc;
        if (c->posenn_se) {
            if ((rc = run_posenn_se(c, run, true, a[4], NB))) return rc;
            if ((rc = run_conv_layer_h3(c, run, 5, ws.d_se, 512, c->H2, c->W2, a[5], 2 * c6, false, NB))) return rc;
        } else if ((rc = run_conv_layer_h3(c, run, 5, a[4], 256, c->H2, c->W2, a[5], 2 * c6, false, NB))) return rc;
        pose_fused = c->opt_fuse_pose && c->H3 * c->W3 >= 128;
        if ((rc = run_conv_layer_h3(c, run, 6, a[5], 2 * c6, c->H2, c->W2, a[6], 512, true, NB, pose_fused, &pose_bm, &pose_mt, &pose_ntn,
                                    fold_pose ? static_cast<float*>(d_pose) : nullptr))) return rc;
        c->cnv7_valid = !pose_fused;
    } else if (run.impl == 0) {
        if (c->opt_patch_f32 && c->d_w1patch_f32 && c->packed_ld == 8) { if ((rc = run_patch_layer(c, run, 0, true, ws.d_packed, a[0], NB))) return rc; }
        else if ((rc = run_conv_layer(c, run, 0, ws.d_packed, 8, H, W, a[0], 16, NB))) return rc;
        if (c->opt_patch_f32 && c->d_w2patch_f32) { if ((rc = run_patch_layer(c, run, 1, true, a[0], a[1], NB))) return rc; }
        else if ((rc = run_conv_layer(c, run, 1, a[0], 16, c->H1, c->W1, a[1], 32, NB))) return rc;
        if (c->opt_patch_f32 && c->d_w3patch_f32) { if ((rc = run_patch_layer(c, run, 2, true, a[1], a[2], NB))) return rc; }
        else if ((rc = run_conv_layer(c, run, 2, a[1], 32, c->H2, c->W2, a[2], 64, NB))) return rc;
        if ((rc = run_conv_layer(c, run, 3, a[2], 64, c->H2, c->W2, a[3], 128, NB))) return rc;
        if ((rc = run_conv_layer(c, run, 4, a[3], 128, c->H2, c->W2, a[4], 256, NB))) return rc;
        if (c->posenn_se) {
            if ((rc = run_posenn_se(c, run, false, a[4], NB))) return rc;
            if ((rc = run_conv_layer(c, run, 5, ws.d_se, 512, c->H2, c->W2, a[5], 2 * c6, NB))) return rc;
        } else if ((rc = run_conv_layer(c, run, 5, a[4], 256, c->H2, c->W2, a[5], 2 * c6, NB))) return rc;
        pose_fused = c->opt_fuse_pose && c->H3 * c->W3 >= 128 && c->L[6].npad == 256;
        pose_bm = 128; pose_ntn = 8;
        if ((rc = run_conv_layer(c, run, 6, a[5], 2 * c6, c->H2, c->W2, a[6], 512, NB, pose_fused, &pose_mt))) return rc;
        c->cnv7_valid = !pose_fused;
    } else {
        const std::string P = "pose_exp_net/";
        const int c10 = 2 * v.cin_per_frame;
        if (v.cin_per_frame != 5) return fail(c, DAVO_ERR_INVALID, "impl 1 supports the 10-channel (v1) input only");
        if ((rc = run_direct(c, run, "cnv1", ws.d_packed, NB, H, W, c10, 10, 0, P + "cnv1/weights", P + "cnv1/biases", 7, 16, 2, 1, a[0], 16, 0))) return rc;
        if ((rc = run_direct(c, run, "cnv2", a[0], NB, c->H1, c->W1, 16, 16, 0, P + "cnv2/weights", P + "cnv2/biases", 5, 32, 2, 1, a[1], 32, 0))) return rc;
        if ((rc = run_direct(c, run, "cnv3", a[1], NB, c->H2, c->W2, 32, 32, 0, P + "cnv3/weights", P + "cnv3/biases", 3, 64, 1, 2, a[2], 64, 0))) return rc;
        if ((rc = run_direct(c, run, "cnv4", a[2], NB, c->H2, c->W2, 64, 64, 0, P + "cnv4/weights", P + "cnv4/biases", 3, 128, 1, 4, a[3], 128, 0))) return rc;
        if ((rc = run_direct(c, run, "cnv5", a[3], NB, c->H2, c->W2, 128, 128, 0, P + "cnv5/weights", P + "cnv5/biases", 3, 256, 1, 8, a[4], 256, 0))) return rc;
        if (c->posenn_se && (rc = run_posenn_se(c, run, false, a[4], NB))) return rc;
        const char* heads[2] = {"rotation", "translation"};
        for (int h = 0; h < 2; ++h) {
            const std::string hp = P + "pose/" + heads[h] + "/";
            const float* x6 = c->posenn_se ? ws.d_se : a[4];
            if ((rc = run_direct(c, run, "cnv6", x6, NB, c->H2, c->W2, 256, c->posenn_se ? 512 : 256, c->posenn_se ? h * 256 : 0, hp + "cnv6/weights", hp + "cnv6/biases", 3, c6, 1, 2, a[5], 2 * c6, h * c6))) return rc;
            if ((rc = run_direct(c, run, "cnv7", a[5], NB, c->H2, c->W2, c6, 2 * c6, h * c6, hp + "cnv7/weights", hp + "cnv7/biases", 3, 256, 2, 1, a[6], 512, h * 256))) return rc;
        }
    }
    bool snap_done = false;
    if (!(pose_fused && fold_pose)) {
        ProfScope ps(c, run.stream, "pose_head");
        if (pose_fused) {
            HIP_TRY(c, launch_pose_from_tiles(c->d_pose_tiles + (size_t)run.slot * c->pose_tiles_floats, NB, c->H3 * c->W3, pose_bm,
                                              pose_mt, pose_ntn, c->d_bpred, static_cast<float*>(d_pose), h3 ? run.snap : SnapArgs{}, sel, s));
            snap_done = true;
        } else {
            HIP_TRY(c, launch_pose_head(a[6], NB, c->H3 * c->W3, c->d_wpred, c->d_bpred, ws.d_pose_partial, static_cast<float*>(d_pose), sel, s));
        }
    }
    if (h3 && run.snap.record && !snap_done) HIP_TRY(c, launch_range_guard_snapshot(run.snap, s));
    c->last_B = B;
    c->last_pairs = sel;
    c->last_precision = h3 ? 1 : 0;
    if (res) *res = RunResult{h3, f32_fallback};
    return DAVO_OK;
}

}
```

davo_amd/csrc/launch_f32.hip:

```cpp
#include "conv_igemm.h"
#include "launch.h"

namespace davo {
namespace {

template <int KS, int STRIDE, int BN, int LAYER>
hipError_t launch_conv_t(const ConvParams& p, dim3 grid, hipStream_t s) {
    auto kern = conv_igemm_f32<KS, STRIDE, BN, LAYER>;
    hipError_t e = ensure_dynamic_lds(reinterpret_cast<const void*>(kern), Tile<BN>::LDS_BYTES);
    if (e != hipSuccess) return e;
    hipLaunchKernelGGL(kern, grid, dim3(256), Tile<BN>::LDS_BYTES, s, p);
    return hipGetLastError();
}

template <int KS, int STRIDE, int LAYER>
hipError_t launch_bn(int BN, const ConvParams& p, dim3 grid, hipStream_t s) {
    switch (BN) {
        case 32: return launch_conv_t<KS, STRIDE, 32, LAYER>(p, grid, s);
        case 64: return launch_conv_t<KS, STRIDE, 64, LAYER>(p, grid, s);
        case 128: return launch_conv_t<KS, STRIDE, 128, LAYER>(p, grid, s);
    }
    return hipErrorInvalidValue;
}

template <int KS, int STRIDE, int RBN, int LAYER>
hipError_t launch_mainrem_t(const ConvParams& pm, const ConvParams& pr, int n_main, int n_rem, int groups, hipStream_t s) {
    auto kern = conv_igemm_f32_mainrem<KS, STRIDE, RBN, LAYER>;
    hipError_t e = ensure_dynamic_lds(reinterpret_cast<const void*>(kern), Tile<128>::LDS_BYTES);
    if (e != hipSuccess) return e;
    hipLaunchKernelGGL(kern, dim3((n_main + n_rem) * groups), dim3(256), Tile<128>::LDS_BYTES, s, pm, pr, n_main, n_rem, groups);
    return hipGetLastError();
}

template <int LAYER>
hipError_t launch_n256_t(const ConvParams& p, dim3 grid, hipStream_t s) {
    auto kern = conv_igemm_f32_n256<3, 1, LAYER>;
    hipError_t e = ensure_dynamic_lds(reinterpret_cast<const void*>(kern), Tile<256>::LDS_BYTES);
    if (e != hipSuccess) return e;
    hipLaunchKernelGGL(kern, grid, dim3(512), Tile<256>::LDS_BYTES, s, p);
    return hipGetLastError();
}

}

hipError_t launch_layer_n256(int layer, const ConvParams& p, dim3 grid, hipStream_t s) {
    if (layer == 4) return launch_n256_t<5>(p, grid, s);
    if (layer == 5) return launch_n256_t<6>(p, grid, s);
    return hipErrorInvalidValue;
}

hipError_t launch_layer_mainrem(int layer, int rbn, const ConvParams& pm, const ConvParams& pr, int n_main, int n_rem, int groups, hipStream_t s) {
    if (n_main < 8 || n_main % 8 || n_rem < 1 || (groups > 1 && n_rem % 8)) return hipErrorInvalidValue;
    switch (layer * 1000 + rbn) {
        case 3032: return launch_mainrem_t<3, 1, 32, 4>(pm, pr, n_main, n_rem, groups, s);
        case 3064: return launch_mainrem_t<3, 1, 64, 4>(pm, pr, n_main, n_rem, groups, s);
        case 4032: return launch_mainrem_t<3, 1, 32, 5>(pm, pr, n_main, n_rem, groups, s);
        case 4064: return launch_mainrem_t<3, 1, 64, 5>(pm, pr, n_main, n_rem, groups, s);
        case 5032: return launch_mainrem_t<3, 1, 32, 6>(pm, pr, n_main, n_rem, groups, s);
        case 5064: return launch_mainrem_t<3, 1, 64, 6>(pm, pr, n_main, n_rem, groups, s);
        case 6032: return launch_mainrem_t<3, 2, 32, 7>(pm, pr, n_main, n_rem, groups, s);
        case 6064: return launch_mainrem_t<3, 2, 64, 7>(pm, pr, n_main, n_rem, groups, s);
    }
    return hipErrorInvalidValue;
}

hipError_t launch_conv(int KS, int stride, int BN, const ConvParams& p, dim3 grid, hipStream_t s) {
    if (stride == 1) {
        switch (KS) {
            case 1: return launch_bn<1, 1, 0>(BN, p, grid, s);
            case 3: return launch_bn<3, 1, 0>(BN, p, grid, s);
            case 5: return launch_bn<5, 1, 0>(BN, p, grid, s);
            case 7: return launch_bn<7, 1, 0>(BN, p, grid, s);
        }
    } else if (stride == 2) {
        switch (KS) {
            case 1: return launch_bn<1, 2, 0>(BN, p, grid, s);
            case 3: return launch_bn<3, 2, 0>(BN, p, grid, s);
            case 5: return launch_bn<5, 2, 0>(BN, p, grid, s);
            case 7: return launch_bn<7, 2, 0>(BN, p, grid, s);
        }
    }
    return hipErrorInvalidValue;
}

hipError_t launch_layer(int layer, int BN, const ConvParams& p, dim3 grid, hipStream_t s) {
    if (layer == 0 && BN == 16) return launch_conv_t<7, 2, 16, 1>(p, grid, s);
    switch (layer) {
        case 0: return launch_bn<7, 2, 1>(BN, p, grid, s);
        case 1: return launch_bn<5, 2, 2>(BN, p, grid, s);
        case 2: return launch_bn<3, 1, 3>(BN, p, grid, s);
        case 3: return launch_bn<3, 1, 4>(BN, p, grid, s);
        case 4: return launch_bn<3, 1, 5>(BN, p, grid, s);
        case 5: return launch_bn<3, 1, 6>(BN, p, grid, s);
        case 6: return launch_bn<3, 2, 7>(BN, p, grid, s);
    }
    return hipErrorInvalidValue;
}

}
```

davo_amd/csrc/params.h:

```cpp
#pragma once
#include <stdint.h>

#ifndef DAVO_MMPRIO
#define DAVO_MMPRIO 1
#endif
#ifndef DAVO_MMPRIO_H3
#define DAVO_MMPRIO_H3 0
#endif
#define DAVO_PRIO_UP(level_) do { if ((level_) > 0) __builtin_amdgcn_s_setprio(level_); } while (0)
#define DAVO_PRIO_DOWN(level_) do { if ((level_) > 0) __builtin_amdgcn_s_setprio(0); } while (0)

namespace davo {

constexpr int NCLS = 19;
constexpr int SQ_CHUNKS = 32;
constexpr int PH_SPLIT = 8;
constexpr int SE5_C = 256, SE5_HID = 32, SE5_CHUNKS = 32;

struct Variant {
    int cin_per_frame, cnv6_out, se_act, norm_flow, abs_mode, att_source, mask_rgb, mask_info;
};

constexpr int SQ_REC = 24;
__host__ __device__ inline bool att_class_table(int a) { return a >= 4 && a <= 12; }
__host__ __device__ inline bool att_tgt_attended(int a) { return a == 3 || a == 6 || a == 8 || a == 10 || a == 12; }
__host__ __device__ inline bool att_desc_depth(int a) { return a == 11 || a == 12; }
__host__ __device__ inline bool att_desc_hist(int a) { return a == 4 || (a >= 7 && a <= 10); }
__host__ __device__ inline bool att_desc_rgb(int a) { return a == 5 || a == 6; }
__host__ __device__ inline bool att_desc_flow(int a) { return a >= 7 && a <= 10; }
__host__ __device__ inline int att_se_in(int a) { return a == 1 ? 2 : att_desc_depth(a) ? 1 : att_desc_rgb(a) ? 3 : a == 4 ? NCLS : NCLS + 2; }
__host__ __device__ inline int att_se_hidden(int a) { return (a == 4 || a == 7 || a == 8) ? NCLS : 8; }
__host__ __device__ inline int att_se_frames(int a) { return (att_tgt_attended(a) || att_desc_depth(a)) ? 3 : 2; }

constexpr int PAIRS_SRC0 = 1, PAIRS_SRC1 = 2, PAIRS_BOTH = 3;
__host__ __device__ inline int pairs_per_window(int sel) { return sel == PAIRS_BOTH ? 2 : 1; }
__host__ __device__ inline int pair_window(int n, int sel) { return sel == PAIRS_BOTH ? n >> 1 : n; }
__host__ __device__ inline int pair_source(int n, int sel) { return sel == PAIRS_BOTH ? n & 1 : sel >> 1; }
__host__ __device__ inline int pair_pose_row(int n, int sel) { return 2 * pair_window(n, sel) + pair_source(n, sel); }
__host__ __device__ inline bool pair_reads_frame(int frame, int sel) { return frame == 0 || ((sel >> (frame - 1)) & 1); }

struct FilterRows { int ky0, nky; };
__host__ __device__ inline FilterRows valid_filter_rows(int m0, int m1, int Hout, int Wout, int Hin, int stride, int pad_t, int rate) {
    FilterRows fr = {0, 3};
    const int hw = Hout * Wout;
    const int n0 = m0 / hw;
    if (m1 < m0 || m1 / hw != n0) return fr;
    const int ymin = (m0 - n0 * hw) / Wout, ymax = (m1 - n0 * hw) / Wout;
    int lo = 0, hi = 2;
    while (lo < hi && ymax * stride - pad_t + lo * rate < 0) ++lo;
    while (hi > lo && ymin * stride - pad_t + hi * rate > Hin - 1) --hi;
    fr.ky0 = lo;
    fr.nky = hi - lo + 1;
    return fr;
}
__host__ __device__ inline int h3_real_chunk(int v, int ky0, int nky) {
    const int sc = v / 3, kx = v - 3 * sc;
    const int blk = nky == 3 ? sc / 3 : (nky == 2 ? sc >> 1 : sc);
    return (blk * 3 + ky0 + (sc - blk * nky)) * 3 + kx;
}

struct ConvParams {
    const float* x;
    const float* w;
    const float* bias;
    float* y;
    const float* zeros;
    int Hin, Win, Hout, Wout;
    int cin_log2;
    int x_ld, x_coff;
    int y_ld, y_coff;
    int Cout;
    int pad_t, pad_l, rate;
    const int* tile_order;
    int M;
    int nchunks, Kpad, ntaps;
    int ntiles_n;
    int mtile0;
    int relu;
    int g_x_coff, g_y_coff;
    long g_w, g_bias;
    const float* pose_w;
    float* pose_partial;
    int pose_P, pose_mt;
};

constexpr int BM = 128;
constexpr int BK = 32;
constexpr int LDK = 36;

template <int BN> struct Tile;
template <> struct Tile<16> {
    static constexpr int WN = 1, WM = 4, TM = 1, TN = 1, NB_LOADS = 1, WAVES = 4, RPP = 32, A_LOADS = 4;
    static constexpr int LDS_BYTES = 2 * (128 + 16) * 36 * 4;
};
template <int BN> struct Tile {
    static constexpr int WAVES = BN == 256 ? 8 : 4;
    static constexpr int WN = BN == 256 ? 4 : (BN >= 64 ? 2 : 1);
    static constexpr int WM = WAVES / WN;
    static constexpr int TM = BM / WM / 32;
    static constexpr int TN = BN / WN / 32;
    static constexpr int RPP = WAVES * 8;
    static constexpr int A_LOADS = BM / RPP;
    static constexpr int NB_LOADS = BN / RPP;
    static constexpr int LDS_BYTES = 2 * (BM + BN) * LDK * 4;
};

struct ConvParamsH {
    const uint8_t* x;
    const uint8_t* w;
    const float* bias;
    uint8_t* y;
    const uint8_t* zeros;
    int Hin, Win, Hout, Wout;
    long x_pix_bytes;
    int x_pix_log2;
    int x_boff;
    int cb_log2;
    int tpc_log2;
    int cpb;
    int nchunks;
    long w_row_bytes;
    int y_mode, y_ld, y_coff, Cout;
    int pad_t, pad_l, rate;
    int M, ntaps, ntiles_n, mtile0, relu;
    const int* tile_order;
    int Mtot;
    int xs;
    int deep;
    unsigned* sk_counter;
    uint8_t* sk_y;
    unsigned* sk_range;
    int sk_parts, sk_relu;
    int g_x_boff, g_y_coff;
    long g_w, g_bias;
    float out_scale;
    float bias_scale;
    unsigned* range;
    const float* pose_w;
    float* pose_partial;
    int pose_P, pose_mt;
    unsigned* pose_counter;
    const float* pose_bias;
    float* pose_out;
    int pose_NB, pose_bm, pose_total;
    int pose_sel;
    int dbg;
};

constexpr int LDB = 144;

template <int WM, int WN, int TM, int TN, int NSTG = 2> struct TileH {
    static constexpr int THREADS = WM * WN * 64;
    static constexpr int BMH = WM * TM * 32;
    static constexpr int BNH = WN * TN * 32;
    static constexpr int A_LOADS = BMH * 8 / THREADS;
    static constexpr int B_LOADS = BNH * 8 / THREADS;
    static constexpr int ROWS_PER_PASS = THREADS / 8;
    static constexpr int LDS_BYTES = 2 * (BMH + BNH) * LDB;
#ifndef DAVO_H3_STAGES
#define DAVO_H3_STAGES 2
#endif
    static constexpr int DMA_STAGES = DAVO_H3_STAGES == 2 ? NSTG : DAVO_H3_STAGES;
    static constexpr int LDS_BYTES_DMA = DMA_STAGES * (BMH + BNH) * 128;
    static_assert(A_LOADS >= 1 && A_LOADS <= 4 && B_LOADS >= 1 && B_LOADS <= 4, "staging shape");
};

template <int WM, int WN, int TM, int TN, int NSTG, int RATE> struct TileX {
    using T = TileH<WM, WN, TM, TN, NSTG>;
    static constexpr int PR = (T::BMH + 2 * RATE + 7) / 8 * 8;
    static constexpr int NWV = WM * WN;
    static constexpr int A_SLOTS = (PR / 8 + NWV - 1) / NWV;
    static constexpr int APC = (A_SLOTS + 2) / 3;
    static constexpr int LDS_BYTES = 2 * PR * 128 + T::DMA_STAGES * T::BNH * 128 + NWV * 1024 + 128;
};

template <int W> struct TileSW {
    static constexpr int BM = 208, BN = 32 * W, THREADS = 64 * W, WAVES = W;
    static constexpr int NP = BM / 16;
    static constexpr int NC = 2;
    static constexpr int RPP = THREADS / 8;
    static constexpr int NAJ = (BM + RPP - 1) / RPP;
    static constexpr int NBJ = BN / RPP;
    static constexpr int A_SLOT = BM * 128, B_SLOT = BN * 128;
    static constexpr int DUMMY = WAVES * 1024;
    static constexpr int LDS_BYTES = 2 * (A_SLOT + B_SLOT) + DUMMY;
    static constexpr int lds_bytes(int nsa) { return nsa * A_SLOT + 2 * B_SLOT + DUMMY; }
    static_assert(NBJ == 4 && 192 + 8 * 2 == BM, "staging shape");
};
typedef TileSW<8> TileS;

namespace cp1 {
constexpr int KS = 7, TH = 8, TW = 16;
constexpr int PH = 2 * TH + KS - 2, PW = 2 * TW + KS - 2;
constexpr int UNITS = 32;
constexpr int ROWB = UNITS * 16;
constexpr int PLANE = PH * 2 * ROWB;
constexpr int STEPS = 2 * KS;
constexpr int WBYTES = STEPS * 2 * 64 * 16;
constexpr int LDS_BYTES = 2 * PLANE;
constexpr int THREADS = 256;
}

namespace cp2 {
constexpr int KS = 5, TH = 8, TW = 8;
constexpr int PH = 2 * TH + KS - 2;
constexpr int PWU = TW + 2;
constexpr int ROWB = 2 * PWU * 16;
constexpr int ROW_UNITS = 2 * PWU;
constexpr int REGION = (PH * ROWB + 255) / 256 * 256;
constexpr int NDMA = (PH * ROW_UNITS + 63) / 64;
constexpr int PATCH = 4 * REGION;
constexpr int LDS_BYTES = 2 * PATCH;
constexpr int STEPS = KS * 3;
constexpr int WBYTES = STEPS * 2 * 2 * 64 * 16;
constexpr int THREADS = 256;
static_assert(NDMA * 1024 <= REGION, "the last DMA piece stays inside its region");
}

namespace cp3 {
constexpr int RATE = 2, TH = 8, TW = 8;
constexpr int PH = TH + 2 * RATE, PW = TW + 2 * RATE;
constexpr int ROWB = PW * 16;
constexpr int REGION = PH * ROWB;
constexpr int PATCH = 8 * REGION;
constexpr int NDMA = PATCH / 1024;
constexpr int LDS_BYTES = 2 * PATCH;
constexpr int STEPS = 9;
constexpr int WBYTES = STEPS * 4 * 2 * 64 * 16;
constexpr int THREADS = 256;
static_assert(REGION % 256 == 0 && PATCH % 1024 == 0 && (2 * ROWB) % 256 == 128, "bank-conflict-free fragment reads, whole DMA pieces");
}

struct ConvPatchParams {
    const uint8_t* x;
    const uint8_t* w;
    const float* bias;
    uint8_t* y;
    const uint8_t* zeros;
    int H, W, Ho, Wo, pad_t, pad_l;
    int tiles_x, tiles_y, ntiles;
    float out_scale;
    float bias_scale;
    unsigned* range;
    const uint8_t* img;
    const float* flow;
    const float* seg;
    const float* tab;
    Variant v;
    int sel;
    int dbg;
};

constexpr int RANGE_WORDS = 12, RANGE_SNAP = 6, RANGE_SEQ = 7, RANGE_SE = 8;
__host__ __device__ inline bool range_value_fails(float vmax) {
    return !(vmax < 65504.f) || (vmax > 0.f && vmax < 0x1p-6f);
}
__device__ inline void range_note(unsigned* __restrict__ rec_layer, float vmax, bool leader) {
    if (!leader) return;
    const unsigned u = __builtin_bit_cast(unsigned, vmax);
    if (u > __atomic_load_n(rec_layer, __ATOMIC_RELAXED)) (void)__hip_atomic_fetch_max(rec_layer, u, __ATOMIC_RELAXED, __HIP_MEMORY_SCOPE_AGENT);
}
struct SnapArgs {
    unsigned* record;
    unsigned* host_mirror;
    unsigned seq;
    const uint8_t *img, *flow, *seg;
    uint8_t *s_img, *s_flow, *s_seg;
    unsigned img_vec, flow_vec_half, flow_vec, seg_vec;
    int B;
    const uint8_t* depth;
    uint8_t* s_depth;
    int se;
};

}
```

include/davo_hip.h:

```cpp
#ifndef DAVO_HIP_H
#define DAVO_HIP_H

#include <stddef.h>
#include <stdint.h>

#ifdef __cplusplus
extern "C" {
#endif

typedef struct davo_ctx davo_ctx;

typedef enum {
    DAVO_OK = 0,
    DAVO_ERR_INVALID = -1,
    DAVO_ERR_HIP = -2,
    DAVO_ERR_NOT_READY = -3,
    DAVO_ERR_NOMEM = -4,
    DAVO_ERR_RANGE = -5,
    DAVO_ERR_COMM = -6
} davo_status;

typedef struct {
    int32_t cin_per_frame;
    int32_t cnv6_out;
    int32_t se_act;
    int32_t norm_flow;
    int32_t abs_mode;
    int32_t att_source;
    int32_t mask_rgb;
    int32_t mask_info;
} davo_variant;

int davo_create(davo_ctx** out, int device, int H, int W, int max_batch, const davo_variant* v);

int davo_set_posenn_se(davo_ctx* ctx, int mode);

int davo_load_weight(davo_ctx* ctx, const char* tf_name, const float* data,
                     const int64_t* shape, int ndim);

int davo_weights_missing(davo_ctx* ctx);

int davo_forward(davo_ctx* ctx, int B, const uint8_t* img, const float* flow, const float* seg,
                 float* pose_out);

int davo_forward_depth(davo_ctx* ctx, int B, const uint8_t* img, const float* flow, const float* seg,
                       const float* depth, float* pose_out);
int davo_forward_device_depth(davo_ctx* ctx, int B, const void* d_img, const void* d_flow, const void* d_seg,
                              const void* d_depth, void* d_pose, float* elapsed_ms);
int davo_submit_depth(davo_ctx* ctx, int B, const uint8_t* img, const float* flow, const float* seg,
                      const float* depth, float* pose_out, int hold);
int davo_calibrate_depth(davo_ctx* ctx, int batch, const void* d_img, const void* d_flow, const void* d_seg,
                         const void* d_depth, int* shifts_out);

int davo_forward_device(davo_ctx* ctx, int B, const void* d_img, const void* d_flow,
                        const void* d_seg, void* d_pose, float* elapsed_ms);

int davo_submit(davo_ctx* ctx, int B, const uint8_t* img, const float* flow, const float* seg, float* pose_out, int hold);
int davo_wait(davo_ctx* ctx, int leave_pending);
int davo_pending(davo_ctx* ctx);

enum { DAVO_PAIRS_SRC0 = 1, DAVO_PAIRS_SRC1 = 2, DAVO_PAIRS_BOTH = 3 };
int davo_set_pairs(davo_ctx* ctx, int pairs);
int davo_get_pairs(const davo_ctx* ctx);

int davo_set_feature_export(davo_ctx* ctx, int on);
typedef struct {
    float* att_19;
    float* attention;
    float* masked_image;
    float* image;
    float* feat_rot;
    float* feat_trans;
} davo_feature_out;
int davo_forward_features(davo_ctx* ctx, int B, const uint8_t* img, const float* flow, const float* seg,
                          const float* depth, float* pose_out, const davo_feature_out* out);

const char* davo_last_error(const davo_ctx* ctx);
void davo_destroy(davo_ctx* ctx);

int davo_device_malloc(davo_ctx* ctx, size_t bytes, void** out);
int davo_device_free(davo_ctx* ctx, void* p);
int davo_host_alloc(int device, size_t bytes, void** out);
int davo_host_free(void* p);
int davo_host_register(int device, void* p, size_t bytes);
int davo_host_unregister(void* p);
int davo_memcpy_h2d(davo_ctx* ctx, void* dst, const void* src, size_t bytes);
int davo_memcpy_d2h(davo_ctx* ctx, void* dst, const void* src, size_t bytes);
int davo_synchronize(davo_ctx* ctx);
int davo_set_stream(davo_ctx* ctx, void* hip_stream);
int davo_set_inflight(davo_ctx* ctx, int n);

int davo_profile_enable(davo_ctx* ctx, int on);
int davo_profile_reset(davo_ctx* ctx);
int davo_profile_entry(davo_ctx* ctx, int i, char* name, int name_len, int* launches,
                       double* total_ms);
int davo_profile_samples(davo_ctx* ctx, const char* name, int which, float* out, int cap);

int davo_last_plan(davo_ctx* ctx, int layer, int launch, int* mtiles, int* bn);
int davo_last_split(davo_ctx* ctx, int layer, int* parts);

int davo_set_precision(davo_ctx* ctx, int precision);

int davo_calibrate(davo_ctx* ctx, int batch, const void* d_img, const void* d_flow, const void* d_seg, int* shifts_out);
int davo_activation_range(davo_ctx* ctx, float* max_abs, int* shifts, int reset);
int davo_set_activation_shifts(davo_ctx* ctx, const int* shifts);
int davo_reset_range_state(davo_ctx* ctx);
int davo_range_stats(davo_ctx* ctx, long long* recalibrations, long long* f32_batches, long long* reissued);
const char* davo_range_report(const davo_ctx* ctx);

int davo_set_option(davo_ctx* ctx, const char* key, int value);

#define DAVO_COMM_ID_BYTES 128
int davo_comm_preload(char* err, int err_len);
int davo_comm_unique_id(void* id_out, char* err, int err_len);
int davo_comm_init(davo_ctx* ctx, int nranks, int rank, const void* id);
int davo_comm_size(davo_ctx* ctx, int* nranks, int* rank);
int davo_allgather_poses(davo_ctx* ctx, const float* local, int n_local, int n_per_rank, float* all,
                         float* elapsed_ms);
int davo_allgather_poses_device(davo_ctx* ctx, const void* d_local, int n_per_rank, void* d_all,
                                float* elapsed_ms);
int davo_comm_allreduce(davo_ctx* ctx, double* value, int op);
int davo_comm_barrier(davo_ctx* ctx);
int davo_comm_destroy(davo_ctx* ctx);

int davo_set_impl(davo_ctx* ctx, int impl);

int davo_debug_read(davo_ctx* ctx, const char* tensor, float* host_out, size_t n_floats);

int davo_conv2d_same(int device, const float* x, int N, int H, int W, int Cin,
                     const float* w, int k, int Cout, const float* bias,
                     int stride, int rate, int relu, int precision, float* y, char* err, int err_len);

int davo_plan_layer(int M, int npad, int groups, int* rows, int* tile_bm, int* tile_bn);

int davo_tile_filter_rows(int m0, int m1, int Hout, int Wout, int Hin, int stride, int pad_t, int rate,
                          int* ky0, int* nky, int nblocks, int* chunk_map);

#ifdef __cplusplus
}
#endif
#endif
```

Before: 8975 triplets/s.

## Reorder output pixels by padding class to skip zero-padding taps in dilated convs

Adds pad-class tables that permute the output pixels of the dilated 3x3 stride-1 layers (cnv4-6), grouping pixels whose receptive fields have the same set of in-bounds taps. Each M-tile then walks only the union of its real taps, not all nine, skipping MACs on zero padding. The epilogue scatters results through the row permutation, and a load-balanced tile order spreads tiles with different tap counts across the eight block groups. The cost is an indirect row lookup, extra LDS, a scattered output store, and a fallback when sorting does not reduce the number of taps walked.

```diff
diff --git a/davo_amd/_lib.py b/davo_amd/_lib.py
--- a/davo_amd/_lib.py
+++ b/davo_amd/_lib.py
@@ -30,6 +30,7 @@
     "davo_comm_allreduce", "davo_comm_barrier", "davo_comm_destroy", "davo_plan_layer", "davo_tile_filter_rows",
     "davo_set_pairs", "davo_get_pairs",
     "davo_set_feature_export", "davo_forward_features",
+    "davo_pad_class_tables", "davo_pad_class_tile_order", "davo_plan_layer_f32",
 )
 COMM_ID_BYTES = 128
 
@@ -198,6 +199,10 @@
     ip = ctypes.POINTER(i)
     L.davo_plan_layer.argtypes = [i, i, i, ip, ip, ip]
     L.davo_tile_filter_rows.argtypes = [i] * 8 + [ip, ip, i, ip]
+    usp = ctypes.POINTER(ctypes.c_uint16)
+    L.davo_pad_class_tables.argtypes = [i] * 8 + [ip, usp]
+    L.davo_pad_class_tile_order.argtypes = [usp, i, i, i, ip]
+    L.davo_plan_layer_f32.argtypes = [i] * 4 + [ip, ip, ip]
     L.davo_comm_preload.argtypes = [ctypes.c_char_p, i]
     L.davo_comm_unique_id.argtypes = [vp, ctypes.c_char_p, i]
     L.davo_comm_init.argtypes = [vp, i, i, vp]
diff --git a/davo_amd/csrc/api.hip b/davo_amd/csrc/api.hip
--- a/davo_amd/csrc/api.hip
+++ b/davo_amd/csrc/api.hip
@@ -6,6 +6,7 @@
 
 #include "ctx.h"
 #include "launch.h"
+#include "pad_classes.h"
 #include "plan.h"
 
 using namespace davo;
@@ -680,6 +681,7 @@
     void* misc[] = {c->d_reissue_pose, c->d_range_base, c->d_splitk, c->d_pose_tiles, c->d_w1patch, c->d_w2patch, c->d_w3patch, c->d_w1patch_f32, c->d_w2patch_f32, c->d_w3patch_f32, c->d_zeros, c->d_wpred, c->d_bpred, c->s_pose};
     for (auto p : misc) if (p) (void)hipFree(p);
     for (auto& kv : c->tile_orders) if (kv.second) (void)hipFree(kv.second);
+    for (auto& kv : c->pad_tables) { (void)hipFree(kv.second.row_pixel); (void)hipFree(kv.second.tile_taps); }
     for (auto& pe : c->prof_entries)
         for (auto& ab : pe.pending) { (void)hipEventDestroy(ab.first); (void)hipEventDestroy(ab.second); }
     for (auto e : c->event_pool) (void)hipEventDestroy(e);
@@ -843,6 +845,11 @@
     else if (k == "tile_208x128") c->opt_tile_208x128 = value != 0;
     else if (k == "merge_order") c->opt_merge_order = value < 0 ? -1 : (value > 2 ? 0 : value);
     else if (k == "skip_order") c->opt_skip_order = value < 0 ? 0 : (value > 2 ? 2 : value);
+    else if (k == "pad_classes") {
+        if (value == 0 || value == 1) c->opt_pad_classes = value ? PAD_CLASS_LAYERS : 0;
+        else if (value >= 8 && value <= 15) c->opt_pad_classes = value & 7;
+        else return fail(c, DAVO_ERR_INVALID, "pad_classes must be 0, 1 or 8 + a layer mask (8..15), got %d", value);
+    }
     else if (k == "patch_cnv2") c->opt_patch_cnv2 = value != 0;
     else if (k == "patch_cnv3") c->opt_patch_cnv3 = value != 0;
     else if (k == "fold_tails") c->opt_fold_tails = value < 0 ? -1 : (value > 2 ? 1 : value);
@@ -968,6 +975,32 @@
     if (chunk_map)
         for (int v = 0; v < 3 * fr.nky * nblocks; ++v) chunk_map[v] = h3_real_chunk(v, fr.ky0, fr.nky);
     return DAVO_OK;
+}
+
+int davo_pad_class_tables(int NB, int Hout, int Wout, int Hin, int Win, int pad_t, int pad_l, int rate, int* row_pixel, unsigned short* tile_taps) {
+    if (!row_pixel || !tile_taps || NB < 1 || Hout < 1 || Wout < 1 || Hin < 1 || Win < 1 || rate < 1 || (long)NB * Hout * Wout > 0x7fffff00L) return DAVO_ERR_INVALID;
+    std::vector<int32_t> rows;
+    std::vector<uint16_t> taps;
+    const bool sorted = pad_class_tables(NB, Hout, Wout, Hin, Win, pad_t, pad_l, rate, BM, &rows, &taps);
+    memcpy(row_pixel, rows.data(), rows.size() * sizeof(int32_t));
+    memcpy(tile_taps, taps.data(), taps.size() * sizeof(uint16_t));
+    return sorted ? 1 : 0;
+}
+
+int davo_pad_class_tile_order(const unsigned short* tile_taps, int mtile0, int mtiles, int ntiles_n, int* order) {
+    if (!tile_taps || !order || mtile0 < 0 || mtiles < 1 || ntiles_n < 1) return DAVO_ERR_INVALID;
+    std::vector<int> o;
+    pad_class_tile_order(tile_taps, mtile0, mtiles, ntiles_n, &o);
+    memcpy(order, o.data(), o.size() * sizeof(int));
+    return DAVO_OK;
+}
+
+int davo_plan_layer_f32(int mtiles, int npad, int groups, int ncu, int* mtile0, int* launch_mtiles, int* tile_bn) {
+    if (mtiles < 1 || npad < 32 || npad % 32 || groups < 1 || ncu < 1 || !mtile0 || !launch_mtiles || !tile_bn) return DAVO_ERR_INVALID;
+    const std::vector<Launch> plan = plan_layer(mtiles, npad, groups, ncu);
+    if (plan.empty() || plan.size() > 2) return DAVO_ERR_INVALID;
+    for (size_t i = 0; i < plan.size(); ++i) { mtile0[i] = plan[i].mtile0; launch_mtiles[i] = plan[i].mtiles; tile_bn[i] = plan[i].BN; }
+    return (int)plan.size();
 }
 
 int davo_plan_layer(int M, int npad, int groups, int* rows, int* tile_bm, int* tile_bn) {
diff --git a/davo_amd/csrc/conv_igemm.h b/davo_amd/csrc/conv_igemm.h
--- a/davo_amd/csrc/conv_igemm.h
+++ b/davo_amd/csrc/conv_igemm.h
@@ -62,9 +62,10 @@
     return start + (bid >> 3);
 }
 
-template <int KS, int STRIDE, int BN, int LAYER>
+template <int KS, int STRIDE, int BN, int LAYER, bool PC = false>
 __device__ __forceinline__ void conv_igemm_f32_body(const ConvParams& p, const int wg_x, const int nwg_x, const int wg_y) {
     using T = Tile<BN>;
+    static_assert(!PC || (KS == 3 && STRIDE == 1 && BN >= 32 && BN <= 128), "pad classes: the dilated 3x3 stride-1 layers on four-wave tiles");
     constexpr bool N16 = BN == 16;
     extern __shared__ __attribute__((aligned(16))) float smem[];
     float* As = smem;
@@ -90,8 +91,10 @@
 #pragma unroll
     for (int j = 0; j < 4; ++j) {
         if (j >= T::A_LOADS) { iy0[j] = -(1 << 28); ix0[j] = 0; pix0[j] = 0; continue; }
-        const int m = mtile * BM + r0 + RPP * j;
-        if (m < p.M) {
+        int m = mtile * BM + r0 + RPP * j;
+        bool m_ok = m < p.M;
+        if constexpr (PC) { m = p.row_pixel[m]; m_ok = m >= 0; }
+        if (m_ok) {
             const int hw = p.Hout * p.Wout;
             const int n = m / hw, rem = m - n * hw;
             const int oy = rem / p.Wout, ox = rem - oy * p.Wout;
@@ -114,6 +117,13 @@
     int st0 = 0, st1 = 0, st2 = 0, st3 = 0;
     const int cpt = p.cin_log2 >= 5 ? 1 << (p.cin_log2 - 5) : 1;
     int l_cb = 0;
+    int pc_taps = 0;
+    int* pc_rows = reinterpret_cast<int*>(smem + 2 * (BM + BN) * LDK);
+    if constexpr (PC) {
+        pc_taps = __builtin_amdgcn_readfirstlane(p.tile_taps[mtile]) & 0x1ff;
+        if (pc_taps == 0) pc_taps = 1 << 4;
+        if (tid < BM) pc_rows[tid] = p.row_pixel[mtile * BM + tid];
+    }
 #define DAVO_ADDR_A(j_, ptr_, st_)                                                                 \
     {                                                                                              \
         const int iy = iy0[j_] + dy, ix = ix0[j_] + dx;                                            \
@@ -126,7 +136,7 @@
 #define DAVO_LOAD_CHUNK(q_) DAVO_LOAD_CHUNK_R(q_, ra0, ra1, ra2, ra3, rb0, rb1, rb2, rb3)
 #define DAVO_LOAD_CHUNK_R(q_, ra0, ra1, ra2, ra3, rb0, rb1, rb2, rb3)                              \
     {                                                                                              \
-        const int kg = (q_) * BK + kk;                                                             \
+        const int kg = (PC ? __builtin_ctz(pc_taps) * cpt + l_cb : (q_)) * BK + kk;                \
         if (l_cb == 0) {                                                                           \
             const int tap = kg >> p.cin_log2, c = kg & cmask;                                      \
             const int ky = tap / KS, kx = tap - ky * KS;                                           \
@@ -139,6 +149,7 @@
             if constexpr (T::A_LOADS > 2) { pa2 += st2; pa3 += st3; }                              \
         }                                                                                          \
         l_cb = l_cb + 1 == cpt ? 0 : l_cb + 1;                                                     \
+        if (PC && l_cb == 0) pc_taps &= pc_taps - 1;                                               \
         ra0 = *reinterpret_cast<const float4*>(pa0);                                               \
         ra1 = *reinterpret_cast<const float4*>(pa1);                                               \
         if constexpr (T::A_LOADS > 2) {                                                            \
@@ -194,7 +205,9 @@
     }
 
     int q0 = 0, q1 = p.nchunks;
-    if constexpr (KS == 3) {
+    if constexpr (PC) {
+        q1 = __builtin_popcount(pc_taps) * cpt;
+    } else if constexpr (KS == 3) {
         if (p.cin_log2 >= 5) {
             const FilterRows fr = valid_filter_rows(mtile * BM, min(mtile * BM + BM, p.M) - 1, p.Hout, p.Wout, p.Hin, STRIDE, p.pad_t, p.rate);
             const int per_row = 3 << (p.cin_log2 - 5);
@@ -385,15 +398,16 @@
         }
         return;
     }
-    if (DAVO_F32_FAST_EPILOGUE && (mtile + 1) * BM <= p.M && (ntile + 1) * BN <= p.Cout) {
-        float* __restrict__ tbase = yg + (long)mtile * BM * p.y_ld + ntile * BN;
+    if (DAVO_F32_FAST_EPILOGUE && (mtile + 1) * BM <= p.M && (ntile + 1) * BN <= p.Cout && (!PC || (long)p.M * p.y_ld <= 0x7fffffffL)) {
+        float* __restrict__ tbase = yg + (PC ? 0L : (long)mtile * BM * p.y_ld) + ntile * BN;
         const unsigned ld = (unsigned)p.y_ld;
         const bool relu = p.relu != 0;
 #pragma unroll
         for (int i = 0; i < T::TM; ++i)
 #pragma unroll
             for (int r = 0; r < 16; ++r) {
-                const unsigned roff = (unsigned)(wm * T::TM * 32 + i * 32 + (r & 3) + 8 * (r >> 2) + 4 * lh) * ld + (unsigned)(wn * T::TN * 32 + li);
+                const int trow = wm * T::TM * 32 + i * 32 + (r & 3) + 8 * (r >> 2) + 4 * lh;
+                const unsigned roff = (unsigned)(PC ? pc_rows[trow] : trow) * ld + (unsigned)(wn * T::TN * 32 + li);
 #pragma unroll
                 for (int j = 0; j < T::TN; ++j) {
                     float v = acc[i][j][r];
@@ -413,10 +427,10 @@
 #pragma unroll
             for (int r = 0; r < 16; ++r) {
                 const int row = wm * T::TM * 32 + i * 32 + (r & 3) + 8 * (r >> 2) + 4 * lh;
-                const int m = mtile * BM + row;
+                const int m = PC ? pc_rows[row] : mtile * BM + row;
                 float v = acc[i][j][r];
                 if (p.relu) v = fmaxf(v, 0.f);
-                if (n_ok && m < p.M) yg[(long)m * p.y_ld + n] = v;
+                if (n_ok && (PC ? m >= 0 : m < p.M)) yg[(long)m * p.y_ld + n] = v;
             }
     }
 }
@@ -424,6 +438,12 @@
 template <int KS, int STRIDE, int BN, int LAYER>
 __global__ __launch_bounds__(256, 2) void conv_igemm_f32(ConvParams p) {
     conv_igemm_f32_body<KS, STRIDE, BN, LAYER>(p, blockIdx.x, gridDim.x, blockIdx.y);
+}
+
+constexpr int PC_LDS_EXTRA = BM * 4;
+template <int KS, int STRIDE, int BN, int LAYER>
+__global__ __launch_bounds__(256, 2) void conv_igemm_f32_pc(ConvParams p) {
+    conv_igemm_f32_body<KS, STRIDE, BN, LAYER, true>(p, blockIdx.x, gridDim.x, blockIdx.y);
 }
 
 template <int KS, int STRIDE, int LAYER>
@@ -436,6 +456,13 @@
     const int b = blockIdx.x, nm = groups * n_main;
     if (b < nm) conv_igemm_f32_body<KS, STRIDE, 128, LAYER>(pm, b % n_main, n_main, b / n_main);
     else conv_igemm_f32_body<KS, STRIDE, RBN, LAYER>(pr, (b - nm) % n_rem, n_rem, (b - nm) / n_rem);
+}
+
+template <int KS, int STRIDE, int RBN, int LAYER>
+__global__ __launch_bounds__(256, 2) void conv_igemm_f32_mainrem_pc(ConvParams pm, ConvParams pr, int n_main, int n_rem, int groups) {
+    const int b = blockIdx.x, nm = groups * n_main;
+    if (b < nm) conv_igemm_f32_body<KS, STRIDE, 128, LAYER, true>(pm, b % n_main, n_main, b / n_main);
+    else conv_igemm_f32_body<KS, STRIDE, RBN, LAYER, true>(pr, (b - nm) % n_rem, n_rem, (b - nm) / n_rem);
 }
 
 #undef DAVO_ADDR_A
diff --git a/davo_amd/csrc/ctx.h b/davo_amd/csrc/ctx.h
--- a/davo_amd/csrc/ctx.h
+++ b/davo_amd/csrc/ctx.h
@@ -83,6 +83,13 @@
     bool h3 = false;
     bool f32_fallback = false;
 };
+
+struct PadTables {
+    int* row_pixel = nullptr;
+    unsigned short* tile_taps = nullptr;
+    std::vector<uint16_t> host_taps;
+};
+constexpr int PAD_CLASS_LAYERS = 6;
 
 struct Comm;
 
@@ -107,6 +114,8 @@
     int opt_merge_order = -1;
     int opt_skip_order = 1;
     std::map<std::vector<int>, int*> tile_orders;
+    int opt_pad_classes = davo::PAD_CLASS_LAYERS;
+    std::map<std::vector<int>, davo::PadTables> pad_tables;
     bool opt_tile_208x128 = false;
     bool opt_merge_cnv4 = false;
     bool opt_share_taps = true;
diff --git a/davo_amd/csrc/forward.hip b/davo_amd/csrc/forward.hip
--- a/davo_amd/csrc/forward.hip
+++ b/davo_amd/csrc/forward.hip
@@ -4,6 +4,7 @@
 
 #include "ctx.h"
 #include "launch.h"
+#include "pad_classes.h"
 #include "plan.h"
 
 namespace davo {
@@ -110,6 +111,53 @@
     return dev;
 }
 
+const PadTables* pad_tables_for(davo_ctx* c, int li, int NB, int Hout, int Wout, int Hin, int Win, int pad_t, int pad_l, int rate, int* rc) {
+    *rc = DAVO_OK;
+    const std::vector<int> key = {li, NB, Hout, Wout, Hin, Win, pad_t, pad_l, rate};
+    auto it = c->pad_tables.find(key);
+    if (it != c->pad_tables.end()) return it->second.row_pixel ? &it->second : nullptr;
+    PadTables t;
+    std::vector<int32_t> rows;
+    if (!pad_class_tables(NB, Hout, Wout, Hin, Win, pad_t, pad_l, rate, BM, &rows, &t.host_taps)) {
+        c->pad_tables[key] = PadTables();
+        return nullptr;
+    }
+    auto upload = [&](void** dev, const void* src, size_t bytes) {
+        if (hipMalloc(dev, bytes) != hipSuccess) { *dev = nullptr; return false; }
+        return hipMemcpy(*dev, src, bytes, hipMemcpyHostToDevice) == hipSuccess;
+    };
+    if (!upload(reinterpret_cast<void**>(&t.row_pixel), rows.data(), rows.size() * sizeof(int32_t)) ||
+        !upload(reinterpret_cast<void**>(&t.tile_taps), t.host_taps.data(), t.host_taps.size() * sizeof(uint16_t))) {
+        if (t.row_pixel) (void)hipFree(t.row_pixel);
+        if (t.tile_taps) (void)hipFree(t.tile_taps);
+        *rc = fail(c, DAVO_ERR_HIP, "pad-class tables of layer %d: %s", li, hipGetErrorString(hipGetLastError()));
+        return nullptr;
+    }
+    return &(c->pad_tables[key] = std::move(t));
+}
+
+const int* tile_order_pc(davo_ctx* c, int li, int mtile0, int mtiles, int ntiles_n, int M, int Hout, int Wout, const PadTables& t) {
+    if (!c->opt_skip_order) return nullptr;
+    const std::vector<int> key = {li, 100, BM, mtile0, mtiles, ntiles_n, M, Hout, Wout};
+    auto it = c->tile_orders.find(key);
+    if (it != c->tile_orders.end()) return it->second;
+    bool uniform = true;
+    for (int m = 1; m < mtiles; ++m) uniform = uniform && tap_count(t.host_taps[mtile0 + m]) == tap_count(t.host_taps[mtile0]);
+    int* dev = nullptr;
+    if (!uniform) {
+        std::vector<int> order;
+        pad_class_tile_order(t.host_taps.data(), mtile0, mtiles, ntiles_n, &order);
+        if (hipMalloc(reinterpret_cast<void**>(&dev), order.size() * sizeof(int)) != hipSuccess ||
+            hipMemcpy(dev, order.data(), order.size() * sizeof(int), hipMemcpyHostToDevice) != hipSuccess) {
+            if (dev) (void)hipFree(dev);
+            dev = nullptr;
+            (void)hipGetLastError();
+        }
+    }
+    c->tile_orders[key] = dev;
+    return dev;
+}
+
 int slot_scratch(davo_ctx* c, const Run& run, float** buf, size_t* floats, size_t need, float** region, size_t extra_bytes = 0) {
     if (need > *floats) {
         if (*buf) { int rs = sync_all_slots(c); if (rs) return rs; HIP_TRY(c, hipFree(*buf)); *buf = nullptr; }
@@ -146,7 +194,15 @@
         if (pose_mt) *pose_mt = mtiles;
     }
     c->last_plan[li][0] = c->last_plan[li][1] = 0; c->last_split[li] = 1;
+    const PadTables* pc = nullptr;
+    if (li >= 3 && li <= 5 && ((c->opt_pad_classes >> (li - 3)) & 1) && L.KS == 3 && L.stride == 1 && L.cin_log2 >= 5 && L.groups == 1 && !fuse_pose && !c->opt_f32_n256) {
+        int rc = DAVO_OK;
+        pc = pad_tables_for(c, li, NB, Ho, Wo, Hin, Win, pt, pl, L.rate, &rc);
+        if (rc) return rc;
+        if (pc) { p.row_pixel = pc->row_pixel; p.tile_taps = pc->tile_taps; }
+    }
     auto order_for = [&](const Launch& l, int ntn) {
+        if (pc) return tile_order_pc(c, li, l.mtile0, l.mtiles, ntn, p.M, Ho, Wo, *pc);
         return (L.KS == 3 && L.cin_log2 >= 5) ? tile_order_for(c, li, 0, BM, l.mtile0, l.mtiles, ntn, p.M, Ho, Wo, Hin, L.stride, pt, L.rate) : nullptr;
     };
     if (c->opt_f32_n256 && (li == 4 || li == 5) && L.npad == 256 && L.groups == 1 && !fuse_pose && mtiles >= c->ncu) {
@@ -186,7 +242,7 @@
         p.mtile0 = plan[i].mtile0;
         p.ntiles_n = plan[i].BN == 16 ? 1 : L.npad / plan[i].BN;
         dim3 grid(plan[i].mtiles * p.ntiles_n, L.groups);
-        p.tile_order = (L.KS == 3 && L.cin_log2 >= 5) ? tile_order_for(c, li, 0, BM, plan[i].mtile0, plan[i].mtiles, p.ntiles_n, p.M, Ho, Wo, Hin, L.stride, pt, L.rate) : nullptr;
+        p.tile_order = order_for(plan[i], p.ntiles_n);
         const std::string label = i == 0 ? std::string(L.label) : std::string(L.label) + ".rem";
         ProfScope ps(c, run.stream, label.c_str());
         HIP_TRY(c, launch_layer(li, plan[i].BN, p, grid, run.stream));
diff --git a/davo_amd/csrc/launch_f32.hip b/davo_amd/csrc/launch_f32.hip
--- a/davo_amd/csrc/launch_f32.hip
+++ b/davo_amd/csrc/launch_f32.hip
@@ -10,6 +10,34 @@
     hipError_t e = ensure_dynamic_lds(reinterpret_cast<const void*>(kern), Tile<BN>::LDS_BYTES);
     if (e != hipSuccess) return e;
     hipLaunchKernelGGL(kern, grid, dim3(256), Tile<BN>::LDS_BYTES, s, p);
+    return hipGetLastError();
+}
+
+template <int BN, int LAYER>
+hipError_t launch_conv_pc_t(const ConvParams& p, dim3 grid, hipStream_t s) {
+    auto kern = conv_igemm_f32_pc<3, 1, BN, LAYER>;
+    hipError_t e = ensure_dynamic_lds(reinterpret_cast<const void*>(kern), Tile<BN>::LDS_BYTES + PC_LDS_EXTRA);
+    if (e != hipSuccess) return e;
+    hipLaunchKernelGGL(kern, grid, dim3(256), Tile<BN>::LDS_BYTES + PC_LDS_EXTRA, s, p);
+    return hipGetLastError();
+}
+
+template <int LAYER>
+hipError_t launch_bn_pc(int BN, const ConvParams& p, dim3 grid, hipStream_t s) {
+    switch (BN) {
+        case 32: return launch_conv_pc_t<32, LAYER>(p, grid, s);
+        case 64: return launch_conv_pc_t<64, LAYER>(p, grid, s);
+        case 128: return launch_conv_pc_t<128, LAYER>(p, grid, s);
+    }
+    return hipErrorInvalidValue;
+}
+
+template <int RBN, int LAYER>
+hipError_t launch_mainrem_pc_t(const ConvParams& pm, const ConvParams& pr, int n_main, int n_rem, int groups, hipStream_t s) {
+    auto kern = conv_igemm_f32_mainrem_pc<3, 1, RBN, LAYER>;
+    hipError_t e = ensure_dynamic_lds(reinterpret_cast<const void*>(kern), Tile<128>::LDS_BYTES + PC_LDS_EXTRA);
+    if (e != hipSuccess) return e;
+    hipLaunchKernelGGL(kern, dim3((n_main + n_rem) * groups), dim3(256), Tile<128>::LDS_BYTES + PC_LDS_EXTRA, s, pm, pr, n_main, n_rem, groups);
     return hipGetLastError();
 }
 
@@ -51,6 +79,19 @@
 
 hipError_t launch_layer_mainrem(int layer, int rbn, const ConvParams& pm, const ConvParams& pr, int n_main, int n_rem, int groups, hipStream_t s) {
     if (n_main < 8 || n_main % 8 || n_rem < 1 || (groups > 1 && n_rem % 8)) return hipErrorInvalidValue;
+    if ((pm.row_pixel != nullptr) != (pr.row_pixel != nullptr)) return hipErrorInvalidValue;
+    if (pm.row_pixel) {
+        if (!pm.tile_taps || !pr.tile_taps) return hipErrorInvalidValue;
+        switch (layer * 1000 + rbn) {
+            case 3032: return launch_mainrem_pc_t<32, 4>(pm, pr, n_main, n_rem, groups, s);
+            case 3064: return launch_mainrem_pc_t<64, 4>(pm, pr, n_main, n_rem, groups, s);
+            case 4032: return launch_mainrem_pc_t<32, 5>(pm, pr, n_main, n_rem, groups, s);
+            case 4064: return launch_mainrem_pc_t<64, 5>(pm, pr, n_main, n_rem, groups, s);
+            case 5032: return launch_mainrem_pc_t<32, 6>(pm, pr, n_main, n_rem, groups, s);
+            case 5064: return launch_mainrem_pc_t<64, 6>(pm, pr, n_main, n_rem, groups, s);
+        }
+        return hipErrorInvalidValue;
+    }
     switch (layer * 1000 + rbn) {
         case 3032: return launch_mainrem_t<3, 1, 32, 4>(pm, pr, n_main, n_rem, groups, s);
         case 3064: return launch_mainrem_t<3, 1, 64, 4>(pm, pr, n_main, n_rem, groups, s);
@@ -85,6 +126,15 @@
 
 hipError_t launch_layer(int layer, int BN, const ConvParams& p, dim3 grid, hipStream_t s) {
     if (layer == 0 && BN == 16) return launch_conv_t<7, 2, 16, 1>(p, grid, s);
+    if (p.row_pixel) {
+        if (!p.tile_taps) return hipErrorInvalidValue;
+        switch (layer) {
+            case 3: return launch_bn_pc<4>(BN, p, grid, s);
+            case 4: return launch_bn_pc<5>(BN, p, grid, s);
+            case 5: return launch_bn_pc<6>(BN, p, grid, s);
+        }
+        return hipErrorInvalidValue;
+    }
     switch (layer) {
         case 0: return launch_bn<7, 2, 1>(BN, p, grid, s);
         case 1: return launch_bn<5, 2, 2>(BN, p, grid, s);
diff --git a/davo_amd/csrc/pad_classes.h b/davo_amd/csrc/pad_classes.h
--- /dev/null
+++ b/davo_amd/csrc/pad_classes.h
@@ -0,0 +1,104 @@
+#pragma once
+#include <stdint.h>
+
+#include <algorithm>
+#include <vector>
+
+namespace davo {
+
+constexpr int PAD_CLASS_BLOCKS = 8;
+
+inline unsigned real_tap_mask(int oy, int ox, int Hin, int Win, int pad_t, int pad_l, int rate) {
+    unsigned rows = 0, cols = 0;
+    for (int k = 0; k < 3; ++k) {
+        const int iy = oy - pad_t + k * rate, ix = ox - pad_l + k * rate;
+        if (iy >= 0 && iy < Hin) rows |= 1u << k;
+        if (ix >= 0 && ix < Win) cols |= 1u << k;
+    }
+    unsigned m = 0;
+    for (int ky = 0; ky < 3; ++ky)
+        if (rows >> ky & 1) m |= cols << (3 * ky);
+    return m;
+}
+
+inline int tap_count(unsigned mask) { return __builtin_popcount(mask & 0x1ffu); }
+
+inline bool pad_class_tables(int NB, int Hout, int Wout, int Hin, int Win, int pad_t, int pad_l, int rate, int bm,
+                             std::vector<int32_t>* row_pixel, std::vector<uint16_t>* tile_taps) {
+    const int hw = Hout * Wout;
+    const long M = (long)NB * hw;
+    const long mtiles = (M + bm - 1) / bm;
+    row_pixel->assign((size_t)(mtiles * bm), -1);
+    tile_taps->assign((size_t)mtiles, 0);
+    std::vector<uint16_t> pmask(hw);
+    std::vector<int> by_class[512];
+    std::vector<int> classes;
+    for (int oy = 0; oy < Hout; ++oy)
+        for (int ox = 0; ox < Wout; ++ox) {
+            const unsigned m = real_tap_mask(oy, ox, Hin, Win, pad_t, pad_l, rate);
+            pmask[oy * Wout + ox] = (uint16_t)m;
+            if (by_class[m].empty()) classes.push_back((int)m);
+            by_class[m].push_back(oy * Wout + ox);
+        }
+    std::sort(classes.begin(), classes.end(), [](int a, int b) {
+        const int ca = tap_count(a), cb = tap_count(b);
+        return ca != cb ? ca > cb : a < b;
+    });
+    const int G = (NB + PAD_CLASS_BLOCKS - 1) / PAD_CLASS_BLOCKS;
+    long row = 0;
+    for (int n0 = 0; n0 < NB; n0 += G) {
+        const int n1 = std::min(NB, n0 + G);
+        for (int cls : classes)
+            for (int n = n0; n < n1; ++n)
+                for (int pos : by_class[cls]) {
+                    (*row_pixel)[(size_t)row] = n * hw + pos;
+                    (*tile_taps)[(size_t)(row / bm)] |= pmask[pos];
+                    ++row;
+                }
+    }
+    std::vector<uint16_t> flat((size_t)mtiles, 0);
+    for (long m = 0; m < M; ++m) flat[(size_t)(m / bm)] |= pmask[m % hw];
+    long walked_sorted = 0, walked_flat = 0;
+    for (long t = 0; t < mtiles; ++t) { walked_sorted += tap_count((*tile_taps)[(size_t)t]); walked_flat += tap_count(flat[(size_t)t]); }
+    if (walked_flat <= walked_sorted) {
+        for (long m = 0; m < M; ++m) (*row_pixel)[(size_t)m] = (int32_t)m;
+        *tile_taps = flat;
+        return false;
+    }
+    return true;
+}
+
+inline void pad_class_tile_order(const uint16_t* tile_taps, int mtile0, int mtiles, int ntiles_n, std::vector<int>* order) {
+    const int nt = mtiles * ntiles_n;
+    order->assign((size_t)nt, 0);
+    const int q = nt >> 3, r = nt & 7;
+    int cap[8], start[8];
+    long load[8];
+    std::vector<int> runs[8];
+    for (int x = 0; x < 8; ++x) {
+        start[x] = x < r ? x * (q + 1) : r * (q + 1) + (x - r) * q;
+        cap[x] = q + (x < r ? 1 : 0);
+        load[x] = 0;
+    }
+    std::vector<int> same;
+    for (int want = 9; want >= 0; --want) {
+        same.clear();
+        for (int t = 0; t < nt; ++t)
+            if (tap_count(tile_taps[mtile0 + t / ntiles_n]) == want) same.push_back(t);
+        if (same.empty()) continue;
+        int cnt[8] = {0, 0, 0, 0, 0, 0, 0, 0};
+        for (size_t i = 0; i < same.size(); ++i) {
+            int best = -1;
+            for (int x = 0; x < 8; ++x)
+                if (cap[x] > 0 && (best < 0 || load[x] < load[best])) best = x;
+            ++cnt[best]; --cap[best]; load[best] += want;
+        }
+        size_t i = 0;
+        for (int x = 0; x < 8; ++x)
+            for (int k = 0; k < cnt[x]; ++k) runs[x].push_back(same[i++]);
+    }
+    for (int x = 0; x < 8; ++x)
+        for (size_t k = 0; k < runs[x].size(); ++k) (*order)[(size_t)start[x] + k] = runs[x][k];
+}
+
+}
diff --git a/davo_amd/csrc/params.h b/davo_amd/csrc/params.h
--- a/davo_amd/csrc/params.h
+++ b/davo_amd/csrc/params.h
@@ -82,6 +82,8 @@
     const float* pose_w;
     float* pose_partial;
     int pose_P, pose_mt;
+    const int* row_pixel;
+    const unsigned short* tile_taps;
 };
 
 constexpr int BM = 128;
diff --git a/include/davo_hip.h b/include/davo_hip.h
--- a/include/davo_hip.h
+++ b/include/davo_hip.h
@@ -136,6 +136,11 @@
 int davo_tile_filter_rows(int m0, int m1, int Hout, int Wout, int Hin, int stride, int pad_t, int rate,
                           int* ky0, int* nky, int nblocks, int* chunk_map);
 
+int davo_pad_class_tables(int NB, int Hout, int Wout, int Hin, int Win, int pad_t, int pad_l, int rate,
+                          int* row_pixel, unsigned short* tile_taps);
+int davo_pad_class_tile_order(const unsigned short* tile_taps, int mtile0, int mtiles, int ntiles_n, int* order);
+int davo_plan_layer_f32(int mtiles, int npad, int groups, int ncu, int* mtile0, int* launch_mtiles, int* tile_bn);
+
 #ifdef __cplusplus
 }
 #endif
```

Measured after the change: 9118 triplets/s (median of 6 runs). +1.6%, better.
